# permon/permon

Measured on AMD Instinct MI355X. Metric: QPS iterations/sec + CSR SpMV GB/s (% HBM roofline), higher is better.
Workload: dtype f64; 1 GPU; configs[2]: 3-D elasticity TFETI contact, 2x2x2 subdomains of 43^3 Q1 elements (N=2044416 dof, n_lambda=102268), SMALXE+MPGP on the dual QP, F = B K^+ B' with K^+ explicit (dense local dual operators, storage class_orbit)

## Files before the change

permon_amd/csrc/ctx.hip:

```cpp
#include <sched.h>

#include <algorithm>
#include <thread>

#include "pmh_internal.h"

static thread_local char g_err[1024] = "";

int pmh_set_error(int code, const char *fmt, ...)
{
  va_list ap;
  va_start(ap, fmt);
  vsnprintf(g_err, sizeof(g_err), fmt, ap);
  va_end(ap);
  return code;
}

extern "C" const char *pmh_last_error(void) { return g_err; }

pmh_knobs_s &pmh_knobs()
{
  static pmh_knobs_s k = [] {
    pmh_knobs_s v;
    v.chain = getenv("PMH_NO_CHAIN") ? 0 : 1;
    v.chain_replay = getenv("PMH_NO_CHAIN_REPLAY") ? 0 : 1;
    v.svm_pairing = getenv("PMH_SVM_NO_PAIRING") ? 0 : 1;
    v.gt_fusion = getenv("PMH_NO_GT_FUSION") ? 0 : 1;
    v.multi_rhs = getenv("PMH_NO_MULTI_RHS") ? 0 : 1;
    v.kplus_mv = getenv("PMH_NO_KPLUS_MV") ? 0 : 1;
    v.smalxe_prefetch = getenv("PMH_SMALXE_NO_PREFETCH") ? 0 : 1;
    v.mg_d0_fusion = getenv("PMH_MG_NO_D0_FUSION") ? 0 : 1;
    v.vec_epi = getenv("PMH_NO_VEC_EPI") ? 0 : 1;
    v.mpgp_spec = getenv("PMH_MPGP_NO_SPEC") ? 0 : 1;
    v.orbit_adapted = getenv("PMH_NO_ORBIT_ADAPTED") ? 0 : 1;
    int         nt = 0;
    const char *e  = getenv("PMH_HOST_THREADS");
    if (!e) e = getenv("OMP_NUM_THREADS");
    if (e) nt = atoi(e);
    if (nt <= 0) {
      cpu_set_t set;
      CPU_ZERO(&set);
      nt = (sched_getaffinity(0, sizeof(set), &set) == 0) ? CPU_COUNT(&set) : (int)std::thread::hardware_concurrency();
      nt = std::min(16, nt);
    }
    v.host_threads = std::max(1, std::min(64, nt));
    return v;
  }();
  return k;
}
static int *knob_by_name(const char *name)
{
  if (!name) return nullptr;
  if (!strcmp(name, "chain")) return &pmh_knobs().chain;
  if (!strcmp(name, "chain_applies")) return &pmh_knobs().chain_applies;
  if (!strcmp(name, "chain_launches")) return &pmh_knobs().chain_launches;
  if (!strcmp(name, "chain_replay")) return &pmh_knobs().chain_replay;
  if (!strcmp(name, "chain_replays")) return &pmh_knobs().chain_replays;
  if (!strcmp(name, "chain_replays_redone")) return &pmh_knobs().chain_replays_redone;
  if (!strcmp(name, "host_threads")) return &pmh_knobs().host_threads;
  if (!strcmp(name, "svm_pairing")) return &pmh_knobs().svm_pairing;
  if (!strcmp(name, "gt_fusion")) return &pmh_knobs().gt_fusion;
  if (!strcmp(name, "multi_rhs")) return &pmh_knobs().multi_rhs;
  if (!strcmp(name, "kplus_mv")) return &pmh_knobs().kplus_mv;
  if (!strcmp(name, "smalxe_prefetch")) return &pmh_knobs().smalxe_prefetch;
  if (!strcmp(name, "mg_d0_fusion")) return &pmh_knobs().mg_d0_fusion;
  if (!strcmp(name, "mpgp_spec")) return &pmh_knobs().mpgp_spec;
  if (!strcmp(name, "vec_epi")) return &pmh_knobs().vec_epi;
  if (!strcmp(name, "orbit_adapted")) return &pmh_knobs().orbit_adapted;
  if (!strcmp(name, "orbit_adapted_classes")) return &pmh_knobs().orbit_adapted_classes;
  if (!strcmp(name, "orbit_adapted_fallbacks")) return &pmh_knobs().orbit_adapted_fallbacks;
  if (!strcmp(name, "orbit_adapted_spoil")) return &pmh_knobs().orbit_adapted_spoil;
  if (!strcmp(name, "orbit_narrow")) return &pmh_knobs().orbit_narrow;
  return nullptr;
}
extern "C" int pmh_set_knob(const char *name, int value)
{
  int *k = knob_by_name(name);
  if (!k) return pmh_set_error(PMH_ERR_ARG, "pmh_set_knob: unknown switch '%s'", name ? name : "(null)");
  *k = value;
  return PMH_SUCCESS;
}
extern "C" int pmh_get_knob(const char *name, int *value)
{
  int *k = knob_by_name(name);
  if (!k || !value) return pmh_set_error(PMH_ERR_ARG, "pmh_get_knob: unknown switch '%s'", name ? name : "(null)");
  *value = *k;
  return PMH_SUCCESS;
}

extern "C" int pmh_init(int device, pmh_ctx *out)
{
  PMH_ARG(out);
  int ndev = 0;
  if (hipGetDeviceCount(&ndev) != hipSuccess || ndev <= 0) return pmh_set_error(PMH_ERR_NODEVICE, "pmh_init: no HIP device visible (libpermonhip has no CPU fallback)");
  if (device < 0 || device >= ndev) return pmh_set_error(PMH_ERR_ARG, "pmh_init: device %d out of range [0,%d)", device, ndev);
  PMH_HIP(hipSetDevice(device));
  hipDeviceProp_t prop;
  PMH_HIP(hipGetDeviceProperties(&prop, device));
  if (!strstr(prop.gcnArchName, "gfx950")) return pmh_set_error(PMH_ERR_NODEVICE, "pmh_init: device %d is %s; libpermonhip is built for gfx950 (MI355X) only", device, prop.gcnArchName);
  pmh_ctx c  = new pmh_ctx_s();
  c->device  = device;
  c->num_cus = prop.multiProcessorCount;
  c->comm    = nullptr;
  c->rank    = 0;
  c->size    = 1;
  c->dist_scalars = 0;
  c->force_comm = getenv("PMH_COMM_FORCE") ? 1 : 0;
  PMH_HIP(hipStreamCreateWithFlags(&c->stream, hipStreamNonBlocking));
  PMH_HIP(hipEventCreate(&c->ev0));
  PMH_HIP(hipEventCreate(&c->ev1));
  c->partials_cap = PMH_MAX_VEC_BLOCKS;
  PMH_HIP(hipMalloc((void **)&c->d_partials, sizeof(double) * PMH_MAX_RED * c->partials_cap));
  PMH_HIP(hipMalloc((void **)&c->d_scal, sizeof(double) * PMH_NSCAL));
  PMH_HIP(hipMemset(c->d_scal, 0, sizeof(double) * PMH_NSCAL));
  PMH_HIP(hipHostMalloc((void **)&c->h_scal, sizeof(double) * PMH_NSCAL, hipHostMallocMapped));
  memset(c->h_scal, 0, sizeof(double) * PMH_NSCAL);
  PMH_HIP(hipHostMalloc((void **)&c->h_partials, sizeof(double) * PMH_MAX_RED * c->partials_cap, hipHostMallocMapped));
  memset(c->h_partials, 0, sizeof(double) * PMH_MAX_RED * c->partials_cap);
  PMH_HIP(hipMalloc((void **)&c->d_commbuf, sizeof(double) * PMH_NSCAL));
  *out = c;
  return PMH_SUCCESS;
}

extern "C" int pmh_finalize(pmh_ctx c)
{
  if (!c) return PMH_SUCCESS;
  hipSetDevice(c->device);
  hipStreamSynchronize(c->stream);
  if (c->comm) ncclCommDestroy(c->comm);
  for (int i = 0; i < c->comm_ev_cap; i++) hipEventDestroy(c->comm_ev[i]);
  delete[] c->comm_ev;
  if (c->h_stage) (void)hipHostFree(c->h_stage);
  hipFree(c->d_partials);
  hipFree(c->d_scal);
  hipFree(c->d_commbuf);
  hipHostFree(c->h_scal);
  hipHostFree(c->h_partials);
  hipEventDestroy(c->ev0);
  hipEventDestroy(c->ev1);
  hipStreamDestroy(c->stream);
  delete c;
// ... 262 lines not shown
```

permon_amd/csrc/dualchain.hip:

```cpp
#include <algorithm>
#include <cmath>
#include <type_traits>

#include "dualchain.h"
#include "emit_inline.h"
#include "box_inline.h"
#include "reduce.h"

struct pmh_dualchain_s {
  pmh_ctx  ctx;
  pmh_qppf pf;
  pmh_op   F;
  int      n, m, nwg, nseg, W;
  pmh_csr  gather = nullptr, scatter = nullptr;
  double  *mid_in = nullptr;
  const double *mid_out = nullptr;
  int     *d_seg = nullptr, *d_lrow = nullptr;
  double        *d_ev = nullptr;
  unsigned char *d_ec = nullptr;
  pmh_csr  list_for = nullptr;
  unsigned long long list_uid = 0, sc_uid = 0;
  double  *zeroed   = nullptr;
  int      nlist = 0, *d_reci = nullptr;
  double  *d_recd = nullptr;
  pmh_csr  sc_for = nullptr;
  int     *d_sc2 = nullptr;
  double  *d_sv2 = nullptr;
  unsigned char *d_scnt = nullptr;
  double  *part[3] = {nullptr, nullptr, nullptr};
  double  *c_cur   = nullptr;
  double  *w       = nullptr;
  double  *normGu    = nullptr;
  int      norm_slot = -1;
  const double *x_emitted = nullptr;
  bool     norm_done = false;
  const double *norm_ptr = nullptr;
  int      launches = 0;
  const double      *kept_x     = nullptr;
  unsigned long long kept_epoch = 0;
};


__global__ __launch_bounds__(PMH_EMIT_TILE) void k_dc_emit(int n, const double *__restrict__ x, pmh_emit_args ea)
{
  pmh_emit_regs R;
  pmh_emit_prefetch(ea, R);
  const int r = blockIdx.x * PMH_EMIT_TILE + threadIdx.x;
  pmh_emit_tail(ea, R, r < n ? x[r] : 0.0, 0.0);
}

template <int NU>
__global__ __launch_bounds__(PMH_EMIT_TILE) void k_dc_norm(pmh_emit_tab tab, const double *__restrict__ part, const double *__restrict__ Tt,
                        double *__restrict__ y2, double *__restrict__ norm_d,
                                                         double *__restrict__ norm_h)
{
  __shared__ double pt[PMH_EMIT_NW][64];
  const int         lane = threadIdx.x & 63, wave = threadIdx.x >> 6, m = tab.m;
  double            s1, s2;
  pmh_coarse_share<4, NU>(tab, part, Tt, nullptr, nullptr, s1, s2);
  pt[wave][lane] = s1;
  __syncthreads();
  if (wave == 0) {
    double y = 0.0;
#pragma unroll
    for (int w = 0; w < PMH_EMIT_NW; w++) y += pt[w][lane];
    if (lane < m) y2[lane] = y;
    const double sq = pmh_wave_all<PMH_RED_SUM>(lane < m ? y * y : 0.0);
    if (lane == 0) *norm_d = sq, *norm_h = sq;
  }
}

template <int W>
static __device__ __forceinline__ void dc_gt_load(const double *__restrict__ ev, const unsigned char *__restrict__ ec, int j, double (&v)[W],
                        unsigned char (&c)[W])
{
  typedef double dbl2 __attribute__((ext_vector_type(2)));
#pragma unroll
  for (int e = 0; e < W; e += 2) {
    const dbl2 d = *(const dbl2 *)(ev + (size_t)j * W + e);
    v[e] = d.x, v[e + 1] = d.y;
  }
#pragma unroll
  for (int h = 0; h < W / 8; h++) {
    const unsigned long long cc = *(const unsigned long long *)(ec + (size_t)j * W + 8 * h);
#pragma unroll
    for (int e = 0; e < 8; e++) c[8 * h + e] = (unsigned char)(cc >> (8 * e));
  }
}

struct dc_norm_args {
  const double *part, *Tt;
  double       *y2, *norm_d, *norm_h;
};
template <int W, int NU>
__global__ __launch_bounds__(PMH_EMIT_TILE) void k_dc_gather(int nlist, const int *__restrict__ reci, const double *__restrict__ recd,
                        const int *__restrict__ bcol, const double *__restrict__ bval,
                                                        const double *__restrict__ ev, const unsigned char *__restrict__ ec, pmh_emit_tab tab, const double *__restrict__ part,
                                                        const double *__restrict__ S, double *__restrict__ c_out, dc_norm_args na, const double *__restrict__ x, double *__restrict__ mid)
{
  typedef int    int4v __attribute__((ext_vector_type(4)));
  typedef double dbl2 __attribute__((ext_vector_type(2)));
  __shared__ double cs[64], ps[PMH_EMIT_NW][64], pt[PMH_EMIT_NW][64];
  const int         t = threadIdx.x, lane = t & 63, wave = t >> 6, i = blockIdx.x * PMH_EMIT_TILE + t, m = tab.m;
  int4v             ra = {0, -1, 0, 0}, rb = {0, 0, 0, 0};
  dbl2              da = {0.0, 0.0}, db = {0.0, 0.0};
  if (i < nlist) {
    ra = *(const int4v *)(reci + (size_t)8 * i), rb = *(const int4v *)(reci + (size_t)8 * i + 4);
    da = *(const dbl2 *)(recd + (size_t)4 * i), db = *(const dbl2 *)(recd + (size_t)4 * i + 2);
  }
  const int    r = ra.x, r2 = ra.y, k0 = ra.z, k1 = ra.w, cnt = (i < nlist) ? k1 - k0 : 0;
  const int    j[3]  = {rb.x, rb.y, rb.z};
  const double bv[3] = {da.x, da.y, db.x};
  double        xv[3], v0[W];
  unsigned char c0[W];
#pragma unroll
  for (int u = 0; u < 3; u++) xv[u] = (u < cnt) ? x[j[u]] : 0.0;
#pragma unroll
  for (int e = 0; e < W; e++) v0[e] = 0.0, c0[e] = 0;
  if (cnt > 0) dc_gt_load<W>(ev, ec, j[0], v0, c0);
  if (na.part && blockIdx.x == gridDim.x - 1) {
    double s1, s2;
    pmh_coarse_share<4, NU>(tab, na.part, na.Tt, nullptr, nullptr, s1, s2);
    pt[wave][lane] = s1;
    __syncthreads();
    if (wave == 0) {
      double y = 0.0;
#pragma unroll
      for (int w = 0; w < PMH_EMIT_NW; w++) y += pt[w][lane];
      if (lane < m) na.y2[lane] = y;
      const double sq = pmh_wave_all<PMH_RED_SUM>(lane < m ? y * y : 0.0);
      if (lane == 0) *na.norm_d = sq, *na.norm_h = sq;
    }
    return;
  }
  {
    double s1, s2;
    pmh_coarse_share<4, NU>(tab, part, S, nullptr, nullptr, s1, s2);
    ps[wave][lane] = s1;
    __syncthreads();
    if (wave == 0) {
      double cc = 0.0;
#pragma unroll
      for (int w = 0; w < PMH_EMIT_NW; w++) cc += ps[w][lane];
      cs[lane] = cc;
      if (blockIdx.x == 0 && lane < m) c_out[lane] = cc;
    }
    __syncthreads();
  }
  if (i >= nlist) return;
  double sum = 0.0;
  {
    double q = 0.0;
#pragma unroll
    for (int e = 0; e < W; e++) q += v0[e] * cs[c0[e]];
    sum += bv[0] * (-1.0 * q + xv[0]);
  }
#pragma unroll
  for (int u = 1; u < 3; u++)
    if (u < cnt) {
      double        vv[W];
      unsigned char cc[W];
      dc_gt_load<W>(ev, ec, j[u], vv, cc);
      double q = 0.0;
#pragma unroll
      for (int e = 0; e < W; e++) q += vv[e] * cs[cc[e]];
      sum += bv[u] * (-1.0 * q + xv[u]);
    }
  for (int k = k0 + 3; k < k1; k++) {
    const int     jj = bcol[k];
// ... 181 lines not shown
  DC_CHK(pmh_memcpy_h2d(ctx, dc->d_ev, ev.data(), sizeof(double) * ev.size()));
  DC_CHK(pmh_memcpy_h2d(ctx, dc->d_ec, ec.data(), ec.size()));
  for (int s = 0; s < 3; s++) {
    DC_CHK(pmh_malloc(ctx, sizeof(double) * (size_t)(nseg + 1), (void **)&dc->part[s]));
    DC_CHK(pmh_memset(ctx, dc->part[s], 0, sizeof(double) * (size_t)(nseg + 1)));
  }
  DC_CHK(pmh_malloc(ctx, sizeof(double) * 64, (void **)&dc->c_cur));
  DC_CHK(pmh_memset(ctx, dc->c_cur, 0, sizeof(double) * 64));
  DC_CHK(pmh_malloc(ctx, sizeof(double) * ((size_t)n + nseg + 1), (void **)&dc->w));
  DC_CHK(pmh_memset(ctx, dc->w, 0, sizeof(double) * ((size_t)n + nseg + 1)));
#undef DC_CHK
  *out = dc;
  return PMH_SUCCESS;
}

static int dc_prepare_stages(pmh_dualchain dc)
{
  pmh_ctx ctx = dc->ctx;
  if (!(dc->list_for == dc->gather && dc->list_uid == dc->gather->uid && dc->zeroed == dc->mid_in)) {
    const pmh_csr       Bg = dc->gather;
    std::vector<int>    rp((size_t)Bg->nrows + 1), ci((size_t)Bg->nnz);
    std::vector<double> va((size_t)Bg->nnz);
    PMH_CHK(pmh_memcpy_d2h(ctx, rp.data(), Bg->d_rowptr, sizeof(int) * rp.size()));
    PMH_CHK(pmh_memcpy_d2h(ctx, ci.data(), Bg->d_col, sizeof(int) * ci.size()));
    PMH_CHK(pmh_memcpy_d2h(ctx, va.data(), Bg->d_val, sizeof(double) * va.size()));
    auto key = [&](int r) {
      unsigned long long h = 1469598103934665603ULL;
      for (int k = rp[r]; k < rp[r + 1]; k++) {
        unsigned long long b;
        const double       a = fabs(va[k]);
        memcpy(&b, &a, 8);
        h = (h ^ (unsigned long long)(unsigned)ci[k]) * 1099511628211ULL;
        h = (h ^ b) * 1099511628211ULL;
      }
      return h;
    };
    auto opposite = [&](int r, int q) {
      if (rp[r + 1] - rp[r] != rp[q + 1] - rp[q]) return false;
      for (int k = rp[r], l = rp[q]; k < rp[r + 1]; k++, l++)
        if (ci[k] != ci[l] || va[k] != -va[l]) return false;
      return true;
    };
    std::vector<int> partner((size_t)Bg->nrows, -1);
    {
      std::vector<std::pair<unsigned long long, int>> keyed;
      for (int r = 0; r < Bg->nrows; r++)
        if (rp[r + 1] > rp[r]) keyed.push_back({key(r), r});
      std::sort(keyed.begin(), keyed.end());
      for (size_t a = 0; a < keyed.size(); a++) {
        const int r = keyed[a].second;
        if (partner[r] != -1) continue;
        for (size_t b = a + 1; b < keyed.size() && keyed[b].first == keyed[a].first; b++) {
          const int q = keyed[b].second;
          if (partner[q] == -1 && opposite(r, q)) {
            partner[r] = q, partner[q] = -2;
            break;
          }
        }
      }
    }
    std::vector<int>    reci;
    std::vector<double> recd;
    for (int r = 0; r < Bg->nrows; r++) {
      if (rp[r + 1] == rp[r] || partner[r] == -2) continue;
      const int k0 = rp[r], k1 = rp[r + 1];
      int       j[3] = {0, 0, 0};
      double    b[3] = {0.0, 0.0, 0.0};
      for (int u = 0; u < 3 && k0 + u < k1; u++) j[u] = ci[k0 + u], b[u] = va[k0 + u];
      const int ints[8] = {r, partner[r] >= 0 ? partner[r] : -1, k0, k1, j[0], j[1], j[2], 0};
      reci.insert(reci.end(), ints, ints + 8);
      recd.push_back(b[0]), recd.push_back(b[1]), recd.push_back(b[2]), recd.push_back(0.0);
    }
    if (dc->d_reci) {
      PMH_CHK(pmh_free(ctx, dc->d_reci));
      PMH_CHK(pmh_free(ctx, dc->d_recd));
    }
    dc->d_reci = nullptr, dc->d_recd = nullptr;
    PMH_CHK(pmh_malloc(ctx, sizeof(int) * (reci.size() + 8), (void **)&dc->d_reci));
    PMH_CHK(pmh_malloc(ctx, sizeof(double) * (recd.size() + 4), (void **)&dc->d_recd));
    PMH_CHK(pmh_memcpy_h2d(ctx, dc->d_reci, reci.data(), sizeof(int) * reci.size()));
    PMH_CHK(pmh_memcpy_h2d(ctx, dc->d_recd, recd.data(), sizeof(double) * recd.size()));
    PMH_CHK(pmh_memset(ctx, dc->mid_in, 0, sizeof(double) * (size_t)Bg->nrows));
    dc->nlist = (int)(reci.size() / 8), dc->list_for = Bg, dc->list_uid = Bg->uid, dc->zeroed = dc->mid_in;
  }
  if (dc->sc_for != dc->scatter || dc->sc_uid != dc->scatter->uid) {
    const pmh_csr       Bs = dc->scatter;
    const int           n  = dc->n;
    std::vector<int>    rp((size_t)n + 1), ci((size_t)Bs->nnz);
    std::vector<double> va((size_t)Bs->nnz);
    PMH_CHK(pmh_memcpy_d2h(ctx, rp.data(), Bs->d_rowptr, sizeof(int) * rp.size()));
    PMH_CHK(pmh_memcpy_d2h(ctx, ci.data(), Bs->d_col, sizeof(int) * ci.size()));
    PMH_CHK(pmh_memcpy_d2h(ctx, va.data(), Bs->d_val, sizeof(double) * va.size()));
    std::vector<int>           sc2((size_t)2 * n, 0);
    std::vector<double>        sv2((size_t)2 * n, 0.0);
    std::vector<unsigned char> cnt((size_t)n, 0);
    for (int r = 0; r < n; r++) {
      const int c = rp[r + 1] - rp[r];
      cnt[r]      = (unsigned char)std::min(c, 255);
      for (int u = 0; u < 2 && u < c; u++) sc2[(size_t)2 * r + u] = ci[rp[r] + u], sv2[(size_t)2 * r + u] = va[rp[r] + u];
    }
    if (!dc->d_sc2) {
      PMH_CHK(pmh_malloc(ctx, sizeof(int) * sc2.size(), (void **)&dc->d_sc2));
      PMH_CHK(pmh_malloc(ctx, sizeof(double) * sv2.size(), (void **)&dc->d_sv2));
      PMH_CHK(pmh_malloc(ctx, cnt.size(), (void **)&dc->d_scnt));
    }
    PMH_CHK(pmh_memcpy_h2d(ctx, dc->d_sc2, sc2.data(), sizeof(int) * sc2.size()));
    PMH_CHK(pmh_memcpy_h2d(ctx, dc->d_sv2, sv2.data(), sizeof(double) * sv2.size()));
    PMH_CHK(pmh_memcpy_h2d(ctx, dc->d_scnt, cnt.data(), cnt.size()));
    dc->sc_for = Bs, dc->sc_uid = Bs->uid;
  }
  return PMH_SUCCESS;
}

void pmh_dc_destroy(pmh_dualchain dc)
{
  if (!dc) return;
  pmh_free(dc->ctx, dc->d_seg), pmh_free(dc->ctx, dc->d_lrow), pmh_free(dc->ctx, dc->d_ev), pmh_free(dc->ctx, dc->d_ec);
  if (dc->d_reci) pmh_free(dc->ctx, dc->d_reci), pmh_free(dc->ctx, dc->d_recd);
  if (dc->d_sc2) pmh_free(dc->ctx, dc->d_sc2), pmh_free(dc->ctx, dc->d_sv2), pmh_free(dc->ctx, dc->d_scnt);
  for (int s = 0; s < 3; s++) pmh_free(dc->ctx, dc->part[s]);
  pmh_free(dc->ctx, dc->c_cur), pmh_free(dc->ctx, dc->w);
  delete dc;
}

static int dc_nu(pmh_dualchain dc) { return dc->nwg <= 128 ? 2 : 8; }

template <int V> using dc_int = std::integral_constant<int, V>;
template <typename F>
static void dc_dispatch(pmh_dualchain dc, F f)
{
  const bool w8 = dc->W == 8, nu2 = dc_nu(dc) == 2;
  if (w8 && nu2) f(dc_int<8>(), dc_int<2>());
  else if (w8) f(dc_int<8>(), dc_int<8>());
  else if (nu2) f(dc_int<16>(), dc_int<2>());
  else f(dc_int<16>(), dc_int<8>());
}

static pmh_emit_tab dc_tab(pmh_dualchain dc)
{
  pmh_emit_tab t;
  t.seg = dc->d_seg, t.gcol = dc->pf->G->d_col, t.gval = dc->pf->G->d_val, t.lrow = dc->d_lrow, t.m = dc->m, t.nwg = dc->nwg;
  return t;
}

static pmh_emit_args dc_emit_args(pmh_dualchain dc, double *part0, double *part1)
{
  pmh_emit_args ea;
  memset(&ea, 0, sizeof(ea));
  ea.tab = dc_tab(dc), ea.o[0].part = part0, ea.o[1].part = part1;
  return ea;
}

static void dc_launch_emit(pmh_dualchain dc, const double *x, double *part)
{
  hipLaunchKernelGGL(k_dc_emit, dim3((unsigned)dc->nwg), dim3(PMH_EMIT_TILE), 0, dc->ctx->stream, dc->n, x, dc_emit_args(dc, part, nullptr));
}

int pmh_dc_emit_begin(pmh_dualchain dc, const double *x, const double *p, pmh_emit_args *ea)
{
  *ea = dc_emit_args(dc, x ? dc->part[0] : nullptr, p ? dc->part[1] : nullptr);
  if ((x && x == dc->kept_x) || (p && p == dc->kept_x)) dc->kept_x = nullptr;
  if (x) dc->x_emitted = x, dc->norm_done = false, dc->norm_ptr = nullptr;
  return PMH_SUCCESS;
}

void pmh_dc_invalidate(pmh_dualchain dc, bool keep_applied)
// ... 2 lines not shown
  if (!keep_applied) dc->kept_x = nullptr;
}

int pmh_dc_set_norm_target(pmh_dualchain dc, double *Gu, int slot)
{
  PMH_ARG(dc && Gu && slot >= 0 && slot < PMH_NSCAL);
  dc->normGu = Gu, dc->norm_slot = slot, dc->norm_ptr = nullptr, dc->norm_done = false;
  return PMH_SUCCESS;
}

bool pmh_dc_norm_ready(pmh_dualchain dc, const double *u)
{
  if (!dc || !dc->normGu) return false;
  if (dc->norm_ptr == u) return true;
  if (dc->x_emitted == u && !dc->norm_done) {
    dc_dispatch(dc, [&](auto, auto NU) {
      hipLaunchKernelGGL(k_dc_norm<decltype(NU)::value>, dim3(1), dim3(PMH_EMIT_TILE), 0, dc->ctx->stream, dc_tab(dc), (const double *)dc->part[0], (const double *)dc->pf->d_Tt, dc->normGu,
                         dc->ctx->d_scal + dc->norm_slot, dc->ctx->h_scal + dc->norm_slot);
    });
    if (hipGetLastError() != hipSuccess) return false;
    dc->norm_done = true, dc->norm_ptr = u;
    return true;
  }
  return false;
}
int pmh_dc_last_launches(pmh_dualchain dc) { return dc ? dc->launches : 0; }

static int dc_last_stage(pmh_dualchain dc, const double *x, double *y, double rho, const pmh_vec_epi *epi)
{
  pmh_ctx     ctx = dc->ctx;
  hipStream_t st  = ctx->stream;
  const int   n = dc->n;
  const dim3  vgrid((unsigned)dc->nwg), eblk(PMH_EMIT_TILE);
  const int   kind = epi ? epi->kind : 0;
  pmh_emit_args ea = dc_emit_args(dc, nullptr, nullptr);
  pmh_vec_epi   e;
  memset(&e, 0, sizeof(e));
  if (epi) e = *epi;
  e.h_partials = nullptr;
  if (epi && epi->hosted) e.h_partials = ctx->h_partials, *epi->hosted = dc->nwg;
  if (kind == PMH_VEPI_GRAD_SPLIT && epi->emitted_p) {
    ea.o[1].part    = dc->part[1];
    *epi->emitted_p = 1;
  }
  dc_dispatch(dc, [&](auto W, auto NU) {
    constexpr int w = decltype(W)::value, nu = decltype(NU)::value;
    auto kern = kind == PMH_VEPI_P1 ? k_dc_final<PMH_VEPI_P1, w, nu> : kind == PMH_VEPI_GRAD_SPLIT ? k_dc_final<PMH_VEPI_GRAD_SPLIT, w, nu> : k_dc_final<0, w, nu>;
    hipLaunchKernelGGL(kern, vgrid, eblk, 0, st, n, (const double *)dc->d_ev, (const unsigned char *)dc->d_ec, ea.tab, (const double *)dc->pf->d_S, (const double *)dc->c_cur, (const double *)dc->w, rho, y,
                       e, x, ea);
  });
  dc->launches++;
  PMH_HIP(hipGetLastError());
  return PMH_SUCCESS;
}

int pmh_dc_apply(pmh_dualchain dc, const double *x, double *y, double rho, const pmh_vec_epi *epi)
{
  pmh_ctx     ctx = dc->ctx;
  hipStream_t st  = ctx->stream;
  const int   n = dc->n;
  const dim3  vgrid((unsigned)dc->nwg), eblk(PMH_EMIT_TILE);
  const int   kind = epi ? epi->kind : 0;
  dc->launches     = 0;
  dc->kept_x       = nullptr;
  const pmh_emit_tab tab = dc_tab(dc);
  int slot = (epi && epi->in_slot > 0) ? epi->in_slot - 1 : -1;
  if (slot < 0) {
    slot = (kind == PMH_VEPI_GRAD_SPLIT) ? 0 : (kind == PMH_VEPI_P1 ? 1 : 2);
    if (slot == 0) dc->x_emitted = x, dc->norm_done = false, dc->norm_ptr = nullptr;
    dc_launch_emit(dc, x, dc->part[slot]);
    dc->launches++;
  }
  PMH_CHK(dc->F->stages(&dc->gather, &dc->mid_in, &dc->scatter, &dc->mid_out));
  const pmh_csr Bg = dc->gather, Bs = dc->scatter;
  if (Bg->ncols != n || Bs->nrows != n) return pmh_set_error(PMH_ERR_STATE, "pmh_dc_apply: the operator's stages changed their dual dimension");
  PMH_CHK(dc_prepare_stages(dc));
  {
    dc_norm_args na;
    memset(&na, 0, sizeof(na));
    if (dc->normGu && dc->x_emitted && !dc->norm_done) {
      na.part = dc->part[0], na.Tt = dc->pf->d_Tt, na.y2 = dc->normGu, na.norm_d = ctx->d_scal + dc->norm_slot, na.norm_h = ctx->h_scal + dc->norm_slot;
      dc->norm_done = true, dc->norm_ptr = dc->x_emitted;
    }
    const dim3 ggrid((unsigned)(std::max(1, (dc->nlist + PMH_EMIT_TILE - 1) / PMH_EMIT_TILE) + (na.part ? 1 : 0)));
    dc_dispatch(dc, [&](auto W, auto NU) {
      hipLaunchKernelGGL(HIP_KERNEL_NAME(k_dc_gather<decltype(W)::value, decltype(NU)::value>), ggrid, eblk, 0, st, dc->nlist, (const int *)dc->d_reci, (const double *)dc->d_recd,
                         (const int *)Bg->d_col, (const double *)Bg->d_val, (const double *)dc->d_ev, (const unsigned char *)dc->d_ec, tab, (const double *)dc->part[slot],
                         (const double *)dc->pf->d_S, dc->c_cur, na, x, dc->mid_in);
    });
    dc->launches++;
  }
  PMH_HIP(hipGetLastError());
  PMH_CHK(dc->F->mid_apply());
  hipLaunchKernelGGL(k_dc_scatter, vgrid, eblk, 0, st, n, (const unsigned char *)dc->d_scnt, (const int *)dc->d_sc2, (const double *)dc->d_sv2, (const int *)Bs->d_rowptr, (const int *)Bs->d_col,
                     (const double *)Bs->d_val, dc->mid_out, dc->w, dc_emit_args(dc, dc->w + n, nullptr));
  dc->launches++;
  PMH_HIP(hipGetLastError());
  PMH_CHK(pmh_comm_allreduce_sum(ctx, dc->w, (size_t)n + (size_t)dc->nseg));
  PMH_CHK(dc_last_stage(dc, x, y, rho, epi));
  dc->kept_x = x, dc->kept_epoch = ctx->free_epoch;
  pmh_knobs().chain_applies++, pmh_knobs().chain_launches += dc->launches;
  return PMH_SUCCESS;
}

int pmh_dc_replay(pmh_dualchain dc, const double *x, double *y, double rho, const pmh_vec_epi *epi, int *replayed)
{
  const int kind = epi ? epi->kind : 0;
  if (replayed) *replayed = 0;
  bool      ok   = pmh_knobs().chain_replay && x && dc->kept_x == x && dc->kept_epoch == dc->ctx->free_epoch && (kind == 0 || kind == PMH_VEPI_GRAD_SPLIT);
  if (ok) {
    pmh_csr       g = nullptr, sc = nullptr;
    double       *mi = nullptr;
    const double *mo = nullptr;
    PMH_CHK(dc->F->stages(&g, &mi, &sc, &mo));
    ok = g && sc && g == dc->list_for && g->uid == dc->list_uid && mi == dc->zeroed && sc == dc->sc_for && sc->uid == dc->sc_uid && mo == dc->mid_out;
  }
  if (!ok) return pmh_dc_apply(dc, x, y, rho, epi);
  dc->launches = 0;
  if (kind == PMH_VEPI_GRAD_SPLIT && !(epi->in_slot > 0)) {
    dc->x_emitted = x, dc->norm_done = false, dc->norm_ptr = nullptr;
    dc_launch_emit(dc, x, dc->part[0]);
    dc->launches++;
  }
  PMH_CHK(dc_last_stage(dc, x, y, rho, epi));
  if (replayed) *replayed = 1;
  pmh_knobs().chain_applies++, pmh_knobs().chain_replays++, pmh_knobs().chain_launches += dc->launches;
  return PMH_SUCCESS;
}

int pmh_dc_test_emit(pmh_dualchain dc, const double *x)
{
  pmh_emit_args ea;
  PMH_CHK(pmh_dc_emit_begin(dc, x, nullptr, &ea));
  dc_launch_emit(dc, x, ea.o[0].part);
  PMH_HIP(hipGetLastError());
  return PMH_SUCCESS;
}
int pmh_dc_test_direction_sums(pmh_dualchain dc, int cap, double *host, int *nseg)
{
  PMH_ARG(host && nseg && cap >= dc->nseg);
  *nseg = dc->nseg;
  return pmh_memcpy_d2h(dc->ctx, host, dc->part[1], sizeof(double) * (size_t)dc->nseg);
}
int pmh_dc_test_info(pmh_dualchain dc, long long info[10])
{
  pmh_ctx ctx = dc->ctx;
  PMH_CHK(dc->F->stages(&dc->gather, &dc->mid_in, &dc->scatter, &dc->mid_out));
  PMH_CHK(dc_prepare_stages(dc));
  std::vector<int>           reci((size_t)8 * dc->nlist);
  std::vector<unsigned char> cnt((size_t)dc->n);
  PMH_CHK(pmh_memcpy_d2h(ctx, reci.data(), dc->d_reci, sizeof(int) * reci.size()));
  PMH_CHK(pmh_memcpy_d2h(ctx, cnt.data(), dc->d_scnt, cnt.size()));
  long long np = 0, n3 = 0, n2 = 0;
  for (int i = 0; i < dc->nlist; i++) np += reci[(size_t)8 * i + 1] >= 0, n3 += reci[(size_t)8 * i + 3] - reci[(size_t)8 * i + 2] > 3;
  for (int r = 0; r < dc->n; r++) n2 += cnt[r] > 2;
  const long long v[10] = {dc->n, dc->m, dc->nwg, dc->nseg, dc->W, dc_nu(dc), dc->nlist, np, n3, n2};
  for (int k = 0; k < 10; k++) info[k] = v[k];
  return PMH_SUCCESS;
}
int pmh_dc_test_read(pmh_dualchain dc, int what, int cap, double *host, int *len)
{
  PMH_ARG(host && len && what >= 0 && what <= 10);
  PMH_ARG(what < 4 || what > 6 || what == 6 || (dc->gather && dc->scatter));
  PMH_ARG((what != 7 && what != 8) || dc->normGu);
  pmh_ctx       ctx = dc->ctx;
  const int     m = dc->m;
  const double *src[11] = {dc->part[0], dc->part[1], dc->part[2], dc->c_cur, dc->mid_in, dc->mid_out, dc->w, dc->normGu, nullptr, dc->pf->d_S, dc->pf->d_Tt};
  const int     cnt[11] = {dc->nseg, dc->nseg, dc->nseg, m, dc->gather ? dc->gather->nrows : 0, dc->scatter ? dc->scatter->ncols : 0, dc->n + dc->nseg, m, 2, m * m, m * m};
  PMH_ARG(cap >= cnt[what]);
  *len = cnt[what];
  PMH_CHK(pmh_sync(ctx));
  if (what == 8) {
    host[1] = ctx->h_scal[dc->norm_slot];
    return pmh_memcpy_d2h(ctx, host, ctx->d_scal + dc->norm_slot, sizeof(double));
  }
  return pmh_memcpy_d2h(ctx, host, src[what], sizeof(double) * (size_t)cnt[what]);
}

struct StagedOp : pmh_op_s {
  pmh_csr g, mdl, sc;
  double *mi = nullptr, *mo = nullptr;
  ~StagedOp() override
  {
    pmh_free(ctx, mi);
    pmh_free(ctx, mo);
  }
  int mult(const double *x, double *y) override
  {
    PMH_CHK(pmh_csr_mult(g, x, mi));
    PMH_CHK(pmh_csr_mult(mdl, mi, mo));
    return pmh_csr_mult(sc, mo, y);
  }
  int stages(pmh_csr *gather, double **mid_in, pmh_csr *scatter, const double **mid_out) override
  {
    *gather = g, *mid_in = mi, *scatter = sc, *mid_out = mo;
    return PMH_SUCCESS;
  }
  int mid_apply() override { return pmh_csr_mult(mdl, mi, mo); }
};

extern "C" int pmh_op_test_create_staged(pmh_csr gather, pmh_csr middle, pmh_csr scatter, pmh_op *op)
{
  PMH_ARG(gather && middle && scatter && op && gather->nrows >= 1 && gather->ncols >= 1);
  PMH_ARG(middle->nrows == gather->nrows && middle->ncols == gather->nrows && scatter->nrows == gather->ncols && scatter->ncols == gather->nrows);
  StagedOp *o = new StagedOp();
  o->ctx = gather->ctx, o->n = gather->ncols, o->g = gather, o->mdl = middle, o->sc = scatter;
  const size_t bytes = sizeof(double) * (size_t)gather->nrows;
  int          rc    = pmh_malloc(o->ctx, bytes, (void **)&o->mi);
  if (!rc) rc = pmh_malloc(o->ctx, bytes, (void **)&o->mo);
  if (!rc) rc = pmh_memset(o->ctx, o->mi, 0, bytes);
  if (!rc) rc = pmh_memset(o->ctx, o->mo, 0, bytes);
  if (rc) {
    delete o;
    return rc;
  }
  *op = o;
  return PMH_SUCCESS;
}
```

permon_amd/csrc/emit_inline.h:

```cpp
#pragma once
#include <hip/hip_runtime.h>

#include "pmh_internal.h"

#define PMH_EMIT_TILE 1024
#define PMH_EMIT_NW (PMH_EMIT_TILE / 64)

template <int CTRL>
static __device__ __forceinline__ double pmh_dpp_mov(double v)
{
  int lo = __double2loint(v), hi = __double2hiint(v);
  lo     = __builtin_amdgcn_update_dpp(0, lo, CTRL, 0xf, 0xf, false);
  hi     = __builtin_amdgcn_update_dpp(0, hi, CTRL, 0xf, 0xf, false);
  return __hiloint2double(hi, lo);
}

template <int OP = PMH_RED_SUM>
static __device__ __forceinline__ double pmh_wave_all(double v)
{
#define PMH_COMB(a, b) ((OP == PMH_RED_SUM) ? ((a) + (b)) : fmin((a), (b)))
  v = PMH_COMB(v, pmh_dpp_mov<0xB1>(v));
  v = PMH_COMB(v, pmh_dpp_mov<0x4E>(v));
  v = PMH_COMB(v, pmh_dpp_mov<0x141>(v));
  v = PMH_COMB(v, pmh_dpp_mov<0x140>(v));
// ... 12 lines not shown
{
  __shared__ double bp[K][PMH_EMIT_NW];
  const int         lane = threadIdx.x & 63, wave = threadIdx.x >> 6, nw = blockDim.x >> 6;
#pragma unroll
  for (int k = 0; k < K; k++) {
    const double s = (op[k] == PMH_RED_SUM) ? pmh_wave_all<PMH_RED_SUM>(v[k]) : pmh_wave_all<PMH_RED_MIN>(v[k]);
    if (lane == 0) bp[k][wave] = s;
  }
  __syncthreads();
  if (threadIdx.x < K) {
    const int k = threadIdx.x;
    double    r = bp[k][0];
    for (int w = 1; w < nw; w++) r = (op[k] == PMH_RED_SUM) ? (r + bp[k][w]) : fmin(r, bp[k][w]);
    partials[(size_t)k * ld + blockIdx.x] = r;
    if (h_partials) h_partials[(size_t)k * ld + blockIdx.x] = r;
  }
}

static __device__ __forceinline__ double pmh_sum_block_partials(const double *__restrict__ row, int nblocks)
{
  const int lane = threadIdx.x & 63;
  double    p[8];
#pragma unroll
  for (int u = 0; u < 8; u++) p[u] = (lane + 64 * u < nblocks) ? row[lane + 64 * u] : 0.0;
  double acc = 0.0;
#pragma unroll
  for (int u = 0; u < 8; u++) acc += p[u];
  return pmh_wave_all<PMH_RED_SUM>(acc);
}

struct pmh_emit_regs {
  int    k0[4], k1[4], pp[4], gc[4][4];
  double gv[4][4];
};
static __device__ __forceinline__ void pmh_emit_prefetch(const pmh_emit_args &ea, pmh_emit_regs &R)
{
  if (ea.o[0].part == nullptr && ea.o[1].part == nullptr) return;
  const int lane = threadIdx.x & 63, wave = __builtin_amdgcn_readfirstlane(threadIdx.x >> 6), base = (int)blockIdx.x * PMH_EMIT_TILE;
#pragma unroll
  for (int q = 0; q < 4; q++) {
    const int s = (int)blockIdx.x * 64 + wave + q * PMH_EMIT_NW;
    R.k0[q] = ea.tab.seg[3 * s], R.k1[q] = ea.tab.seg[3 * s + 1], R.pp[q] = ea.tab.seg[3 * s + 2];
  }
#pragma unroll
  for (int q = 0; q < 4; q++)
#pragma unroll
    for (int u = 0; u < 4; u++) {
      const int k = R.k0[q] + lane + 64 * u;
      R.gv[q][u]  = (k < R.k1[q]) ? ea.tab.gval[k] : 0.0;
      R.gc[q][u]  = (k < R.k1[q]) ? ea.tab.gcol[k] - base : 0;
    }
}
static __device__ __forceinline__ void pmh_emit_tail(const pmh_emit_args &ea, const pmh_emit_regs &R, double v0, double v1)
{
  __shared__ double xs[2][PMH_EMIT_TILE];
  const int         t = threadIdx.x, lane = t & 63, base = (int)blockIdx.x * PMH_EMIT_TILE;
  const bool        e0 = ea.o[0].part != nullptr, e1 = ea.o[1].part != nullptr;
  if (!e0 && !e1) return;
  xs[0][t] = v0, xs[1][t] = v1;
  __syncthreads();
#pragma unroll
  for (int q = 0; q < 4; q++) {
    if (R.k1[q] <= R.k0[q]) continue;
    double a0 = 0.0, a1 = 0.0;
#pragma unroll
    for (int u = 0; u < 4; u++)
      if (R.k0[q] + lane + 64 * u < R.k1[q]) a0 += R.gv[q][u] * xs[0][R.gc[q][u]], a1 += R.gv[q][u] * xs[1][R.gc[q][u]];
    for (int k = R.k0[q] + lane + 256; k < R.k1[q]; k += 64) {
      const double v = ea.tab.gval[k];
      const int    c = ea.tab.gcol[k] - base;
      a0 += v * xs[0][c], a1 += v * xs[1][c];
    }
    if (e0) {
      a0 = pmh_wave_all<PMH_RED_SUM>(a0);
      if (lane == 0) ea.o[0].part[R.pp[q]] = a0;
    }
    if (e1) {
      a1 = pmh_wave_all<PMH_RED_SUM>(a1);
      if (lane == 0) ea.o[1].part[R.pp[q]] = a1;
    }
  }
}

template <int RPW, int NU = 8>
static __device__ __forceinline__ void pmh_coarse_share(const pmh_emit_tab &tab, const double *__restrict__ part, const double *__restrict__ M1,
                        const double *__restrict__ M2, double *a_out,
                                                       double &s1, double &s2)
{
  const int lane = threadIdx.x & 63, wave = threadIdx.x >> 6, nw = blockDim.x >> 6, m = tab.m;
  s1 = 0.0, s2 = 0.0;
#pragma unroll 1
  for (int qb = 0; qb < RPW; qb += 4) {
    if (wave + nw * qb >= m) break;
    double pv[4][NU], m1[4], m2[4];
#pragma unroll
    for (int q = 0; q < 4; q++) {
      const int  r  = wave + nw * (qb + q);
      const bool in = r < m;
      const int  c0 = in ? tab.lrow[r] : 0, c1 = in ? tab.lrow[r + 1] : 0;
#pragma unroll
      for (int u = 0; u < NU; u++) {
        const int c = c0 + lane + 64 * u;
        pv[q][u]    = (c < c1) ? part[c] : 0.0;
      }
      m1[q] = (in && M1 && lane < m) ? M1[(size_t)r * m + lane] : 0.0;
      m2[q] = (in && M2 && lane < m) ? M2[(size_t)r * m + lane] : 0.0;
    }
#pragma unroll
    for (int q = 0; q < 4; q++) {
      const int r = wave + nw * (qb + q);
      if (r >= m) break;
      double acc = 0.0;
#pragma unroll
      for (int u = 0; u < NU; u++) acc += pv[q][u];
      acc = pmh_wave_all<PMH_RED_SUM>(acc);
      if (a_out && lane == 0) a_out[r] = acc;
      s1 += m1[q] * acc, s2 += m2[q] * acc;
    }
  }
}
```

permon_amd/csrc/feti.hip:

```cpp
#include <algorithm>
#include <cmath>

#include "pmh_internal.h"
#include "feti_internal.h"
#include "mv_internal.h"
#include "diag_inv.h"
#include "reduce.h"


extern "C" int pmh_gluing_create(pmh_ctx ctx, int n_x, int n_lambda, int n_leaves, const int *leaves_row, const int *leaves_root, const double *leaves_sign, pmh_gluing *out)
{
  PMH_ARG(ctx && out && n_x >= 0 && n_lambda >= 0 && n_leaves >= 0);
  PMH_ARG(n_leaves == 0 || (leaves_row && leaves_root && leaves_sign));
  for (int i = 0; i < n_leaves; i++) {
    if (leaves_row[i] < 0 || leaves_row[i] >= n_x) return pmh_set_error(PMH_ERR_ARG, "pmh_gluing_create: leaf %d row %d out of [0,%d)", i, leaves_row[i], n_x);
    if (leaves_root[i] < 0 || leaves_root[i] >= n_lambda) return pmh_set_error(PMH_ERR_ARG, "pmh_gluing_create: leaf %d root %d out of [0,%d)", i, leaves_root[i], n_lambda);
  }
  auto build = [&](int nrows, int ncols, const int *rows, const int *cols, pmh_csr *M) -> int {
    std::vector<int>    rp((size_t)nrows + 1, 0), ci((size_t)n_leaves);
    std::vector<double> va((size_t)n_leaves);
    for (int i = 0; i < n_leaves; i++) rp[rows[i] + 1]++;
    for (int r = 0; r < nrows; r++) rp[r + 1] += rp[r];
    std::vector<int> pos(rp.begin(), rp.end() - 1);
    for (int i = 0; i < n_leaves; i++) {
// ... 727 lines not shown
  return pmh_csr_timing_enable(M->K->K, max_launches);
}

extern "C" int pmh_matinv_timing_get(pmh_matinv M, int *launches, double *total_ms, double *bytes_per_launch)
{
  PMH_ARG(M && launches && total_ms);
  if (M->mvc_state == 1) return pmh_matinv_mv_timing(M->mvc, 0, launches, total_ms, bytes_per_launch);
  if (M->Kb) {
    if (bytes_per_launch) *bytes_per_launch = pmh_bsr3_bytes(M->Kb);
    return pmh_bsr3_timing_get(M->Kb, launches, total_ms);
  }
  if (bytes_per_launch) PMH_CHK(pmh_csr_algorithmic_bytes(M->K->K, bytes_per_launch));
  return pmh_csr_timing_get(M->K->K, PMH_EPI_NONE, launches, total_ms);
}

extern "C" int pmh_matinv_multi_rhs_active(pmh_matinv M, int *active)
{
  PMH_ARG(M && active);
  PMH_CHK(matinv_mvc_init(M));
  *active = M->mvc_state == 1;
  return PMH_SUCCESS;
}

int pmh_matinv_test_pick(int entries, const double *hs, const int *hi, int cap, double *scal, int *ints)
{
  for (int e = 0; e < entries && e < cap; e++) {
    const int q = hi[(1 * entries + e) * 2 + 1] > hi[(0 * entries + e) * 2 + 1] ? 1 : 0;
    for (int k = 0; k < 2; k++) {
      if (scal) scal[2 * e + k] = hs[(q * entries + e) * 2 + k];
      if (ints) ints[2 * e + k] = hi[(q * entries + e) * 2 + k];
    }
  }
  return PMH_SUCCESS;
}
extern "C" int pmh_matinv_test_info(pmh_matinv M, long long info[8], int cap, double *scal, int *ints)
{
  PMH_ARG(M && info && cap >= 0);
  if (M->mvc_state == 1) return pmh_matinv_mv_test_state(M->mvc, info, cap, scal, ints);
  const int           nb = M->nblocks;
  std::vector<double> hs(4 * (size_t)nb);
  std::vector<int>    hi(4 * (size_t)nb);
  int                 na = 0, dn = 0;
  PMH_CHK(pmh_sync(M->ctx));
  PMH_CHK(pmh_memcpy_d2h(M->ctx, hs.data(), M->d_bs, sizeof(double) * hs.size()));
  PMH_CHK(pmh_memcpy_d2h(M->ctx, hi.data(), M->d_bi, sizeof(int) * hi.size()));
  PMH_CHK(pmh_memcpy_d2h(M->ctx, &na, M->d_nactive, sizeof(int)));
  PMH_CHK(pmh_memcpy_d2h(M->ctx, &dn, M->d_done, sizeof(int)));
  info[0] = M->wgs, info[1] = M->Kb ? 1 : 0, info[2] = 1, info[3] = na, info[4] = dn, info[5] = nb, info[6] = M->last_max_its, info[7] = M->total_spmv;
  return pmh_matinv_test_pick(nb, hs.data(), hi.data(), cap, scal, ints);
}

extern "C" int pmh_matinv_last_iterations(pmh_matinv M, int *max_block_its, long long *total_spmv)
{
  PMH_ARG(M);
  if (max_block_its) *max_block_its = M->last_max_its;
  if (total_spmv) *total_spmv = M->total_spmv;
  return PMH_SUCCESS;
}

struct FetiDualOp : pmh_op_s {
  pmh_gluing B;
  pmh_matinv Kplus;
  double    *t1, *t2;
  long long  applies = 0;
  ~FetiDualOp() override
  {
    pmh_free(ctx, t1);
    pmh_free(ctx, t2);
  }
  int mult(const double *x, double *y) override
  {
    applies++;
    if (Kplus->E && pmh_fexplicit_matches(Kplus->E, B)) return pmh_fexplicit_apply(Kplus->E, x, y);
    PMH_CHK(pmh_gluing_mult(B, x, t1));
    PMH_CHK(pmh_matinv_mult(Kplus, t1, t2));
    return pmh_gluing_mult_transpose(B, t2, y);
  }
  int mult_transpose(const double *x, double *y) override { return mult(x, y); }
  int stages(pmh_csr *gather, double **mid_in, pmh_csr *scatter, const double **mid_out) override
  {
    if (Kplus->E && pmh_fexplicit_matches(Kplus->E, B)) return pmh_fexplicit_stages(Kplus->E, gather, mid_in, scatter, mid_out);
    *gather = B->Bt, *mid_in = t1, *scatter = B->B, *mid_out = t2;
    return PMH_SUCCESS;
  }
  int mid_apply() override
  {
    applies++;
    if (Kplus->E && pmh_fexplicit_matches(Kplus->E, B)) return pmh_fexplicit_mid(Kplus->E);
    return pmh_matinv_mult(Kplus, t1, t2);
  }
};

extern "C" int pmh_feti_dual_applies(pmh_op F, long long *n)
{
  const FetiDualOp *o = dynamic_cast<const FetiDualOp *>(F);
  PMH_ARG(o && n);
  *n = o->applies;
  return PMH_SUCCESS;
}

extern "C" int pmh_op_create_feti_dual(pmh_gluing B, pmh_matinv Kplus, pmh_op *F)
{
  PMH_ARG(B && Kplus && F);
  PMH_ARG(B->n_x == Kplus->n);
  FetiDualOp *o = new FetiDualOp();
  o->ctx        = B->ctx;
  o->n          = B->n_lambda;
  o->B          = B;
  o->Kplus      = Kplus;
  PMH_CHK(pmh_malloc(o->ctx, sizeof(double) * (size_t)(B->n_x ? B->n_x : 1), (void **)&o->t1));
  PMH_CHK(pmh_malloc(o->ctx, sizeof(double) * (size_t)(B->n_x ? B->n_x : 1), (void **)&o->t2));
  *F = o;
  return PMH_SUCCESS;
}

extern "C" int pmh_pc_dual_lumped_apply(pmh_gluing B, pmh_blockdiag K, const double *x, double *y)
{
  PMH_ARG(B && K && B->n_x == K->n);
  pmh_ctx ctx = B->ctx;
  double *xw, *yw;
  PMH_CHK(pmh_malloc(ctx, sizeof(double) * (size_t)(K->n ? K->n : 1), (void **)&xw));
  PMH_CHK(pmh_malloc(ctx, sizeof(double) * (size_t)(K->n ? K->n : 1), (void **)&yw));
  int rc = pmh_gluing_mult(B, x, xw);
  if (!rc) rc = pmh_blockdiag_mult(K, xw, yw);
  if (!rc) rc = pmh_gluing_mult_transpose(B, yw, y);
  pmh_free(ctx, xw);
  pmh_free(ctx, yw);
  return rc;
}

struct pmh_feti_chain_s {
  pmh_ctx    ctx;
  pmh_gluing B;
  pmh_matinv Kplus;
  pmh_qppf   pf;
  int        n_x, n_lambda, has_box;
  pmh_op     F, A;
  double    *f, *d, *b_bar, *b, *lb_new, *lam_tilde, *t_x, *t_l;
};

extern "C" int pmh_qpt_feti_chain_create(pmh_gluing B, pmh_matinv Kplus, const double *f, const double *c, pmh_qppf pf, const double *e, const double *lb, pmh_feti_chain *out)
{
  PMH_ARG(B && Kplus && f && c && out && (!pf || e));
  PMH_ARG(B->n_x == Kplus->n && (!pf || pf->n == B->n_lambda));
  pmh_ctx          ctx = B->ctx;
  const int        nl = B->n_lambda, nx = B->n_x;
  pmh_feti_chain   ch = new pmh_feti_chain_s();
  memset(ch, 0, sizeof(*ch));
  ch->ctx = ctx, ch->B = B, ch->Kplus = Kplus, ch->pf = pf, ch->n_x = nx, ch->n_lambda = nl, ch->has_box = lb ? 1 : 0;
  const size_t bl = sizeof(double) * (size_t)(nl ? nl : 1), bx = sizeof(double) * (size_t)(nx ? nx : 1);
  PMH_CHK(pmh_malloc(ctx, bx, (void **)&ch->f));
  PMH_CHK(pmh_malloc(ctx, bx, (void **)&ch->t_x));
  PMH_CHK(pmh_malloc(ctx, bl, (void **)&ch->d));
  PMH_CHK(pmh_malloc(ctx, bl, (void **)&ch->t_l));
  PMH_CHK(pmh_malloc(ctx, bl, (void **)&ch->lam_tilde));
  PMH_CHK(pmh_memcpy_d2d(ctx, ch->f, f, bx));
  PMH_CHK(pmh_op_create_feti_dual(B, Kplus, &ch->F));
  PMH_CHK(pmh_matinv_mult(Kplus, ch->f, ch->t_x));
  PMH_CHK(pmh_gluing_mult_transpose(B, ch->t_x, ch->d));
  PMH_CHK(pmh_vec_axpy(ctx, nl, ch->d, -1.0, c));
  if (lb) {
    PMH_CHK(pmh_malloc(ctx, bl, (void **)&ch->lb_new));
    PMH_CHK(pmh_memcpy_d2d(ctx, ch->lb_new, lb, bl));
  }
  if (!pf) {
    PMH_CHK(pmh_memset(ctx, ch->lam_tilde, 0, bl));
// ... 121 lines not shown
```

permon_amd/csrc/feti_internal.h:

```cpp
#pragma once
#include <algorithm>
#include <vector>

#include "pmh_internal.h"

struct pmh_fexplicit_s;

struct pmh_gluing_s {
  pmh_ctx ctx;
  int     n_x, n_lambda, n_leaves;
  pmh_csr B, Bt;
  double *d_tmp;
  std::vector<int>    h_row, h_root;
  std::vector<double> h_sign;
};

struct pmh_blockdiag_s {
  pmh_ctx          ctx;
  int              nblocks, n;
  std::vector<int> rowstart;
  int             *d_rowstart;
  pmh_csr          K;
  pmh_bsr3         Kb = nullptr;
};

struct pmh_matinv_s {
  pmh_blockdiag K;
  pmh_ctx       ctx;
  int           n, nblocks, wgs;
  double        rtol, atol;
  int           max_it, jacobi;
  double       *dinv, *r, *z, *p, *Ap;
  double       *d_part, *d_partB;
  double       *d_bs;
  int          *d_bi;
  int          *d_nactive, *d_done, *h_nactive;
  int           last_max_its;
  long long     total_spmv;
  int     kdim;
  double *d_R, *d_coef, *d_fproj, *d_kpart;
  double *d_fnorm2 = nullptr;
  double  kernel_tol = 64.0;
  int  left = 0, nfix = 0;
  int *d_fix = nullptr;
  pmh_mg  mg;
  pmh_bsr3 Kb;
  pmh_fexplicit_s *E;
  struct pmh_matinv_mv_s *mvc = nullptr;
  int                     mvc_state = 0;
};

bool pmh_fexplicit_matches(pmh_fexplicit_s *E, pmh_gluing B);
int  pmh_fexplicit_apply(pmh_fexplicit_s *E, const double *lambda, double *y);
int  pmh_fexplicit_stages(pmh_fexplicit_s *E, pmh_csr *gather, double **mid_in, pmh_csr *scatter, const double **mid_out);
int  pmh_fexplicit_mid(pmh_fexplicit_s *E);
int  pmh_fexplicit_store_symmetrized(pmh_fexplicit_s *E, int b, const double *S, int lds);
int  pmh_fexplicit_mark_assembled(pmh_fexplicit_s *E, long long n_solves, double seconds);
struct fx_batch_window {
  int       begin = 0, end = 1 << 30;
  int       nbatch = 0;
  long long nsolves = 0;
  double    loop_seconds = 0.0;
  bool      complete = false;
};
int  pmh_fexplicit_set_window(pmh_fexplicit_s *E, fx_batch_window *w);

#include "mv_internal.h"
struct pmh_asm_solver {
  pmh_matinv    M = nullptr;
  pmh_matinv_mv V = nullptr;
  double       *umv = nullptr;
  int open(pmh_matinv solver, int nslots)
  {
    M = solver;
    if (nslots == solver->nblocks) return PMH_SUCCESS;
    if (nslots != solver->nblocks * PMH_MV_R) return pmh_set_error(PMH_ERR_ARG, "pmh_fexplicit_assemble: %d slots for a solver of %d blocks (one per block, or %d per block)", nslots, solver->nblocks, PMH_MV_R);
    int rc = pmh_matinv_mv_create(solver, &V);
    if (rc == PMH_EPI_UNSUPPORTED)
      return pmh_set_error(PMH_ERR_SUP, "pmh_fexplicit_assemble: the multi-right-hand-side K^+ does not apply to this solver: %s", pmh_mv_why());
    if (rc) return rc;
    return pmh_malloc(M->ctx, sizeof(double) * len(), (void **)&umv);
  }
  void close()
  {
    if (V) pmh_matinv_mv_destroy(V), V = nullptr;
    if (umv && M) pmh_free(M->ctx, umv), umv = nullptr;
  }
  int    R() const { return V ? PMH_MV_R : 1; }
  size_t len() const { return (size_t)std::max(1, M->n) * R(); }
  int    rows(int s) const { return M->K->rowstart[s / R() + 1] - M->K->rowstart[s / R()]; }
  int    rhs_index(int s, int rel) const { return V ? (M->K->rowstart[s / PMH_MV_R] + rel) * PMH_MV_R + s % PMH_MV_R : M->K->rowstart[s] + rel; }
  const double *sol_of(const double *sol, int s) const { return V ? sol + (size_t)(s % PMH_MV_R) * M->n + M->K->rowstart[s / PMH_MV_R] : sol + M->K->rowstart[s]; }
  int solve(const double *rhs, double *sol)
  {
    if (!V) return pmh_matinv_mult(M, rhs, sol);
    PMH_CHK(pmh_matinv_mv_mult(V, rhs, umv));
    return pmh_matinv_mv_to_columns(V, umv, sol);
  }
  bool hit_the_limit() const { return (V ? pmh_matinv_mv_last_iterations(V) : M->last_max_its) >= M->max_it; }
};
```

permon_amd/csrc/fexplicit.hip:

```cpp
#include <algorithm>
#include <thread>
#include <chrono>
#include <cmath>
#include <map>

#include "feti_internal.h"
#include "fshared.h"
#include "fx_assemble.h"
#include "pmh_internal.h"
#include "reduce.h"

typedef double dbl2 __attribute__((ext_vector_type(2)));

struct pmh_fexplicit_s {
  pmh_ctx       ctx;
  pmh_gluing    B;
  pmh_blockdiag K;
  pmh_gluing    Bhat;
  int           nb, ntot;
  std::vector<int> gstart;
  std::vector<int> ngam;
  std::vector<int> gamma;
  std::vector<size_t> goff;
  std::vector<int> ld;
// ... 958 lines not shown

int pmh_fexplicit_store_symmetrized(pmh_fexplicit_s *E, int b, const double *S, int lds)
{
  PMH_ARG(E && b >= 0 && b < E->nb && S && lds >= E->ngam[b]);
  if (E->sh || (E->storage != PMH_FX_FULL && E->storage != PMH_FX_SYM)) return pmh_set_error(PMH_ERR_SUP, "pmh_fexplicit_store_symmetrized: FULL / SYM storage only");
  if (E->stripe_size > 1) return pmh_set_error(PMH_ERR_SUP, "pmh_fexplicit_store_symmetrized: not on a striped operator");
  const int n = E->ngam[b];
  if (!n) return PMH_SUCCESS;
  const long long tot = (long long)n * n;
  const dim3      grid((unsigned)std::max(1LL, std::min(2048LL, (tot + PMH_BLOCK - 1) / PMH_BLOCK)));
  hipLaunchKernelGGL(k_fx_store_sym, grid, dim3(PMH_BLOCK), 0, E->ctx->stream, n, lds, E->ld[b], E->storage == PMH_FX_SYM ? 1 : 0, S, E->W[b]);
  PMH_HIP(hipGetLastError());
  return PMH_SUCCESS;
}

int pmh_fexplicit_mark_assembled(pmh_fexplicit_s *E, long long n_solves, double seconds)
{
  PMH_ARG(E);
  E->assembled = 1, E->n_solves += n_solves, E->assemble_seconds += seconds;
  return PMH_SUCCESS;
}


static int fx_gemv(pmh_fexplicit E)
{
  if (!E->nwg) return PMH_SUCCESS;
  if (E->storage == PMH_FX_SYM) {
    hipStream_t st    = E->ctx->stream;
    bool        timed = false;
    if (E->ev_on && (E->ev_seen++ % E->ev_stride) == 0 && (size_t)(2 * E->ev_used + 2) <= E->ev.size() && (size_t)E->ev_used < E->ev_mid.size()) {
      timed = true;
      PMH_HIP(hipEventRecord(E->ev[2 * E->ev_used], st));
    }
#define SYMV_LAUNCH(V) hipLaunchKernelGGL(k_fx_symv<V>, dim3(E->nsw), dim3(PMH_BLOCK), 0, st, (const int *)E->d_sw_block, (const int *)E->d_sw_band, (const int *)E->d_sw_seg, (const int *)E->d_gstart, (const int *)E->d_ld, (const long long *)E->d_woff, (const long long *)E->d_poff, (const long long *)E->d_doff, (const double *)E->Wbase, (const double *)E->xh, E->ydir, E->partial, E->seg)
    SYMV_LAUNCH(0);
#undef SYMV_LAUNCH
    if (timed) PMH_HIP(hipEventRecord(E->ev_mid[E->ev_used], st));
    if (E->nfw)
      hipLaunchKernelGGL(k_fx_symv_fin, dim3(E->nfw), dim3(PMH_BLOCK), 0, st, (const int *)E->d_fw_block, (const int *)E->d_fw_col0, (const int *)E->d_gstart, (const int *)E->d_ld, (const long long *)E->d_poff,
                         (const long long *)E->d_doff, (const int *)E->d_own_ptr, (const int *)E->d_own_list, (const double *)E->ydir, (const double *)E->partial, E->yh, E->seg);
    if (timed) {
      PMH_HIP(hipEventRecord(E->ev[2 * E->ev_used + 1], st));
      E->ev_used++;
    }
    PMH_HIP(hipGetLastError());
    return PMH_SUCCESS;
  }
  hipStream_t st    = E->ctx->stream;
  bool        timed = false;
  if (E->ev_on && (E->ev_seen++ % E->ev_stride) == 0 && (size_t)(2 * E->ev_used + 2) <= E->ev.size()) {
    timed = true;
    PMH_HIP(hipEventRecord(E->ev[2 * E->ev_used], st));
  }
#define FX_LAUNCH(RW) hipLaunchKernelGGL(k_fx_gemv<RW>, dim3(E->nwg), dim3(PMH_BLOCK), 0, st, (const int *)E->d_wg_block, (const int *)E->d_wg_row0, (const int *)E->d_gstart, (const int *)E->d_ngam, (const int *)E->d_ld, (const long long *)E->d_woff, (const double *)E->Wbase, (const double *)E->xh, E->yh)
  if (E->rw == 8) FX_LAUNCH(8);
  else if (E->rw == 2) FX_LAUNCH(2);
  else FX_LAUNCH(4);
#undef FX_LAUNCH
  if (timed) {
    PMH_HIP(hipEventRecord(E->ev[2 * E->ev_used + 1], st));
    E->ev_used++;
  }
  PMH_HIP(hipGetLastError());
  return PMH_SUCCESS;
}

bool pmh_fexplicit_matches(pmh_fexplicit_s *E, pmh_gluing B) { return E && E->assembled && (E->B == B || (E->stripe_size >= 1 && E->B->n_lambda == B->n_lambda)); }

int pmh_fexplicit_apply(pmh_fexplicit_s *E, const double *lambda, double *y)
{
  if (E->sh) return fxs_apply(E->sh, lambda, y);
  PMH_CHK(pmh_gluing_mult(E->Bhat, lambda, E->xh));
  PMH_CHK(fx_gemv(E));
  return pmh_gluing_mult_transpose(E->Bhat, E->yh, y);
}

int pmh_fexplicit_stages(pmh_fexplicit_s *E, pmh_csr *gather, double **mid_in, pmh_csr *scatter, const double **mid_out)
{
  if (E->sh) return fxs_stages(E->sh, gather, mid_in, scatter, mid_out);
  *gather = E->Bhat->Bt, *mid_in = E->xh, *scatter = E->Bhat->B, *mid_out = E->yh;
  return PMH_SUCCESS;
}
int pmh_fexplicit_mid(pmh_fexplicit_s *E) { return E->sh ? fxs_mid(E->sh) : fx_gemv(E); }

extern "C" int pmh_fexplicit_mult(pmh_fexplicit E, const double *lambda, double *y)
{
  PMH_ARG(E && lambda && y);
  if (!E->assembled) return pmh_set_error(PMH_ERR_STATE, "pmh_fexplicit_mult: the explicit blocks are not assembled yet");
  return pmh_fexplicit_apply(E, lambda, y);
}

extern "C" int pmh_fexplicit_dense_mult(pmh_fexplicit E, const double *xh, double *yh)
{
  PMH_ARG(E && xh && yh);
  if (E->sh) {
    const size_t nbytes = sizeof(double) * (size_t)fxs_multivector_length(E->sh);
    PMH_CHK(pmh_memcpy_d2d(E->ctx, fxs_X(E->sh), xh, nbytes));
    PMH_CHK(fxs_dense(E->sh));
    return pmh_memcpy_d2d(E->ctx, yh, fxs_Y(E->sh), nbytes);
  }
  PMH_CHK(pmh_memcpy_d2d(E->ctx, E->xh, xh, sizeof(double) * (size_t)E->ntot));
  PMH_CHK(fx_gemv(E));
  return pmh_memcpy_d2d(E->ctx, yh, E->yh, sizeof(double) * (size_t)E->ntot);
}

extern "C" int pmh_fexplicit_compressed_size(pmh_fexplicit E, int *ntot, int *gstart )
{
  PMH_ARG(E);
  if (E->sh) {
    if (ntot) *ntot = (int)fxs_multivector_length(E->sh);
    if (gstart)
      for (int b = 0; b <= E->nb; b++) gstart[b] = -1;
    return PMH_SUCCESS;
  }
  if (ntot) *ntot = E->ntot;
  if (gstart)
    for (int b = 0; b <= E->nb; b++) gstart[b] = E->gstart[b];
  return PMH_SUCCESS;
}

extern "C" int pmh_matinv_attach_explicit(pmh_matinv Kplus, pmh_fexplicit E)
{
  PMH_ARG(Kplus);
  if (E && !E->assembled) return pmh_set_error(PMH_ERR_STATE, "pmh_matinv_attach_explicit: assemble the explicit blocks first");
  if (E && E->stripe_size < 1 && E->K->n != Kplus->n) return pmh_set_error(PMH_ERR_ARG, "pmh_matinv_attach_explicit: size mismatch (%d vs %d)", E->K->n, Kplus->n);
  Kplus->E = E;
  return PMH_SUCCESS;
}

extern "C" int pmh_fexplicit_timing_enable(pmh_fexplicit E, int max_launches, int stride)
{
  PMH_ARG(E && max_launches >= 0);
  if (E->sh) return fxs_timing_enable(E->sh, max_launches);
  while ((int)E->ev.size() < 2 * max_launches) {
    hipEvent_t e;
    PMH_HIP(hipEventCreate(&e));
    E->ev.push_back(e);
  }
  while ((int)E->ev_mid.size() < max_launches) {
    hipEvent_t e;
    PMH_HIP(hipEventCreate(&e));
    E->ev_mid.push_back(e);
  }
  E->ev_on = max_launches > 0, E->ev_used = 0, E->ev_seen = 0, E->ev_stride = std::max(1, stride);
  return PMH_SUCCESS;
}

extern "C" int pmh_fexplicit_timing_get(pmh_fexplicit E, int *launches, double *total_ms, double *first_kernel_ms)
{
  PMH_ARG(E && launches && total_ms);
  if (E->sh) {
    return fxs_timing_get(E->sh, launches, total_ms, first_kernel_ms);
  }
  PMH_CHK(pmh_sync(E->ctx));
  double tot = 0.0, first = 0.0;
  for (int i = 0; i < E->ev_used; i++) {
    float ms = 0.f;
    PMH_HIP(hipEventElapsedTime(&ms, E->ev[2 * i], E->ev[2 * i + 1]));
    tot += ms;
    if (E->storage == PMH_FX_SYM) {
      PMH_HIP(hipEventElapsedTime(&ms, E->ev[2 * i], E->ev_mid[i]));
      first += ms;
    }
  }
  *launches = E->ev_used, *total_ms = tot;
  if (first_kernel_ms) *first_kernel_ms = (E->storage == PMH_FX_SYM) ? first : tot;
// ... 3 lines not shown
```

permon_amd/csrc/fshared.h:

```cpp
#pragma once
#include "feti_internal.h"

struct fx_shared;
int       fxs_create(pmh_gluing B, pmh_blockdiag K, const int *block_class, int sym, fx_shared **out, const int *extra_ptr = nullptr, const int *extra_rel = nullptr);
void      fxs_destroy(fx_shared *S);
int       fxs_set_stripe(fx_shared *S, int rank, int size);
int       fxs_class_union(fx_shared *S, int c, int *n_c, int *urel_out);
int       fxs_set_symmetry(fx_shared *S, int c, int nsym, const int *posmap, const signed char *sign);
int       fxs_set_symmetry_ops(fx_shared *S, int c, int nsym, const int *ops);
int       fxs_orbit_adapted(fx_shared *S, int c);
long long fxs_dense_bytes(fx_shared *S);
double    fxs_apply_bytes(fx_shared *S);
double    fxs_apply_flops(fx_shared *S);
void      fxs_apply_flops_detail(fx_shared *S, double *issued, double *dense);
int       fxs_assemble(fx_shared *S, pmh_matinv solver, int nslots, const int *slot_class, double rtol, int max_it, long long *n_solves, fx_batch_window *w = nullptr);
int       fxs_apply(fx_shared *S, const double *lambda, double *y);
int       fxs_dense(fx_shared *S);
int       fxs_stages(fx_shared *S, pmh_csr *gather, double **mid_in, pmh_csr *scatter, const double **mid_out);
int       fxs_mid(fx_shared *S);
long long fxs_multivector_length(fx_shared *S);
double   *fxs_X(fx_shared *S);
double   *fxs_Y(fx_shared *S);
int       fxs_fill_pattern(fx_shared *S, int byte);
int       fxs_get_block(fx_shared *S, int b, int n, const int *gamma, double *out_host);
int       fxs_test_load_class(fx_shared *S, int c, const double *W_host, int *all_loaded);
int       fxs_orbit_plan_info(fx_shared *S, int c, long long info[24]);
int       fxs_orbit_adapted_info(fx_shared *S, int c, long long info[200]);
int       fxs_orbit_adapted_transform(fx_shared *S, int c, int inverse, const double *in, double *out);
int       fxs_timing_enable(fx_shared *S, int max_launches);
int       fxs_timing_get(fx_shared *S, int *launches, double *total_ms, double *first_kernel_ms);
```

permon_amd/csrc/fshared.hip:

```cpp
#include "fshared_adapted.h"
#include "fx_assemble.h"
#include "orbitbasis.h"

extern char **environ;

static int fxs_build_launch(fx_shared *S)
{
  if (S->sym) {
    struct band { int c, g, m, nj; };
    std::vector<band> bands;
    long long         steps = 0;
    for (int c = 0; c < S->ncls; c++) {
      fxs_class &C = S->C[c];
      for (int m = C.nmb - 1; m >= 0; m--) {
        if (!C.own[FXM_MB * m]) continue;
        for (int g = 0; g < C.ngroups; g++) {
          const int nj = std::min(C.nsb, FXM_MB * (m + 1)) * FXM_RT;
          bands.push_back({c, g, m, nj});
          steps += (nj + 1) / 2;
        }
      }
    }
    int nwg = (int)std::max(1LL, std::min((long long)S->ctx->num_cus, steps));
    if (const char *e = getenv("PMH_FXM_NWG")) nwg = std::max(1, atoi(e));
// ... 161 lines not shown
    } else if (sym) {
      C.nsb = C.ld / FXM_RS, C.nmb = (C.nsb + FXM_MB - 1) / FXM_MB;
      C.own.assign((size_t)std::max(1, C.nsb), 1);
      C.ptm.assign((size_t)C.nmb + 1, 0);
      for (int m = 0; m < C.nmb; m++) C.ptm[m + 1] = C.ptm[m] + (long long)std::min(C.nsb, FXM_MB * (m + 1)) * FXM_RS * FXS_S;
      C.ptoff = pttot, C.ptsize = C.ptm[C.nmb];
      pttot += C.ngroups * C.ptsize;
      wtot += (long long)FXM_RS * FXM_RS * ((long long)C.nsb * (C.nsb + 1) / 2);
    } else
      wtot += (long long)C.ld * C.ld;
    xtot += (long long)C.ngroups * C.ld * C.S;
    PMH_CHK(pmh_malloc(ctx, sizeof(int) * (size_t)std::max(1, C.nc), (void **)&C.d_urel));
    if (C.nc) PMH_CHK(pmh_memcpy_h2d(ctx, C.d_urel, C.urel.data(), sizeof(int) * (size_t)C.nc));
  }
  if (xtot >= (1LL << 31)) return pmh_set_error(PMH_ERR_SUP, "pmh_fexplicit_create_shared: the multivector numbering exceeds 32-bit indices");
  S->nX = xtot, S->wtot = wtot;
  std::vector<int> rows((size_t)std::max(1, B->n_leaves));
  for (int i = 0; i < B->n_leaves; i++) {
    const int        b = lb[i];
    const fxs_class &C = S->C[S->cls[b]];
    rows[i]            = (int)(C.xoff + (long long)group[b] * C.ld * C.S + (long long)C.pos[B->h_row[i] - K->rowstart[b]] * C.S + slot[b]);
  }
  if (sym == 2) {
    for (auto &C : S->C) C.tmask.assign((size_t)std::max(1, C.ngroups) * std::max(1, C.nc) * FXS_S, 0);
    for (int i = 0; i < B->n_leaves; i++) {
      const int  b = lb[i];
      fxs_class &C = S->C[S->cls[b]];
      C.tmask[((size_t)group[b] * C.nc + C.pos[B->h_row[i] - K->rowstart[b]]) * FXS_S + slot[b]] = 1;
    }
    for (auto &C : S->C) {
      PMH_CHK(pmh_malloc(ctx, C.tmask.size(), (void **)&C.d_tmask));
      PMH_CHK(pmh_memcpy_h2d(ctx, C.d_tmask, C.tmask.data(), C.tmask.size()));
    }
  }
  PMH_CHK(pmh_gluing_create(ctx, (int)std::max(1LL, xtot), B->n_lambda, B->n_leaves, rows.data(), B->h_root.data(), B->h_sign.data(), &S->Bc));
  if (sym == 2) {
    if (2 * xtot >= (1LL << 31)) return pmh_set_error(PMH_ERR_SUP, "pmh_fexplicit_create_shared_orbit: the signed multivector numbering exceeds 32-bit indices");
    std::vector<int>    rows2((size_t)std::max(1, 2 * B->n_leaves)), root2((size_t)std::max(1, 2 * B->n_leaves));
    std::vector<double> sign2((size_t)std::max(1, 2 * B->n_leaves));
    for (int i = 0; i < B->n_leaves; i++) {
      const int slot_i = slot[lb[i]], base = rows[i] - slot_i, Sc = S->C[S->cls[lb[i]]].S;
      rows2[2 * i] = 2 * base + slot_i, rows2[2 * i + 1] = 2 * base + Sc + slot_i;
      root2[2 * i] = root2[2 * i + 1] = B->h_root[i];
      sign2[2 * i] = B->h_sign[i], sign2[2 * i + 1] = -B->h_sign[i];
    }
    PMH_CHK(pmh_gluing_create(ctx, (int)std::max(1LL, 2 * xtot), B->n_lambda, 2 * B->n_leaves, rows2.data(), root2.data(), sign2.data(), &S->Bc2));
    PMH_CHK(pmh_malloc(ctx, sizeof(double) * (size_t)std::max(32LL, 2 * xtot), (void **)&S->X2));
    PMH_CHK(pmh_memset(ctx, S->X2, 0, sizeof(double) * (size_t)std::max(32LL, 2 * xtot)));
  }
  {
    const size_t bytes = sizeof(double) * (size_t)std::max(32LL, wtot);
    hipError_t   e     = hipMalloc((void **)&S->Wbase, bytes);
    if (e != hipSuccess) return pmh_set_error(PMH_ERR_HIP, "pmh_fexplicit_create_shared: %.2f GB for the shared explicit operators: %s", bytes / 1e9, hipGetErrorString(e));
    PMH_HIP(hipMemsetAsync(S->Wbase, 0, bytes, ctx->stream));
  }
  if (sym == 1) {
    S->pt_tot = pttot;
    PMH_CHK(pmh_malloc(ctx, sizeof(double) * (size_t)std::max(16LL, pttot), (void **)&S->pt));
  }
  PMH_CHK(pmh_malloc(ctx, sizeof(double) * (size_t)std::max(16LL, xtot), (void **)&S->X));
  PMH_CHK(pmh_malloc(ctx, sizeof(double) * (size_t)std::max(16LL, xtot), (void **)&S->Y));
  PMH_CHK(pmh_memset(ctx, S->X, 0, sizeof(double) * (size_t)std::max(16LL, xtot)));
  PMH_CHK(pmh_memset(ctx, S->Y, 0, sizeof(double) * (size_t)std::max(16LL, xtot)));
  std::vector<int>       ldv(S->ncls);
  std::vector<long long> wo(S->ncls), xo(S->ncls);
  for (int c = 0; c < S->ncls; c++) ldv[c] = S->C[c].ld, wo[c] = S->C[c].woff, xo[c] = S->C[c].xoff;
  PMH_CHK(pmh_malloc(ctx, sizeof(int) * S->ncls, (void **)&S->d_ld));
  PMH_CHK(pmh_malloc(ctx, sizeof(long long) * S->ncls, (void **)&S->d_woff));
  PMH_CHK(pmh_malloc(ctx, sizeof(long long) * S->ncls, (void **)&S->d_xoff));
  PMH_CHK(pmh_memcpy_h2d(ctx, S->d_ld, ldv.data(), sizeof(int) * S->ncls));
  PMH_CHK(pmh_memcpy_h2d(ctx, S->d_woff, wo.data(), sizeof(long long) * S->ncls));
  PMH_CHK(pmh_memcpy_h2d(ctx, S->d_xoff, xo.data(), sizeof(long long) * S->ncls));
  if (sym != 2) PMH_CHK(fxs_build_launch(S));
  *out = S;
  return PMH_SUCCESS;
}

static void fxa_free(pmh_ctx ctx, fxs_class &C)
{
  fxa_class *a = C.oa;
  if (!a) return;
  if (a->Wh) (void)hipFree(a->Wh);
  for (void *q : {(void *)a->d_ir, (void *)a->d_tab, (void *)a->Xh, (void *)a->Yh, (void *)a->d_toff, (void *)a->d_osize, (void *)a->d_tbase, (void *)a->d_opos, (void *)a->d_rowinfo, (void *)a->d_items,
                  (void *)a->d_tmask, (void *)a->d_tabN, (void *)a->d_tabNT, (void *)a->d_nfx, (void *)a->d_nyd, (void *)a->d_nxh, (void *)a->d_nyh})
    if (q) pmh_free(ctx, q);
  delete a;
  C.oa = nullptr;
}

void fxs_destroy(fx_shared *S)
{
  if (!S) return;
  pmh_ctx ctx = S->ctx;
  for (auto &C : S->C) {
    if (C.d_urel) pmh_free(ctx, C.d_urel);
    if (C.d_tmask) pmh_free(ctx, C.d_tmask);
    if (C.d_nseg) pmh_free(ctx, C.d_nseg);
    if (C.d_ptoff) pmh_free(ctx, C.d_ptoff);
    if (C.d_ownfirst) pmh_free(ctx, C.d_ownfirst);
    if (C.d_posmap) pmh_free(ctx, C.d_posmap), pmh_free(ctx, C.d_sign);
    if (C.d_gidx) pmh_free(ctx, C.d_gidx), pmh_free(ctx, C.d_reppos), pmh_free(ctx, C.d_use);
    if (C.d_coltab) pmh_free(ctx, C.d_coltab), pmh_free(ctx, C.d_fintab), pmh_free(ctx, C.d_finbase);
    if (C.d_kinv) pmh_free(ctx, C.d_kinv), pmh_free(ctx, C.d_unittab), pmh_free(ctx, C.d_lut);
    fxa_free(ctx, C);
  }
  if (S->pt) pmh_free(ctx, S->pt);
  if (S->d_wgl) pmh_free(ctx, S->d_wgl);
  if (S->d_items) pmh_free(ctx, S->d_items);
  if (S->d_wgfirst) pmh_free(ctx, S->d_wgfirst);
  if (S->d_wgfirst_all) pmh_free(ctx, S->d_wgfirst_all);
  if (S->d_fin_args) pmh_free(ctx, S->d_fin_args);
  if (S->d_zrow_of) pmh_free(ctx, S->d_zrow_of), pmh_free(ctx, (void *)S->d_coltab_of), pmh_free(ctx, (void *)S->d_gidx_of);
  pmh_gluing_destroy(S->Bc);
  for (auto e : S->ev_mid) (void)hipEventDestroy(e);
  pmh_gluing_destroy(S->Bc2);
  pmh_free(ctx, S->X2);
  if (S->Wbase) (void)hipFree(S->Wbase);
  if (S->Afund) (void)hipFree(S->Afund);
  if (S->cpart) pmh_free(ctx, S->cpart);
  if (S->part) pmh_free(ctx, S->part);
  pmh_free(ctx, S->X), pmh_free(ctx, S->Y), pmh_free(ctx, S->d_wg), pmh_free(ctx, S->d_ld), pmh_free(ctx, S->d_woff), pmh_free(ctx, S->d_xoff);
  for (hipEvent_t e : S->ev) (void)hipEventDestroy(e);
  delete S;
}


static inline int fxm_owner(int m, int nmb, int size)
{
  const int i = nmb - 1 - m, round = i / size, k = i % size;
  return (round & 1) ? size - 1 - k : k;
}

extern "C" int pmh_fexplicit_class_sym_plan(int n_c, int size, int *owner_out, double *bytes_per_rank)
{
  PMH_ARG(n_c >= 1 && size >= 1);
  const int nsb = (n_c + FXM_RS - 1) / FXM_RS, nmb = (nsb + FXM_MB - 1) / FXM_MB;
  if (bytes_per_rank)
    for (int r = 0; r < size; r++) bytes_per_rank[r] = 0.0;
  for (int m = 0; m < nmb; m++) {
    const int o = fxm_owner(m, nmb, size);
    if (owner_out) owner_out[m] = o;
    if (bytes_per_rank)
      for (int sb = FXM_MB * m; sb < std::min(nsb, FXM_MB * (m + 1)); sb++) bytes_per_rank[o] += (double)(sb + 1) * FXM_RT * FXM_RT * 2048.0;
  }
  return PMH_SUCCESS;
}

int fxs_set_stripe(fx_shared *S, int rank, int size)
{
  if (S->sym == 2) {
    S->stripe_rank = rank, S->stripe_size = size, S->fxo_ready = 0;
    return PMH_SUCCESS;
  }
  if (S->sym) {
    for (auto &C : S->C) {
      for (int m = 0; m < C.nmb; m++)
        for (int sb = FXM_MB * m; sb < std::min(C.nsb, FXM_MB * (m + 1)); sb++) C.own[sb] = fxm_owner(m, C.nmb, size) == rank;
    }
    return fxs_build_launch(S);
  }
  for (auto &C : S->C) {
    const int nrg = C.ld / 32;
    C.r0 = (int)((long long)nrg * rank / size) * 32;
    C.r1 = (int)((long long)nrg * (rank + 1) / size) * 32;
  }
  return fxs_build_launch(S);
}

long long fxs_dense_bytes(fx_shared *S) { return S->sym ? (long long)S->owned_bytes : (long long)sizeof(double) * S->wtot; }
static bool fxa_active(fx_shared *S)
{
  if (S->sym != 2 || !pmh_knobs().orbit_adapted) return false;
  bool any = false;
  for (const fxs_class &C : S->C) {
    if (!C.nc) continue;
    if (!C.oa) return false;
    any = true;
  }
  return any;
}
int fxs_orbit_adapted(fx_shared *S, int c) { return c >= 0 && c < S->ncls && S->C[c].oa && fxa_active(S); }
double fxs_apply_flops(fx_shared *S)
{
  if (!fxa_active(S)) return S->sym == 2 ? S->flops : 0.0;
  double f = 0.0;
  for (const fxs_class &C : S->C)
    if (C.oa) f += C.oa->flops;
  return f;
}
void fxs_apply_flops_detail(fx_shared *S, double *issued, double *dense)
{
  *issued = S->sym == 2 ? S->flops_issued : 0.0, *dense = S->sym == 2 ? S->flops_dense : 0.0;
  if (!fxa_active(S)) return;
  *issued = 0.0;
  for (const fxs_class &C : S->C)
    if (C.oa) *issued += C.oa->flops_issued;
}
double fxs_apply_bytes(fx_shared *S)
{
  if (!fxa_active(S)) return S->bytes;
  double b = 0.0;
  for (const fxs_class &C : S->C)
    if (C.oa) b += C.oa->bytes;
  return b;
}

int fxs_class_union(fx_shared *S, int c, int *n_c, int *urel_out)
{
  PMH_ARG(S && c >= 0 && c < S->ncls);
  if (n_c) *n_c = S->C[c].nc;
  if (urel_out && S->C[c].nc) memcpy(urel_out, S->C[c].urel.data(), sizeof(int) * (size_t)S->C[c].nc);
  return PMH_SUCCESS;
}

int fxs_set_symmetry(fx_shared *S, int c, int nsym, const int *posmap, const signed char *sign)
{
  PMH_ARG(S && c >= 0 && c < S->ncls && nsym >= 1 && posmap && sign);
  if (!S->sym) return pmh_set_error(PMH_ERR_SUP, "pmh_fexplicit_set_class_symmetry: needs the PMH_FX_CLASS_SYM or PMH_FX_CLASS_ORBIT storage");
  S->fxo_ready = 0;
  fxs_class &C  = S->C[c];
  const int  nc = C.nc;
  std::vector<char> seen((size_t)std::max(1, nc));
  for (int g = 0; g < nsym; g++) {
    std::fill(seen.begin(), seen.end(), 0);
    for (int i = 0; i < nc; i++) {
      const int t = posmap[(size_t)g * nc + i];
      if (t < 0 || t >= nc || seen[t] || (sign[(size_t)g * nc + i] != 1 && sign[(size_t)g * nc + i] != -1))
        return pmh_set_error(PMH_ERR_ARG, "pmh_fexplicit_set_class_symmetry: operation %d is not a signed permutation of the %d touched dofs", g, nc);
      if (g == 0 && (t != i || sign[i] != 1)) return pmh_set_error(PMH_ERR_ARG, "pmh_fexplicit_set_class_symmetry: operation 0 must be the identity");
      seen[t] = 1;
    }
  }
  C.nsym = nsym;
  C.h_ops.clear();
  fxa_free(S->ctx, C);
  C.h_posmap.assign(posmap, posmap + (size_t)nsym * nc);
  C.h_sign.assign(sign, sign + (size_t)nsym * nc);
  if (C.d_posmap) pmh_free(S->ctx, C.d_posmap), pmh_free(S->ctx, C.d_sign);
  PMH_CHK(pmh_malloc(S->ctx, sizeof(int) * (size_t)std::max(1, nsym * nc), (void **)&C.d_posmap));
  PMH_CHK(pmh_malloc(S->ctx, (size_t)std::max(1, nsym * nc), (void **)&C.d_sign));
  if (nc) {
    PMH_CHK(pmh_memcpy_h2d(S->ctx, C.d_posmap, C.h_posmap.data(), sizeof(int) * (size_t)nsym * nc));
    PMH_CHK(pmh_memcpy_h2d(S->ctx, C.d_sign, C.h_sign.data(), (size_t)nsym * nc));
  }
  return PMH_SUCCESS;
}


int fxs_set_symmetry_ops(fx_shared *S, int c, int nsym, const int *ops)
{
  PMH_ARG(S && c >= 0 && c < S->ncls && ops && nsym == S->C[c].nsym);
  S->C[c].h_ops.assign(ops, ops + 6 * (size_t)nsym);
  return PMH_SUCCESS;
}

static int fxo_instance(int tm, int tn, int tnw, bool tables)
{
  if (tnw == 48) return tables && tn == 64 && (tm == 192 || tm == 128 || tm == 64) ? tm + 2 : 0;
  if (tm != 144 && tm != 128 && tm != 112 && tm != 96 && tm != 80) return 0;
  if (!tables) return tn == 128 ? 1000 + tm : 0;
  return tn == 64 ? tm + 1 : (tn == 128 ? tm : 0);
}
static int fxo_launch_kind(const fx_shared *S, const fxs_class &C) { return S->merged_tm > 0 && S->nwg_all > 0 ? 2 : (C.S != FXS_S ? 1 : 0); }

static int fxo_gemm(fx_shared *S)
{
  hipStream_t st = S->ctx->stream;
  const bool  merged = S->merged_tm > 0 && S->nwg_all > 0;
  if (merged) {
#define FXO_LAUNCH_ALL(NI, NWM, TNW)                                                                                                                                                                      \
  hipLaunchKernelGGL(HIP_KERNEL_NAME(k_fxo_gemm16<NI, NWM, true, TNW>), dim3(S->nwg_all), dim3(256), 0, st, (const int *)S->d_items, (const long long *)S->d_wgl, (const int *)S->d_wg,                 \
                     (const int *)(S->d_wg + S->ncls), (const int *)nullptr, 0, (const double *)S->Afund, (const int *)nullptr, (const double *)S->X2, S->cpart, (const int *)S->d_wgfirst_all, \
                     (const int *const *)S->d_coltab_of, (const int *)S->d_zrow_of, (const int *const *)S->d_gidx_of, (const int *)(S->d_zrow_of + S->ncls))
    switch (fxo_instance(S->merged_tm, S->merged_tn, S->merged_tnw, true)) {
    case 194: FXO_LAUNCH_ALL(3, 4, 48); break;
    case 130: FXO_LAUNCH_ALL(2, 4, 48); break;
    case 66: FXO_LAUNCH_ALL(1, 4, 48); break;
    case 144: FXO_LAUNCH_ALL(9, 1, 128); break;
    case 145: FXO_LAUNCH_ALL(9, 1, 64); break;
    case 128: FXO_LAUNCH_ALL(4, 2, 128); break;
    case 129: FXO_LAUNCH_ALL(4, 2, 64); break;
    case 112: FXO_LAUNCH_ALL(7, 1, 128); break;
    case 113: FXO_LAUNCH_ALL(7, 1, 64); break;
    case 96: FXO_LAUNCH_ALL(3, 2, 128); break;
    case 97: FXO_LAUNCH_ALL(3, 2, 64); break;
    case 80: FXO_LAUNCH_ALL(5, 1, 128); break;
// ... 37 lines not shown
      case 112: FXO_LAUNCH_T(7, 1, 128); break;
      case 113: FXO_LAUNCH_T(7, 1, 64); break;
      case 96: FXO_LAUNCH_T(3, 2, 128); break;
      case 97: FXO_LAUNCH_T(3, 2, 64); break;
      case 80: FXO_LAUNCH_T(5, 1, 128); break;
      case 81: FXO_LAUNCH_T(5, 1, 64); break;
      default: return pmh_set_error(PMH_ERR_STATE, "PMH_FX_CLASS_ORBIT: row tile %d has no 16x16x4 kernel", C.tm);
      }
#undef FXO_LAUNCH_T
    } else {
      switch (fxo_instance(C.tm, C.tn, C.tnw, false)) {
      case 1144: FXO_LAUNCH((k_fxo_gemm16<9, 1>)); break;
      case 1128: FXO_LAUNCH((k_fxo_gemm16<4, 2>)); break;
      case 1112: FXO_LAUNCH((k_fxo_gemm16<7, 1>)); break;
      case 1096: FXO_LAUNCH((k_fxo_gemm16<3, 2>)); break;
      case 1080: FXO_LAUNCH((k_fxo_gemm16<5, 1>)); break;
      default: return pmh_set_error(PMH_ERR_STATE, "PMH_FX_CLASS_ORBIT: row tile %d has no 16x16x4 kernel", C.tm);
      }
    }
#undef FXO_LAUNCH
    if (!merged && S->ev_mid_pending >= 0 && c == S->ncls - 1) PMH_HIP(hipEventRecord(S->ev_mid[S->ev_mid_pending], st));
#ifdef FXO_TRACE
    if (++traced == 300) {
      std::vector<unsigned long long> h(8 * 64 * 8);
      PMH_HIP(hipStreamSynchronize(st));
      PMH_HIP(hipMemcpy(h.data(), d_trace, sizeof(unsigned long long) * h.size(), hipMemcpyDeviceToHost));
      for (int w = 0; w < 8; w++) {
        fprintf(stderr, "FXO_TRACE workgroup %d (cycles of the shader clock; per chunk: loads issued | products | wait vmcnt | LDS store | barrier | total)\n", w * 37);
        for (int ch = 0; ch < 63; ch++) {
          const unsigned long long *q = &h[((size_t)w * 64 + ch) * 8];
          if (!q[5]) break;
#ifdef FXO_TRACE_FULL
          fprintf(stderr, "  chunk %2d: %6llu | %6llu | %6llu | %6llu | %6llu | %6llu\n", ch, q[1] - q[0], q[2] - q[1], q[3] - q[2], q[4] - q[3], q[5] - q[4], q[5] - q[0]);
#else
          fprintf(stderr, "  chunk %2d: %6llu | %6llu | %6llu | %6llu | %6llu | %6llu\n", ch, 0ULL, q[2] - q[0], 0ULL, 0ULL, q[5] - q[2], q[5] - q[0]);
#endif
        }
      }
    }
#endif
    if (C.fin_elems > 0 && !S->d_fin_args)
      hipLaunchKernelGGL(k_fxo_fin, dim3((unsigned)((C.fin_elems + PMH_BLOCK - 1) / PMH_BLOCK), C.ngroups), dim3(PMH_BLOCK), 0, st, C.Mp / C.tm, C.tm, C.nsymp, C.nc, (const int *)C.d_fintab,
                         (const int *)C.d_unittab, (const long long *)C.d_finbase, (const int *)C.d_lut, (const int *)C.d_coltab, (const double *)S->cpart, (const signed char *)C.d_use, (const int *)C.d_reppos, (const int *)C.d_posmap, C.xoff, C.ld,
                         S->Y, C.S, (const char *)C.d_tmask);
  }
  if (S->d_fin_args && S->fin_nbx > 0)
    hipLaunchKernelGGL(k_fxo_fin_all, dim3((unsigned)S->fin_nbx, (unsigned)S->fin_ngroups, (unsigned)S->ncls), dim3(PMH_BLOCK), 0, st, (const fxo_fin_args *)S->d_fin_args, (const double *)S->cpart, S->Y);
  PMH_HIP(hipGetLastError());
  return PMH_SUCCESS;
}

__global__ __launch_bounds__(PMH_BLOCK) void k_fxo_signed_copy(long long n, int nslot, const double *__restrict__ X, double *__restrict__ X2)
{
  for (long long i = (long long)blockIdx.x * PMH_BLOCK + threadIdx.x; i < n; i += (long long)gridDim.x * PMH_BLOCK) {
    const long long p = i / nslot, sl = i % nslot;
    const double    v = X[i];
    X2[2 * p * nslot + sl] = v, X2[(2 * p + 1) * nslot + sl] = -v;
  }
}

static void fxa_launch_transform(fx_shared *S, const fxs_class &C, bool inv)
{
  const fxa_class *a  = C.oa;
  hipStream_t      st = S->ctx->stream;
  if (a->narrow) {
    const dim3 grid(a->norb, C.ngroups), block(FXN_T);
    if (inv)
      hipLaunchKernelGGL(k_fxa_narrow<true>, grid, block, 0, st, (const double *)a->d_tabNT, (const int *)a->d_osize, (const int *)a->d_nyd, (const long long *)a->d_nyh, a->norb, (long long)C.ld * FXS_S,
                         (const double *)a->Yh, S->Y + C.xoff);
    else
      hipLaunchKernelGGL(k_fxa_narrow<false>, grid, block, 0, st, (const double *)a->d_tabN, (const int *)a->d_osize, (const int *)a->d_nfx, (const long long *)a->d_nxh, a->norb, 2LL * C.ld * FXS_S,
                         (const double *)(S->X2 + 2 * C.xoff), a->Xh);
    return;
  }
  const dim3 grid(a->norb, (a->NC + FXA_CB - 1) / FXA_CB);
  if (inv)
    hipLaunchKernelGGL(k_fxa_transform<true>, grid, dim3(PMH_BLOCK), 0, st, (const fxa_irrep *)a->d_ir, (const double *)a->d_tab, (const long long *)a->d_toff, (const int *)a->d_osize, (const int *)a->d_tbase,
                       (const int *)a->d_opos, (const int *)a->d_rowinfo, a->NC, C.nc, C.ld, C.xoff, (const double *)S->X2, a->Xh, (const double *)a->Yh, S->Y, (const char *)a->d_tmask);
  else
    hipLaunchKernelGGL(k_fxa_transform<false>, grid, dim3(PMH_BLOCK), 0, st, (const fxa_irrep *)a->d_ir, (const double *)a->d_tab, (const long long *)a->d_toff, (const int *)a->d_osize, (const int *)a->d_tbase,
                       (const int *)a->d_opos, (const int *)a->d_rowinfo, a->NC, C.nc, C.ld, C.xoff, (const double *)S->X2, a->Xh, (const double *)a->Yh, S->Y, (const char *)a->d_tmask);
}

static int fxa_launch(fx_shared *S)
{
  hipStream_t st = S->ctx->stream;
  for (fxs_class &C : S->C)
    if (C.oa) fxa_launch_transform(S, C, false);
  for (fxs_class &C : S->C)
    if (fxa_class *a = C.oa)
      if (a->nitems) hipLaunchKernelGGL(k_fxa_prod, dim3(a->nitems), dim3(64 * FXA_WAVES), 0, st, (const int *)a->d_items, (const fxa_irrep *)a->d_ir, (const double *)a->Wh, (const double *)a->Xh, a->Yh);
  if (S->ev_mid_pending >= 0) PMH_HIP(hipEventRecord(S->ev_mid[S->ev_mid_pending], st));
  for (fxs_class &C : S->C)
    if (C.oa) fxa_launch_transform(S, C, true);
  PMH_HIP(hipGetLastError());
  return PMH_SUCCESS;
}

template <class T> static int fxa_upload(pmh_ctx ctx, const std::vector<T> &h, T **d)
{
  PMH_CHK(pmh_malloc(ctx, sizeof(T) * std::max<size_t>(1, h.size()), (void **)d));
  if (!h.empty()) PMH_CHK(pmh_memcpy_h2d(ctx, *d, h.data(), sizeof(T) * h.size()));
  return PMH_SUCCESS;
}

static int fxa_build_class(fx_shared *S, fxs_class &C, bool spoil)
{
  pmh_ctx     ctx = S->ctx;
  oab_basis   B;
  std::string why;
  if (!oab_build(C.nsym, C.nc, C.h_posmap.data(), C.h_sign.data(), C.h_ops.data(), B, why)) {
    if (getenv("PMH_ORBIT_ADAPTED_VERBOSE")) fprintf(stderr, "orbit_adapted: no basis (%s): the class keeps the GEMM\n", why.c_str());
    return PMH_SUCCESS;
  }
  if (B.norb != C.M_all) return PMH_SUCCESS;
  for (int o = 0; o < B.norb; o++)
    if (B.opos[B.tbase[o]] != C.reps[o]) return PMH_SUCCESS;
  fxa_class *a = new fxa_class();
  C.oa = a;
  a->norb = B.norb, a->NC = C.ngroups * FXS_S, a->nc = C.nc;
  const int M = C.M_all;
  long long wtot = 0, htot = 0, ytot = 0;
  a->narrow = pmh_knobs().orbit_narrow && a->NC <= FXN_NC && C.nc < (1 << 23);
  double    tfl = 0.0, tfl_issued = 0.0, tab_read = 0.0;
  for (int o = 0; o < B.norb; o++) {
    const double no = B.osize[o], no4 = (B.osize[o] + 3) & ~3;
    tfl += 2.0 * 2.0 * no * no * a->NC;
    tfl_issued += 2.0 * 2.0 * no * (a->narrow ? no4 : no) * a->NC;
    tab_read += a->narrow ? no * no4 * C.ngroups : 48.0 * 48.0;
  }
  a->flops = tfl, a->flops_issued = tfl_issued;
  for (int i = 0; i < OAB_NIRREP; i++) {
    fxa_irrep &I = a->ir[i];
    I.d = B.d[i], I.m = B.m[i];
    I.nks = ((I.m + 7) / 8 + FXA_KU - 1) / FXA_KU * FXA_KU, I.nob = (I.m + 15) / 16, I.nbt = (I.d * a->NC + 15) / 16, I.ldy = 16 * I.nbt;
    I.woff = wtot, I.hoff = htot, I.yoff = ytot;
    wtot += (long long)I.nob * I.nks * 128, htot += (long long)I.nbt * I.nks * 128, ytot += (long long)I.nob * 16 * I.ldy;
    a->flops += 2.0 * (double)I.m * I.m * I.d * a->NC;
    a->flops_issued += 2.0 * (16.0 * I.nob) * (8.0 * I.nks) * (16.0 * I.nbt);
  }
  a->bytes = 8.0 * ((double)wtot + 2.0 * htot + 2.0 * ytot + 2.0 * tab_read + 2.0 * (double)C.nc * a->NC) + (a->narrow ? 2.0 * 12.0 * C.nc * C.ngroups : 0.0);
  {
    const size_t bytes = sizeof(double) * (size_t)std::max(128LL, wtot);
    hipError_t   e     = hipMalloc((void **)&a->Wh, bytes);
    if (e != hipSuccess) return pmh_set_error(PMH_ERR_HIP, "PMH_FX_CLASS_ORBIT: %.2f GB for the blocks of the symmetry-adapted form: %s", bytes / 1e9, hipGetErrorString(e));
    PMH_HIP(hipMemsetAsync(a->Wh, 0, bytes, ctx->stream));
  }
  PMH_CHK(pmh_malloc(ctx, sizeof(double) * (size_t)std::max(128LL, htot), (void **)&a->Xh));
  PMH_CHK(pmh_malloc(ctx, sizeof(double) * (size_t)std::max(128LL, ytot), (void **)&a->Yh));
  PMH_CHK(pmh_memset(ctx, a->Xh, 0, sizeof(double) * (size_t)std::max(128LL, htot)));
  PMH_CHK(pmh_memset(ctx, a->Yh, 0, sizeof(double) * (size_t)std::max(128LL, ytot)));
  std::vector<int> rowinfo((size_t)C.nc), orb_of((size_t)C.nc), items;
  for (int o = 0; o < B.norb; o++)
    for (int t = 0; t < B.osize[o]; t++) orb_of[B.tbase[o] + t] = o;
  for (int r = 0; r < C.nc; r++) rowinfo[r] = B.row_irrep[r] | (B.row_partner[r] << 4) | (B.row_index[r] << 8);
  {
    int order[OAB_NIRREP];
    for (int i = 0; i < OAB_NIRREP; i++) order[i] = i;
    std::stable_sort(order, order + OAB_NIRREP, [&](int x, int y) { return a->ir[x].m > a->ir[y].m; });
    for (int i : order) {
      const fxa_irrep &I = a->ir[i];
      for (int nb0 = 0; nb0 < I.nbt; nb0 += 4)
        for (int ob = 0; ob < I.nob; ob++) {
          const int nbw = std::min(4, I.nbt - nb0);
          items.insert(items.end(), {i, ob, nb0, nbw});
          a->items_of_width[i][nbw - 1]++;
        }
    }
    a->nitems = (int)(items.size() / 4);
  }
  std::vector<fxa_irrep> irv(a->ir, a->ir + OAB_NIRREP);
// ... 31 lines not shown
          nxh[f] = fxa_xh_off(I, B.row_index[r], n), nyh[f] = I.yoff + (long long)B.row_index[r] * I.ldy + n, nyd[f] = pos << 8 | bits;
        }
      }
    PMH_CHK(fxa_upload(ctx, nfx, &a->d_nfx));
    PMH_CHK(fxa_upload(ctx, nyd, &a->d_nyd));
    PMH_CHK(fxa_upload(ctx, nxh, &a->d_nxh));
    PMH_CHK(fxa_upload(ctx, nyh, &a->d_nyh));
  }
  double *Abuf = nullptr;
  int    *d_reprow = nullptr;
  PMH_CHK(pmh_malloc(ctx, sizeof(double) * (size_t)C.nc * M, (void **)&Abuf));
  PMH_CHK(fxa_upload(ctx, C.reprow, &d_reprow));
  {
    std::vector<int> hops;
    int             *d_hops = nullptr;
    double          *tmp = nullptr;
    PMH_CHK(pmh_malloc(ctx, sizeof(int) * OAB_NOP, (void **)&d_hops));
    PMH_CHK(pmh_malloc(ctx, sizeof(double) * (size_t)C.nc, (void **)&tmp));
    const int nbx = std::max(1, std::min(64, (C.nc + PMH_BLOCK - 1) / PMH_BLOCK));
    for (int o = 0; o < B.norb; o++) {
      if (B.osize[o] == OAB_NOP) continue;
      const int p = C.reps[o];
      hops.clear();
      for (int g = 0; g < OAB_NOP; g++)
        if (C.h_posmap[(size_t)g * C.nc + p] == p) hops.push_back(g);
      PMH_CHK(pmh_memcpy_h2d(ctx, d_hops, hops.data(), sizeof(int) * hops.size()));
      hipLaunchKernelGGL(k_fxa_stab_avg, dim3(nbx), dim3(PMH_BLOCK), 0, ctx->stream, (int)hops.size(), (const int *)d_hops, p, C.reprow[o], C.tm, C.nc, C.nkc, (const int *)C.d_posmap, (const signed char *)C.d_sign,
                         (const int *)C.d_kinv, (const double *)(S->Afund + C.aoff), tmp);
      hipLaunchKernelGGL(k_fxa_stab_store, dim3(nbx), dim3(PMH_BLOCK), 0, ctx->stream, C.reprow[o], C.tm, C.nc, C.nkc, (const int *)C.d_kinv, (const double *)tmp, S->Afund + C.aoff);
      PMH_CHK(pmh_sync(ctx));
    }
    pmh_free(ctx, d_hops), pmh_free(ctx, tmp);
  }
  hipLaunchKernelGGL(k_fxa_rows, dim3(B.norb, (M + 63) / 64), dim3(64), 0, ctx->stream, M, C.tm, C.nkc, (const double *)a->d_tab, (const long long *)a->d_toff, (const int *)a->d_osize, (const int *)a->d_tbase,
                     (const int *)a->d_opos, (const int *)C.d_kinv, (const int *)d_reprow, (const double *)(S->Afund + C.aoff), Abuf);
  int rc = PMH_SUCCESS;
  for (int i = 0; i < OAB_NIRREP && !rc; i++) {
    const fxa_irrep &I = a->ir[i];
    if (!I.m) continue;
    std::vector<int>    fn0((size_t)I.m), orb((size_t)I.m);
    std::vector<double> vs(3 * (size_t)I.m);
    for (int r = 0; r < C.nc; r++)
      if (B.row_irrep[r] == i && B.row_partner[r] == 0) {
        const int k = B.row_index[r], o = orb_of[r];
        fn0[k] = r, orb[k] = o;
        for (int b = 0; b < 3; b++) vs[3 * (size_t)k + b] = B.row_vs[3 * (size_t)r + b];
      }
    int    *d_fn0 = nullptr, *d_orb = nullptr;
    double *d_vs = nullptr;
    if ((rc = fxa_upload(ctx, fn0, &d_fn0)) || (rc = fxa_upload(ctx, orb, &d_orb)) || (rc = fxa_upload(ctx, vs, &d_vs))) break;
    hipLaunchKernelGGL(k_fxa_combine, dim3((unsigned)(((long long)I.m * I.m + PMH_BLOCK - 1) / PMH_BLOCK)), dim3(PMH_BLOCK), 0, ctx->stream, I, M, (const int *)d_fn0, (const int *)d_orb, (const double *)d_vs,
                       (const double *)Abuf, a->Wh);
    rc = pmh_sync(ctx);
    pmh_free(ctx, d_fn0), pmh_free(ctx, d_orb), pmh_free(ctx, d_vs);
  }
  if (!rc) rc = pmh_sync(ctx);
  pmh_free(ctx, Abuf), pmh_free(ctx, d_reprow);
  if (!rc && hipGetLastError() != hipSuccess) rc = pmh_set_error(PMH_ERR_HIP, "PMH_FX_CLASS_ORBIT: a set-up launch of the symmetry-adapted form failed");
  if (!rc && spoil) {
    std::vector<double> bad = tabp;
    for (int o = 0; o < B.norb; o++)
      for (int j = 0; j < B.osize[o]; j++) bad[(size_t)toffp[o] + j] = -bad[(size_t)toffp[o] + j];
    rc = pmh_memcpy_h2d(ctx, a->d_tab, bad.data(), sizeof(double) * bad.size());
    tabp.swap(bad);
  }
  if (!rc && a->narrow) {
    std::vector<double> tabN(tabp.size()), tabNT(tabp.size());
    for (int o = 0; o < B.norb; o++)
      for (int t = 0; t < 48; t++)
        for (int j = 0; j < 48; j++) {
          const double v = tabp[(size_t)toffp[o] + t * 48 + j];
          tabN[(size_t)toffp[o] + fxn_tab_off(t, j)] = v, tabNT[(size_t)toffp[o] + fxn_tab_off(j, t)] = v;
        }
    rc = fxa_upload(ctx, tabN, &a->d_tabN);
    if (!rc) rc = fxa_upload(ctx, tabNT, &a->d_tabNT);
  }
  return rc;
}

static int fxa_setup(fx_shared *S)
{
  pmh_ctx ctx = S->ctx;
  for (fxs_class &C : S->C) fxa_free(ctx, C);
  if (!pmh_knobs().orbit_adapted || S->stripe_size > 1 || ctx->size > 1) return PMH_SUCCESS;
  for (char **e = environ; e && *e; e++)
    if (!strncmp(*e, "PMH_FXO_", 8)) return PMH_SUCCESS;
  const bool spoil = pmh_knobs().orbit_adapted_spoil != 0;
  pmh_knobs().orbit_adapted_spoil = 0;
  bool any = false;
  for (fxs_class &C : S->C) {
    if (!C.nc) continue;
    if (C.S != FXS_S || C.nsym != OAB_NOP || C.h_ops.size() != 6 * (size_t)OAB_NOP || C.m0 != 0 || C.m1 != C.M_all || C.tmask.empty()) {
      if (getenv("PMH_ORBIT_ADAPTED_VERBOSE")) fprintf(stderr, "orbit_adapted: not eligible (slots %d, operations %d, box operations known %d): the class keeps the GEMM\n", C.S, C.nsym, (int)(C.h_ops.size() / 6));
      continue;
    }
    const int rc = fxa_build_class(S, C, spoil);
    if (rc) {
      fxa_free(ctx, C);
      return rc;
    }
    any = any || C.oa;
  }
  if (!any) return PMH_SUCCESS;
  std::vector<double> x((size_t)S->nX, 0.0), y0((size_t)S->nX), y1((size_t)S->nX);
  unsigned long long  seed = 0x9E3779B97F4A7C15ULL;
  for (fxs_class &C : S->C) {
    if (!C.oa) continue;
    for (int g = 0; g < C.ngroups; g++)
      for (int p = 0; p < C.nc; p++)
        for (int sl = 0; sl < FXS_S; sl++)
          if (C.tmask[((size_t)g * C.nc + p) * FXS_S + sl]) {
            seed = seed * 6364136223846793005ULL + 1442695040888963407ULL;
            x[(size_t)(C.xoff + (long long)g * C.ld * FXS_S + (long long)p * FXS_S + sl)] = (double)(seed >> 11) / 4503599627370496.0 - 1.0;
          }
  }
  PMH_CHK(pmh_memcpy_h2d(ctx, S->X, x.data(), sizeof(double) * x.size()));
  for (const fxs_class &C : S->C) {
    const long long n = (long long)C.ngroups * C.ld * C.S;
    if (!n) continue;
    hipLaunchKernelGGL(k_fxo_signed_copy, dim3((unsigned)std::min<long long>(4096, (n + PMH_BLOCK - 1) / PMH_BLOCK)), dim3(PMH_BLOCK), 0, ctx->stream, n, C.S, (const double *)(S->X + C.xoff), S->X2 + 2 * C.xoff);
  }
  PMH_CHK(fxo_gemm(S));
  PMH_CHK(pmh_memcpy_d2h(ctx, y0.data(), S->Y, sizeof(double) * y0.size()));
  PMH_CHK(pmh_memset(ctx, S->Y, 0, sizeof(double) * (size_t)S->nX));
  PMH_CHK(fxa_launch(S));
  PMH_CHK(pmh_memcpy_d2h(ctx, y1.data(), S->Y, sizeof(double) * y1.size()));
  for (fxs_class &C : S->C) {
    if (!C.oa) continue;
    double dd = 0.0, nn = 0.0;
    for (int g = 0; g < C.ngroups; g++)
      for (long long k = 0; k < (long long)C.nc * FXS_S; k++)
        if (C.tmask[(size_t)g * C.nc * FXS_S + (size_t)k]) {
          const size_t i = (size_t)(C.xoff + (long long)g * C.ld * FXS_S + k);
          dd += (y1[i] - y0[i]) * (y1[i] - y0[i]), nn += y0[i] * y0[i];
        }
    if (getenv("PMH_ORBIT_ADAPTED_VERBOSE")) fprintf(stderr, "orbit_adapted: self-check against the GEMM: normwise relative difference %.3e (n_c = %d, %d groups)\n", std::sqrt(dd / nn), C.nc, C.ngroups);
    if (!(dd <= 1e-20 * nn)) fxa_free(ctx, C), pmh_knobs().orbit_adapted_fallbacks++;
    else pmh_knobs().orbit_adapted_classes++;
  }
  PMH_CHK(pmh_memset(ctx, S->X, 0, sizeof(double) * (size_t)S->nX));
  PMH_CHK(pmh_memset(ctx, S->X2, 0, sizeof(double) * 2 * (size_t)S->nX));
  PMH_CHK(pmh_memset(ctx, S->Y, 0, sizeof(double) * (size_t)S->nX));
  return pmh_sync(ctx);
}

static inline int     fxs_row_grid(int n) { return std::max(1, std::min(64, (n + PMH_BLOCK - 1) / PMH_BLOCK)); }
static inline double *fxs_super_band(fx_shared *S, const fxs_class &C, int row)
{
  const long long sb = row / FXM_RS;
  return S->Wbase + C.woff + (long long)FXM_RS * FXM_RS * (sb * (sb + 1) / 2);
}
static void fxo_store_row(fx_shared *S, const fxs_class &C, int row, const int *d_rel, const double *u)
{
  hipLaunchKernelGGL(k_fxo_store_row, dim3(fxs_row_grid(C.nc)), dim3(PMH_BLOCK), 0, S->ctx->stream, row, C.tm, C.nc, C.nkc, d_rel, (const int *)C.d_kinv, u, S->Afund + C.aoff);
}

static void fxs_plan_full(fx_shared *S, fx_asm_plan &P)
{
  for (int c = 0; c < S->ncls; c++) {
    const fxs_class &C = S->C[c];
    for (int p = C.r0; p < std::min(C.r1, C.nc); p++) P.todo[c].push_back({C.urel[p], p});
  }
  P.write = [S](int c, int p, const double *u) {
    const fxs_class &C = S->C[c];
    fx_extract_row(S->ctx, C.nc, C.d_urel, u, S->Wbase + C.woff + (long long)p * C.ld);
  };
}

static void fxs_plan_tiles(fx_shared *S, fx_asm_plan &P)
{
  std::vector<std::map<int, std::vector<std::pair<int, int>>>> members(S->ncls);
  for (int c = 0; c < S->ncls; c++) {
    const fxs_class &C = S->C[c];
    if (C.nsym <= 1) {
      for (int p = 0; p < C.nc; p++)
        if (C.own[p / FXM_RS]) P.todo[c].push_back({C.urel[p], p});
      continue;
    }
    std::vector<int> rep_of((size_t)C.nc, -1), op_of((size_t)C.nc, 0);
    for (int p = 0; p < C.nc; p++) {
      if (rep_of[p] >= 0) continue;
      for (int g = 0; g < C.nsym; g++) {
        const int r = C.h_posmap[(size_t)g * C.nc + p];
        if (rep_of[r] < 0) rep_of[r] = p, op_of[r] = g;
      }
    }
    for (int r = 0; r < C.nc; r++)
      if (C.own[r / FXM_RS]) {
        members[c][rep_of[r]].push_back({r, op_of[r]});
        if (op_of[r] != 0) P.check[c].push_back({C.urel[r], r});
      }
    for (const auto &m : members[c]) P.todo[c].push_back({C.urel[m.first], m.first});
  }
  P.write = [S, members = std::move(members)](int c, int p, const double *u) {
    const fxs_class &C = S->C[c];
    if (members[c].empty()) {
      hipLaunchKernelGGL(k_fxs_extract_sym, dim3(fxs_row_grid(p + 1)), dim3(PMH_BLOCK), 0, S->ctx->stream, p, (const int *)C.d_urel, u, fxs_super_band(S, C, p));
      return;
    }
    for (const auto &rg : members[c].at(p)) {
      const int r = rg.first, g = rg.second;
      hipLaunchKernelGGL(k_fxs_extract_symg, dim3(fxs_row_grid(C.nc)), dim3(PMH_BLOCK), 0, S->ctx->stream, r, C.nc, (double)C.h_sign[(size_t)g * C.nc + p], (const int *)C.d_urel, u,
                         (const int *)(C.d_posmap + (size_t)g * C.nc), (const signed char *)(C.d_sign + (size_t)g * C.nc), fxs_super_band(S, C, r));
    }
  };
  P.check_row = [S](int c, int r, const double *u, double *d_out) {
    const fxs_class &C = S->C[c];
    hipLaunchKernelGGL(k_fxs_check_row, dim3(fxs_row_grid(r + 1)), dim3(PMH_BLOCK), 0, S->ctx->stream, r, (const int *)C.d_urel, u, (const double *)fxs_super_band(S, C, r), d_out);
    return fxs_row_grid(r + 1);
  };
}

static void fxs_plan_orbit(fx_shared *S, fx_asm_plan &P)
{
  for (int c = 0; c < S->ncls; c++) {
    const fxs_class &C = S->C[c];
    if (!C.nc) continue;
    for (int pl = 0; pl < C.m1 - C.m0; pl++) P.todo[c].push_back({C.urel[C.reps[C.m0 + pl]], pl});
    for (int r = 0; r < C.nc; r++)
      if (C.op_of[r] != 0) {
        const int k = (int)(std::lower_bound(C.reps.begin(), C.reps.end(), C.rep_of[r]) - C.reps.begin());
        if (k >= C.m0 && k < C.m1) P.check[c].push_back({C.urel[r], r});
      }
  }
  P.write     = [S](int c, int pl, const double *u) { fxo_store_row(S, S->C[c], S->C[c].reprow[pl], S->C[c].d_urel, u); };
  P.check_row = [S](int c, int r, const double *u, double *d_out) {
    const fxs_class &C = S->C[c];
    const int        g = C.op_of[r], p = C.rep_of[r], pl = (int)(std::lower_bound(C.reps.begin(), C.reps.end(), p) - C.reps.begin()) - C.m0;
    hipLaunchKernelGGL(k_fxo_check_row, dim3(fxs_row_grid(C.nc)), dim3(PMH_BLOCK), 0, S->ctx->stream, C.reprow[pl], C.tm, C.nc, C.nkc, (double)C.h_sign[(size_t)g * C.nc + p], (const int *)C.d_urel,
                       (const int *)C.d_kinv, u, (const int *)(C.d_posmap + (size_t)g * C.nc), (const signed char *)(C.d_sign + (size_t)g * C.nc), (const double *)(S->Afund + C.aoff), d_out);
    return fxs_row_grid(C.nc);
  };
}

int fxs_assemble(fx_shared *S, pmh_matinv solver, int nslots, const int *slot_class, double rtol, int max_it, long long *n_solves, fx_batch_window *w)
{
  PMH_ARG(S && solver && nslots >= 1 && (solver->nblocks == nslots || solver->nblocks * PMH_MV_R == nslots) && slot_class);
  if (S->sym == 2) PMH_CHK(fxo_prepare(S));
  fx_asm_plan P(S->ncls);
  for (int c = 0; c < S->ncls; c++)
    if (S->C[c].nc) P.nloc[c] = S->C[c].nloc;
  if (S->sym == 2) fxs_plan_orbit(S, P);
  else if (S->sym) fxs_plan_tiles(S, P);
  else fxs_plan_full(S, P);
  PMH_CHK(fx_assemble_run(S->ctx, P, solver, nslots, slot_class, rtol, max_it, n_solves, w));
  if (S->sym == 2 && (!w || w->complete)) return fxa_setup(S);
  return PMH_SUCCESS;
}

static int fxs_gemm(fx_shared *S)
{
  if (S->sym == 2 && !S->fxo_ready) return pmh_set_error(PMH_ERR_STATE, "PMH_FX_CLASS_ORBIT: apply before the assembly");
  if (!S->nwg) return PMH_SUCCESS;
  hipStream_t st    = S->ctx->stream;
  const bool  timed = S->ev_on && (size_t)(2 * S->ev_used + 2) <= S->ev.size();
  if (timed) PMH_HIP(hipEventRecord(S->ev[2 * S->ev_used], st));
  const long long stride = std::max(16LL, S->nX);
  if (S->sym == 2) {
    S->ev_mid_pending = timed ? S->ev_used : -1;
    if (fxa_active(S)) PMH_CHK(fxa_launch(S));
    else PMH_CHK(fxo_gemm(S));
    S->ev_mid_pending = -1;
  } else if (S->sym) {
    hipLaunchKernelGGL(k_fxs_symm8, dim3(S->nwg), dim3(FXM_THREADS), 0, st, (const int *)S->d_wg, (const int *)S->d_items, (const long long *)S->d_wgl, (const int *)S->d_ld, (const long long *)S->d_xoff,
                       (const double *)S->Wbase, (const double *)S->X, S->part, stride, S->pt);
    for (auto &C : S->C)
      hipLaunchKernelGGL(k_fxs_symfin, dim3((unsigned)(((long long)C.ld * FXS_S / 2 * 8 + PMH_BLOCK - 1) / PMH_BLOCK), C.ngroups), dim3(PMH_BLOCK), 0, st, C.ld, C.nmb, C.nown, (const int *)C.d_nseg, (const int *)C.d_ownfirst,
                         (const long long *)C.d_ptoff, C.xoff, stride, (const double *)S->part, (const double *)S->pt, S->Y);
  } else {
  hipLaunchKernelGGL(k_fxs_gemm8, dim3(S->nwg), dim3(PMH_BLOCK), 0, st, (const int *)S->d_wg, (const int *)S->d_ld, (const long long *)S->d_woff, (const long long *)S->d_xoff, (const double *)S->Wbase,
                     (const double *)S->X, S->part, stride);
  hipLaunchKernelGGL(k_fxs_fin, dim3((unsigned)((S->nX / 2 + PMH_BLOCK - 1) / PMH_BLOCK)), dim3(PMH_BLOCK), 0, st, S->nX, S->nseg, stride, (const double *)S->part, S->Y);
  }
  if (timed) {
    PMH_HIP(hipEventRecord(S->ev[2 * S->ev_used + 1], st));
    S->ev_used++;
  }
  PMH_HIP(hipGetLastError());
  return PMH_SUCCESS;
}

int fxs_apply(fx_shared *S, const double *lambda, double *y)
{
  if (S->sym == 2) PMH_CHK(pmh_gluing_mult(S->Bc2, lambda, S->X2));
  else PMH_CHK(pmh_gluing_mult(S->Bc, lambda, S->X));
  PMH_CHK(fxs_gemm(S));
  return pmh_gluing_mult_transpose(S->Bc, S->Y, y);
}

int fxs_stages(fx_shared *S, pmh_csr *gather, double **mid_in, pmh_csr *scatter, const double **mid_out)
{
  if (S->sym == 2) *gather = S->Bc2->Bt, *mid_in = S->X2;
  else *gather = S->Bc->Bt, *mid_in = S->X;
  *scatter = S->Bc->B, *mid_out = S->Y;
  return PMH_SUCCESS;
}
int fxs_mid(fx_shared *S) { return fxs_gemm(S); }

int fxs_dense(fx_shared *S)
{
  if (S->sym == 2 && S->nX > 0) {
    for (const fxs_class &C : S->C) {
      const long long n = (long long)C.ngroups * C.ld * C.S;
      if (!n) continue;
      hipLaunchKernelGGL(k_fxo_signed_copy, dim3((unsigned)std::min<long long>(4096, (n + PMH_BLOCK - 1) / PMH_BLOCK)), dim3(PMH_BLOCK), 0, S->ctx->stream, n, C.S, (const double *)(S->X + C.xoff), S->X2 + 2 * C.xoff);
    }
    PMH_HIP(hipGetLastError());
  }
  return fxs_gemm(S);
}
long long fxs_multivector_length(fx_shared *S) { return S->nX; }
double   *fxs_X(fx_shared *S) { return S->X; }
double   *fxs_Y(fx_shared *S) { return S->Y; }

int fxs_fill_pattern(fx_shared *S, int byte)
{
  if (S->sym == 2) {
    PMH_CHK(fxo_prepare(S));
    PMH_HIP(hipMemsetAsync(S->Afund, byte, sizeof(double) * (size_t)S->afund_tot, S->ctx->stream));
    return pmh_sync(S->ctx);
  }
  PMH_HIP(hipMemsetAsync(S->Wbase, byte, sizeof(double) * (size_t)S->wtot, S->ctx->stream));
  return pmh_sync(S->ctx);
}

int fxs_get_block(fx_shared *S, int b, int n, const int *gamma, double *out_host)
{
  const fxs_class    &C = S->C[S->cls[b]];
  if (S->sym == 2) {
    if (!S->fxo_ready || C.m0 != 0 || C.m1 != C.M_all) return pmh_set_error(PMH_ERR_STATE, "pmh_fexplicit_get_block: the orbit storage holds only this rank's representatives");
    std::vector<double> T((size_t)C.Mp * C.ldk), row((size_t)C.nc);
    PMH_HIP(hipMemcpy(T.data(), S->Afund + C.aoff, sizeof(double) * T.size(), hipMemcpyDeviceToHost));
    for (int i = 0; i < n; i++) {
      const int r = C.pos[gamma[i] - S->K->rowstart[b]], p = C.rep_of[r], g = C.op_of[r], pl = (int)(std::lower_bound(C.reps.begin(), C.reps.end(), p) - C.reps.begin());
      const double  sp = (double)C.h_sign[(size_t)g * C.nc + p];
      const int     pr = C.reprow[pl];
      const double *ab = T.data() + (size_t)(pr / C.tm) * C.nkc * (FXO_TK * C.tm) + pr % C.tm;
      for (int cc = 0; cc < C.nc; cc++) {
        const int k = C.kinv[cc];
        row[C.h_posmap[(size_t)g * C.nc + cc]] = sp * (double)C.h_sign[(size_t)g * C.nc + cc] * ab[(size_t)(k / FXO_TK) * (FXO_TK * C.tm) + (k % FXO_TK) * C.tm];
      }
      for (int k = 0; k < n; k++) out_host[(size_t)i * n + k] = row[C.pos[gamma[k] - S->K->rowstart[b]]];
    }
    return PMH_SUCCESS;
  }
  if (S->sym) {
    const long long     len = (long long)FXM_RS * FXM_RS * ((long long)C.nsb * (C.nsb + 1) / 2);
    std::vector<double> T((size_t)len);
    PMH_HIP(hipMemcpy(T.data(), S->Wbase + C.woff, sizeof(double) * (size_t)len, hipMemcpyDeviceToHost));
    auto at = [&](int p, int c) {
      const int hi = std::max(p, c), lo = std::min(p, c), sb = hi / FXM_RS, Il = (hi % FXM_RS) / 16, r = hi & 15, q = r >> 2, l = 16 * (r & 3) + (lo & 15);
      const double v = T[(size_t)((long long)FXM_RS * FXM_RS * ((long long)sb * (sb + 1) / 2) + ((long long)(lo >> 4) * FXM_RT + Il) * 256 + (q >> 1) * 128 + 2 * l + (q & 1))];
      return hi == lo ? 2.0 * v : v;
    };
    for (int i = 0; i < n; i++)
      for (int k = 0; k < n; k++) out_host[(size_t)i * n + k] = at(C.pos[gamma[i] - S->K->rowstart[b]], C.pos[gamma[k] - S->K->rowstart[b]]);
    return PMH_SUCCESS;
  }
  std::vector<double> row((size_t)std::max(1, C.ld));
  for (int i = 0; i < n; i++) {
    const int p = C.pos[gamma[i] - S->K->rowstart[b]];
    PMH_HIP(hipMemcpy(row.data(), S->Wbase + C.woff + (long long)p * C.ld, sizeof(double) * (size_t)C.ld, hipMemcpyDeviceToHost));
    for (int k = 0; k < n; k++) out_host[(size_t)i * n + k] = row[C.pos[gamma[k] - S->K->rowstart[b]]];
  }
  return PMH_SUCCESS;
}

int fxs_test_load_class(fx_shared *S, int c, const double *W, int *all_loaded)
{
  PMH_ARG(S && W && all_loaded && c >= 0 && c < S->ncls);
  if (S->sym != 2) return pmh_set_error(PMH_ERR_ARG, "pmh_fexplicit_test_load_class: needs the PMH_FX_CLASS_ORBIT storage");
  pmh_ctx    ctx = S->ctx;
  if (!S->fxo_ready)
    for (fxs_class &D : S->C) D.test_loaded = 0;
  PMH_CHK(fxo_prepare(S));
  fxs_class &C = S->C[c];
  const int  M = C.m1 - C.m0;
  if (C.nc) {
    std::vector<double> rows((size_t)M * C.nc);
    std::vector<int>    ident((size_t)C.nc);
    for (int pl = 0; pl < M; pl++) memcpy(&rows[(size_t)pl * C.nc], W + (size_t)C.reps[C.m0 + pl] * C.nc, sizeof(double) * (size_t)C.nc);
    for (int i = 0; i < C.nc; i++) ident[i] = i;
    double *d_rows = nullptr;
    int    *d_ident = nullptr;
    PMH_CHK(pmh_malloc(ctx, sizeof(double) * rows.size(), (void **)&d_rows));
    int rc = pmh_malloc(ctx, sizeof(int) * ident.size(), (void **)&d_ident);
    if (!rc) rc = pmh_memcpy_h2d(ctx, d_rows, rows.data(), sizeof(double) * rows.size());
    if (!rc) rc = pmh_memcpy_h2d(ctx, d_ident, ident.data(), sizeof(int) * ident.size());
    for (int pl = 0; pl < M && !rc; pl++)
      fxo_store_row(S, C, C.reprow[pl], d_ident, d_rows + (size_t)pl * C.nc);
    if (!rc && hipGetLastError() != hipSuccess) rc = pmh_set_error(PMH_ERR_HIP, "pmh_fexplicit_test_load_class: launch failed");
// ... 105 lines not shown
```

permon_amd/csrc/fshared_adapted.h:

```cpp
#pragma once
#include "fshared_kernels.h"

#define FXA_CB 64
#define FXA_LDT 49

__host__ __device__ __forceinline__ long long fxa_xh_off(const fxa_irrep &I, int r, int n) { return I.hoff + ((((long long)(n >> 4) * I.nks + (r >> 3)) * 64 + (r & 3) * 16 + (n & 15)) << 1) + ((r >> 2) & 1); }
__device__ __forceinline__ long long fxa_wh_off(const fxa_irrep &I, int r, int c) { return I.woff + ((((long long)(r >> 4) * I.nks + (c >> 3)) * 64 + (c & 3) * 16 + (r & 15)) << 1) + ((c >> 2) & 1); }

template <bool INV>
__global__ __launch_bounds__(PMH_BLOCK) void k_fxa_transform(const fxa_irrep *__restrict__ ir, const double *__restrict__ tab, const long long *__restrict__ toff, const int *__restrict__ osize,
                                                             const int *__restrict__ tbase, const int *__restrict__ opos, const int *__restrict__ rowinfo, int NC, int nc, int ld, long long xbase0,
                                                             const double *__restrict__ X2, double *__restrict__ Xh, const double *__restrict__ Yh, double *__restrict__ Y,
                                                             const char *__restrict__ tmask)
{
  __shared__ double Ts[48 * FXA_LDT];
  __shared__ double vs[48 * FXA_CB];
  const int o = blockIdx.x, no = osize[o], tb = tbase[o], c0 = blockIdx.y * FXA_CB, ncb = min(FXA_CB, NC - c0);
  const double *__restrict__ T = tab + toff[o];
  for (int e = threadIdx.x; e < 48 * 48; e += PMH_BLOCK) {
    const int t = e / 48, j = e % 48;
    Ts[INV ? j * FXA_LDT + t : t * FXA_LDT + j] = T[e];
  }
  for (int e = threadIdx.x; e < ((no + 3) & ~3) * ncb; e += PMH_BLOCK) {
    const int b = e / ncb, cl = e % ncb, col = c0 + cl;
    if (b >= no) vs[b * FXA_CB + cl] = 0.0;
    else if (INV) {
      const int       ri = rowinfo[tb + b];
      const fxa_irrep I  = ir[ri & 15];
      vs[b * FXA_CB + cl] = Yh[I.yoff + (long long)(ri >> 8) * I.ldy + ((ri >> 4) & 3) * NC + col];
    } else
      vs[b * FXA_CB + cl] = X2[2 * (xbase0 + (long long)(col >> 3) * ld * FXS_S + (long long)opos[tb + b] * FXS_S) + (col & 7)];
  }
  __syncthreads();
  for (int e = threadIdx.x; e < no * ncb; e += PMH_BLOCK) {
    const int a = e / ncb, cl = e % ncb, col = c0 + cl;
    double s0 = 0.0, s1 = 0.0, s2 = 0.0, s3 = 0.0;
    for (int b = 0; b < no; b += 4) {
      s0 = FXS_MAD(Ts[a * FXA_LDT + b], vs[b * FXA_CB + cl], s0), s1 = FXS_MAD(Ts[a * FXA_LDT + b + 1], vs[(b + 1) * FXA_CB + cl], s1);
      s2 = FXS_MAD(Ts[a * FXA_LDT + b + 2], vs[(b + 2) * FXA_CB + cl], s2), s3 = FXS_MAD(Ts[a * FXA_LDT + b + 3], vs[(b + 3) * FXA_CB + cl], s3);
    }
    const double s = (s0 + s1) + (s2 + s3);
    if (INV) {
      const int pos = opos[tb + a], g = col >> 3, sl = col & 7;
      if (tmask[((long long)g * nc + pos) * FXS_S + sl]) Y[xbase0 + (long long)g * ld * FXS_S + (long long)pos * FXS_S + sl] = s;
    } else {
      const int       ri = rowinfo[tb + a];
      const fxa_irrep I  = ir[ri & 15];
      Xh[fxa_xh_off(I, ri >> 8, ((ri >> 4) & 3) * NC + col)] = s;
    }
  }
}

#define FXN_NC 16
#define FXN_T (48 * FXS_S / 2)
__host__ __device__ __forceinline__ int fxn_tab_off(int a, int j) { return ((((a >> 4) * 24 + (j >> 1)) * 16 + (a & 15)) << 1) + (j & 1); }

template <bool INV>
__global__ __launch_bounds__(FXN_T) void k_fxa_narrow(const double *__restrict__ tab, const int *__restrict__ osize, const int *__restrict__ rec, const long long *__restrict__ recl, int norb,
                                                      long long gstride, const double *__restrict__ src, double *__restrict__ dst)
{
  __shared__ dbl2 vs[FXN_T];
  const int  o = blockIdx.x, g = blockIdx.y, a = threadIdx.x >> 2, sl = 2 * (threadIdx.x & 3), no = osize[o];
  const bool live = a < no;
  int        r  = 0;
  long long  rl = 0;
  dbl2       v  = dbl2{0.0, 0.0}, t[24];
#pragma unroll
  for (int k = 0; k < 24; k++) t[k] = dbl2{0.0, 0.0};
  if (live) {
    const long long f = ((long long)g * norb + o) * 48 + a;
    r = rec[INV ? f : o * 48 + a], rl = recl[f];
    const dbl2 *__restrict__ row = (const dbl2 *)(tab + (long long)o * 48 * 48 + fxn_tab_off(a, 0));
#pragma unroll
    for (int k = 0; k < 24; k++)
      if (2 * k < no) t[k] = row[16 * k];
    v = *(const dbl2 *)(INV ? src + rl + sl : src + (long long)g * gstride + r + sl);
  }
  vs[threadIdx.x] = v;
  __syncthreads();
  if (!live) return;
  dbl2 s0 = dbl2{0.0, 0.0}, s1 = s0, s2 = s0, s3 = s0;
#pragma unroll
  for (int k = 0; k < 12; k++)
    if (4 * k < no) {
      const dbl2 *x = vs + 4 * k * (FXS_S / 2) + (threadIdx.x & 3);
      const dbl2  x0 = x[0], x1 = x[FXS_S / 2], x2 = x[2 * (FXS_S / 2)], x3 = x[3 * (FXS_S / 2)];
      s0.x = FXS_MAD(t[2 * k].x, x0.x, s0.x), s1.x = FXS_MAD(t[2 * k].y, x1.x, s1.x), s2.x = FXS_MAD(t[2 * k + 1].x, x2.x, s2.x), s3.x = FXS_MAD(t[2 * k + 1].y, x3.x, s3.x);
      s0.y = FXS_MAD(t[2 * k].x, x0.y, s0.y), s1.y = FXS_MAD(t[2 * k].y, x1.y, s1.y), s2.y = FXS_MAD(t[2 * k + 1].x, x2.y, s2.y), s3.y = FXS_MAD(t[2 * k + 1].y, x3.y, s3.y);
    }
  const double sx = (s0.x + s1.x) + (s2.x + s3.x), sy = (s0.y + s1.y) + (s2.y + s3.y);
  if (INV) {
    double *__restrict__ y = dst + (long long)g * gstride + (long long)(r >> 8) * FXS_S + sl;
    if ((r >> sl) & 1) y[0] = sx;
    if ((r >> sl) & 2) y[1] = sy;
  } else
    dst[rl + 2 * sl] = sx, dst[rl + 2 * sl + 2] = sy;
}

template <bool TOYH>
__global__ __launch_bounds__(PMH_BLOCK) void k_fxa_logical(const fxa_irrep *__restrict__ ir, const int *__restrict__ rowinfo, int nc, int NC, const double *__restrict__ in, double *__restrict__ out)
{
  const long long e = (long long)blockIdx.x * PMH_BLOCK + threadIdx.x;
  if (e >= (long long)nc * NC) return;
  const int       ri = rowinfo[e / NC], col = (int)(e % NC), n = ((ri >> 4) & 3) * NC + col;
  const fxa_irrep I  = ir[ri & 15];
  if (TOYH) out[I.yoff + (long long)(ri >> 8) * I.ldy + n] = in[e];
  else out[e] = in[fxa_xh_off(I, ri >> 8, n)];
}

template <int NBW, int U>
__device__ __forceinline__ void fxa_prod_rows(const fxa_irrep &I, int ob, int nb0, const double *__restrict__ Wh, const double *__restrict__ Xh, double *__restrict__ Yh, int lane, int wave,
                                              double (*red)[16 * 64])
{
  const dbl2 *__restrict__ w = (const dbl2 *)(Wh + I.woff + (long long)ob * I.nks * 128) + lane;
  const dbl2 *__restrict__ x = (const dbl2 *)(Xh + I.hoff + (long long)nb0 * I.nks * 128) + lane;
  dbl4 acc[NBW];
#pragma unroll
  for (int j = 0; j < NBW; j++) acc[j] = dbl4{0.0, 0.0, 0.0, 0.0};
  const int ks1 = fxa_wave_k0(I.nks, U, wave + 1);
  for (int ks = fxa_wave_k0(I.nks, U, wave); ks < ks1; ks += U) {
    dbl2 a[U], b[U][NBW];
#pragma unroll
    for (int u = 0; u < U; u++) a[u] = w[(long long)(ks + u) * 64];
#pragma unroll
    for (int u = 0; u < U; u++)
#pragma unroll
      for (int j = 0; j < NBW; j++) b[u][j] = x[((long long)j * I.nks + ks + u) * 64];
#pragma unroll
    for (int u = 0; u < U; u++) {
#pragma unroll
      for (int j = 0; j < NBW; j++) acc[j] = __builtin_amdgcn_mfma_f64_16x16x4f64(a[u].x, b[u][j].x, acc[j], 0, 0, 0);
#pragma unroll
      for (int j = 0; j < NBW; j++) acc[j] = __builtin_amdgcn_mfma_f64_16x16x4f64(a[u].y, b[u][j].y, acc[j], 0, 0, 0);
    }
  }
  if (wave > 0) {
#pragma unroll
    for (int j = 0; j < NBW; j++)
#pragma unroll
      for (int r = 0; r < 4; r++) red[wave - 1][(4 * j + r) * 64 + lane] = acc[j][r];
  }
  __syncthreads();
  if (wave > 0) return;
#pragma unroll
  for (int v = 0; v < FXA_WAVES - 1; v++)
#pragma unroll
    for (int j = 0; j < NBW; j++)
#pragma unroll
      for (int r = 0; r < 4; r++) acc[j][r] += red[v][(4 * j + r) * 64 + lane];
  double *__restrict__ y = Yh + I.yoff + (long long)(ob * 16 + (lane >> 4)) * I.ldy + nb0 * 16 + (lane & 15);
#pragma unroll
  for (int j = 0; j < NBW; j++)
#pragma unroll
    for (int r = 0; r < 4; r++) y[(long long)(4 * r) * I.ldy + j * 16] = acc[j][r];
}

__global__ __launch_bounds__(64 * FXA_WAVES) void k_fxa_prod(const int *__restrict__ items, const fxa_irrep *__restrict__ ir, const double *__restrict__ Wh, const double *__restrict__ Xh,
                                                              double *__restrict__ Yh)
{
  __shared__ double red[FXA_WAVES - 1][16 * 64];
  const int *it = items + 4 * blockIdx.x;
  const int  lane = threadIdx.x & 63, wave = __builtin_amdgcn_readfirstlane(threadIdx.x >> 6);
  const fxa_irrep I = ir[__builtin_amdgcn_readfirstlane(it[0])];
  const int  ob = __builtin_amdgcn_readfirstlane(it[1]), nb0 = __builtin_amdgcn_readfirstlane(it[2]), nbw = __builtin_amdgcn_readfirstlane(it[3]);
  switch (nbw) {
  case 1: fxa_prod_rows<1, fxa_trip_steps(1)>(I, ob, nb0, Wh, Xh, Yh, lane, wave, red); break;
  case 2: fxa_prod_rows<2, fxa_trip_steps(2)>(I, ob, nb0, Wh, Xh, Yh, lane, wave, red); break;
  case 3: fxa_prod_rows<3, fxa_trip_steps(3)>(I, ob, nb0, Wh, Xh, Yh, lane, wave, red); break;
  default: fxa_prod_rows<4, fxa_trip_steps(4)>(I, ob, nb0, Wh, Xh, Yh, lane, wave, red); break;
  }
}

__global__ __launch_bounds__(PMH_BLOCK) void k_fxa_stab_avg(int nh, const int *__restrict__ hops, int p, int pr, int tm, int nc, int nkc, const int *__restrict__ posmap, const signed char *__restrict__ sign,
                                                             const int *__restrict__ kinv, const double *__restrict__ A, double *__restrict__ tmp)
{
  const double *__restrict__ arow = A + (long long)(pr / tm) * nkc * (FXO_TK * tm) + pr % tm;
  for (int c = blockIdx.x * PMH_BLOCK + threadIdx.x; c < nc; c += gridDim.x * PMH_BLOCK) {
    double s = 0.0;
    for (int h = 0; h < nh; h++) {
// ... 46 lines not shown
```

permon_amd/csrc/fshared_types.h:

```cpp
#pragma once
#include <algorithm>
#include <chrono>
#include <map>
#include <cmath>

#include "feti_internal.h"
#include "fshared.h"
#include "pmh_internal.h"
#include "reduce.h"

typedef double dbl2 __attribute__((ext_vector_type(2)));

#define FXS_S 8
#define FXS_PAD 128

struct fxa_irrep {
  int       d, m, nks, nob, nbt, ldy;
  long long woff, hoff, yoff;
};
#define FXA_WAVES 4
#define FXA_KU 8
__host__ __device__ constexpr int fxa_trip_steps(int nbw) { return nbw <= 2 ? FXA_KU : FXA_KU / 2; }
__host__ __device__ inline int fxa_wave_k0(int nks, int U, int wave) { return U * ((nks / U) * wave / FXA_WAVES); }

struct fxa_class {
  int        norb = 0, NC = 0, nitems = 0, nc = 0;
  fxa_irrep  ir[10];
  fxa_irrep *d_ir = nullptr;
  double    *d_tab = nullptr, *Wh = nullptr, *Xh = nullptr, *Yh = nullptr;
  long long *d_toff = nullptr;
  int       *d_osize = nullptr, *d_tbase = nullptr, *d_opos = nullptr, *d_rowinfo = nullptr, *d_items = nullptr;
  char      *d_tmask = nullptr;
  int        narrow = 0;
  double    *d_tabN = nullptr, *d_tabNT = nullptr;
  int       *d_nfx = nullptr, *d_nyd = nullptr;
  long long *d_nxh = nullptr, *d_nyh = nullptr;
  double     flops = 0.0, flops_issued = 0.0, bytes = 0.0;
  int        items_of_width[10][4] = {};
};

struct fxs_class {
  std::vector<int> h_ops;
  fxa_class       *oa = nullptr;
  std::vector<int> blocks;
  std::vector<int> urel;
  std::vector<int> pos;
  int              nloc = 0, nc = 0, ld = 0, ngroups = 0, r0 = 0, r1 = 0;
  long long        woff = 0, xoff = 0;
  int             *d_urel = nullptr;
  int              nsb = 0, nmb = 0;
  std::vector<char> own;
  long long        ptoff = 0, ptsize = 0;
  std::vector<long long> ptm;
  int             *d_nseg = nullptr;
  long long       *d_ptoff = nullptr;
  int             *d_ownfirst = nullptr, nown = 0;
  int                      nsym = 0;
  std::vector<int>         h_posmap;
  std::vector<signed char> h_sign;
  int                     *d_posmap = nullptr;
  signed char             *d_sign = nullptr;
  std::vector<int> reps, rep_of, op_of;
  int              M_all = 0, m0 = 0, m1 = 0, Mp = 0, ldk = 0, nkc = 0, nsymp = 0, tm = 128, tnw = 0;
  long long        aoff = 0, coff = 0;
  int             *d_gidx = nullptr, *d_reppos = nullptr;
  std::vector<char> tmask;
  char             *d_tmask = nullptr;
  std::vector<int>  reprow;
  int              *d_coltab = nullptr, *d_fintab = nullptr;
  long long        *d_finbase = nullptr;
  int               item_first = 0, item_count = 0, fin_elems = 0, wgf_first = 0, wg_count = 0;
  int               tn = 128;
  int               S = 8;
  signed char     *d_use = nullptr;
  std::vector<int> kinv;
  int             *d_kinv = nullptr, *d_unittab = nullptr, *d_lut = nullptr;
  int              nseg = 1;
  int              plan_units = 0, plan_units_work = 0, plan_smax = 0, plan_wg2 = 0, test_loaded = 0;
};

struct fx_shared {
  pmh_ctx                ctx;
  pmh_gluing             B;
  pmh_blockdiag          K;
  int                    nb, ncls;
  std::vector<int>       cls;
  std::vector<fxs_class> C;
  pmh_gluing             Bc = nullptr;
  pmh_gluing             Bc2 = nullptr;
  double                *X2  = nullptr;
  double                *Wbase = nullptr, *X = nullptr, *Y = nullptr;
  long long              nX = 0, wtot = 0;
  int                   *d_wg = nullptr;
  int                    nwg = 0, nseg = 0;
  double                *part = nullptr;
  long long              part_cap = 0;
  int                   *d_ld = nullptr;
  long long             *d_woff = nullptr, *d_xoff = nullptr;
  double                 bytes = 0.0;
  std::vector<hipEvent_t> ev;
  int                    ev_used = 0, ev_on = 0;
  std::vector<hipEvent_t> ev_mid;
  int                    ev_mid_pending = -1;
  int                    sym = 0, segj = 0;
  long long             *d_wgl = nullptr;
  int                   *d_items = nullptr, *d_wgfirst = nullptr;
  int                   *d_wgfirst_all = nullptr, *d_zrow_of = nullptr, nwg_all = 0, merged_tm = 0, merged_tn = 128, merged_tnw = 0;
  const int            **d_coltab_of = nullptr, **d_gidx_of = nullptr;
  void                  *d_fin_args = nullptr;
  int                    fin_nbx = 0, fin_ngroups = 0;
  double                *pt = nullptr;
  long long              pt_tot = 0;
  double                 owned_bytes = 0.0;
  double                *Afund = nullptr, *cpart = nullptr;
  long long              afund_tot = 0, cpart_cap = 0;
  int                    fxo_ready = 0, fxo_S = 1, stripe_rank = 0, stripe_size = 0;
  double                 flops = 0.0, flops_issued = 0.0, flops_dense = 0.0;
};

#define FXO_TM 128
#define FXO_TN 128
#define FXO_TK 16

struct fxo_fin_args {
  int              ntile, tm, nsymp, nc, ld, nslot, nbx, ngroups;
  const int       *fintab, *unittab, *lut, *coltab, *reppos, *posmap;
  const long long *unitbase;
  const signed char *use;
  const char      *tmask;
  long long        xbase0;
};

int  fxo_row_tile(int M);
int  fxo_prepare(fx_shared *S);
```

permon_amd/csrc/pmh_internal.h:

```cpp
#pragma once
#include <hip/hip_runtime.h>
#include <rccl/rccl.h>

#include <cstdarg>
#include <cstdio>
#include <cstdlib>
#include <cstring>
#include <vector>

#include "permon_hip.h"

#define PMH_BLOCK 256
#define PMH_MAX_VEC_BLOCKS 2048
#define PMH_MAX_RED 8
#define PMH_NSCAL 64

int pmh_set_error(int code, const char *fmt, ...);

struct pmh_knobs_s {
  int chain;
  int chain_applies = 0, chain_launches = 0;
  int chain_replay = 1, chain_replays = 0, chain_replays_redone = 0;
  int gt_fusion = 1;
  int smalxe_prefetch = 1;
  int vec_epi = 1;
  int orbit_adapted = 1, orbit_adapted_classes = 0, orbit_adapted_fallbacks = 0, orbit_adapted_spoil = 0;
  int orbit_narrow = 1;
  int mpgp_spec = 1;
  int mg_d0_fusion = 1;
  int kplus_mv = 1;
  int multi_rhs = 1;
  int svm_pairing = 1;
  int host_threads = 1;
};
pmh_knobs_s &pmh_knobs();
inline int   pmh_host_threads() { return pmh_knobs().host_threads > 1 ? pmh_knobs().host_threads : 1; }

#define PMH_HIP(call) \
  do { \
    hipError_t e_ = (call); \
    if (e_ != hipSuccess) return pmh_set_error(PMH_ERR_HIP, "%s:%d %s -> %s", __FILE__, __LINE__, #call, hipGetErrorString(e_)); \
  } while (0)
#define PMH_CHK(call) \
  do { \
    int rc_ = (call); \
    if (rc_) return rc_; \
  } while (0)
#define PMH_NCCL(call) \
  do { \
    ncclResult_t r_ = (call); \
    if (r_ != ncclSuccess) return pmh_set_error(PMH_ERR_COMM, "%s:%d %s -> %s", __FILE__, __LINE__, #call, ncclGetErrorString(r_)); \
  } while (0)
#define PMH_ARG(cond) \
  do { \
    if (!(cond)) return pmh_set_error(PMH_ERR_ARG, "%s:%d argument check failed: %s", __FILE__, __LINE__, #cond); \
  } while (0)

struct pmh_ctx_s {
  int         device;
  int         num_cus;
  hipStream_t stream;
  hipEvent_t  ev0, ev1;
  double     *d_partials;
  int         partials_cap;
  double     *d_scal;
  double     *h_scal;
  double     *h_partials;
  ncclComm_t comm;
  int        rank, size, force_comm;
  double    *d_commbuf;
  int        dist_scalars;
  unsigned long long free_epoch = 0;
  pmh_comm_host_fn hook      = nullptr;
  void            *hook_user = nullptr;
  double          *h_stage   = nullptr;
  size_t           stage_cap = 0;
  hipEvent_t *comm_ev      = nullptr;
  int         comm_ev_cap = 0, comm_ev_used = 0;
  double      comm_ev_bytes = 0.0;
};
static inline bool pmh_comm_on(pmh_ctx c) { return (c->comm || c->hook) && (c->size > 1 || c->force_comm); }
int pmh_comm_allreduce_scalars(pmh_ctx c, double *dscal, int K, const int *ops );
int pmh_comm_sum_host(pmh_ctx c, double *h, int k);

enum { PMH_SPMV_ELL = 0, PMH_SPMV_STREAM = 1, PMH_SPMV_MEDIUM = 2, PMH_SPMV_VECTOR = 3, PMH_SPMV_LONG = 4 };
struct pmh_csr_s {
  pmh_ctx   ctx;
  int       nrows, ncols;
  long long nnz;
  int      *d_rowptr, *d_col;
  double   *d_val;
  int       plan;
  int       width;
  int      *d_rowblocks;
  unsigned short *d_col16;
  int      *d_cbase;
  double         *d_ell_val;
  unsigned short *d_ell_c16;
  int            *d_ell_col;
  int            *d_ell_cbase;
  int             ell_nrb;
  int       n_rowblocks;
  double   *d_blockpart;
  int       n_launch_blocks;
  pmh_csr   transpose;
  const int    *h_rowptr, *h_col;
  const double *h_val;
  unsigned long long uid = 0;
  int           congruent_nrep = 0;
  int      *d_lchunks, *d_lrow;
  double   *d_lpart;
  double   *d_lpart2;
  int       l_nchunks;
  std::vector<hipEvent_t> *ev;
  std::vector<int>        *ev_kind;
  int                      ev_used, ev_pending;
};
int pmh_csr_row_lanes(pmh_csr A);

enum { PMH_EPI_NONE = 0, PMH_EPI_ADD = 1, PMH_EPI_SUB = 2, PMH_EPI_MPGP = 3 };
struct pmh_spmv_epi {
  int           kind;
  const double *y1;
  const double *g, *xx, *lb, *ub;
  int           scal_base;
  const int    *halt;
};
int pmh_csr_spmv_launch(pmh_csr A, const double *x, double *y, const pmh_spmv_epi &epi);
int pmh_csr_adopt_transpose(pmh_csr A, pmh_csr At);
inline void pmh_csr_set_host_hint(pmh_csr A, const int *rowptr, const int *col, const double *val) { A->h_rowptr = rowptr, A->h_col = col, A->h_val = val; }
int pmh_csr_mult_partials(pmh_csr A, const double *x, const int **lrow, const double **part);
int pmh_csr_mult_partials2(pmh_csr A, const double *x, const double *x2, const int **lrow, const double **part, const double **part2);
int pmh_csr_mult_then_dense(pmh_csr A, const double *x, const double *Mt, double *tmp, double *y, int norm_slot = -1);

#define PMH_EPI_UNSUPPORTED (-77)
enum { PMH_VEPI_P1 = 1, PMH_VEPI_GRAD_SPLIT = 2 };
struct pmh_vec_epi {
  int           kind;
  const double *g, *xx, *lb, *ub, *b;
  double        astol;
  double       *gf, *p;
  double       *partials;
  int           ld, prow;
  int           p_fresh, x_from_spec;
  double        spec_alpha;
  double       *x_out;
  int           in_slot, same_input;
  double       *h_partials;
  int          *hosted, *emitted_p, *replayed;
};
struct pmh_emit_tab {
  const int    *seg;
  const int    *gcol;
  const double *gval;
  const int    *lrow;
  int           m, nwg;
};
struct pmh_emit_out {
  double *part;
};
struct pmh_emit_args {
  pmh_emit_tab tab;
  pmh_emit_out o[2];
};

struct pmh_op_s {
  pmh_ctx ctx;
  int     n;
  virtual ~pmh_op_s() {}
  virtual int     mult(const double *x, double *y) = 0;
  virtual int     mult_epi(const double *, double *, const pmh_vec_epi &) { return PMH_EPI_UNSUPPORTED; }
  virtual int     mult_same_input(const double *x, double *y, int *  = nullptr) { return mult(x, y); }
  virtual int     emit_begin(const double * , const double * , pmh_emit_args *) { return PMH_EPI_UNSUPPORTED; }
  virtual void    emit_invalidate(bool  = false) {}
  virtual int     spec_expansion_ready() { return 0; }
  virtual int     mult_transpose(const double *, double *) { return pmh_set_error(PMH_ERR_SUP, "this operator has no MatMultTranspose slot"); }
  virtual pmh_csr as_csr() { return nullptr; }
  virtual int     maxeig_start(double * ) { return PMH_EPI_UNSUPPORTED; }
  virtual int     stages(pmh_csr * , double ** , pmh_csr * , const double ** ) { return PMH_EPI_UNSUPPORTED; }
  virtual int     mid_apply() { return pmh_set_error(PMH_ERR_SUP, "this operator has no middle stage"); }
};

struct pmh_qppf_s {
  pmh_ctx ctx;
  pmh_csr G;
  int     m, n;
  int     orthonormal;
  double *d_inv;
  int     implicit_orth;
  double *d_Tt, *d_S, *tmp_m;
  std::vector<double> h_T;
  double *G_left, *Gt_right;
  double  ggt_mfma_ms, host_inverse_ms;
  int           onerow = 0;
  const double *row = nullptr;
  double        row_aat = 0.0;
  double       *or_part = nullptr, *or_s = nullptr;
};

int pmh_onerow_dot(pmh_qppf pf, const double *v, double coef, double *out);
int pmh_onerow_scaled_row(pmh_qppf pf, const double *s, double coef, const double *v , double *y);

enum { PMH_RED_SUM = 0, PMH_RED_MIN = 1 };
int pmh_finalize_partials(pmh_ctx ctx, const double *partials, int ld, int nblocks, int K, const int *ops, int scal_base, const int *halt = nullptr, int *post_inc = nullptr);
int pmh_finalize_partials_slots(pmh_ctx ctx, const double *partials, int ld, int nblocks, int K, const int *ops, const int *slots);
int pmh_vec_grid(int n);

int pmh_qpc_box_project_flag(pmh_ctx ctx, int n, const double *x, const double *lb, const double *ub, double *Px, int slot);
int pmh_k_dot_partials(pmh_ctx ctx, int n, const double *x, const double *y, int slot);
int pmh_qppf_apply_G_norm2(pmh_qppf pf, const double *v, double *Gv, int slot);
int pmh_mpgp_set_pre_test_hook(pmh_mpgp s, int (*f)(void *), void *user);
int pmh_mpgp_set_convergence_margin(pmh_mpgp s, double margin);
int pmh_mpgp_set_gradient_valid(pmh_mpgp s, int valid, double **g);
int pmh_mpgp_x_applied(pmh_mpgp s);
int pmh_mpgp_set_first_operand_applied(pmh_mpgp s, int on);
int pmh_mpgp_set_pre_p1_hook(pmh_mpgp s, int (*f)(void *), void *user);
int pmh_op_penalized_arm_aux_normG(pmh_op op, const double *u, double *Gu, int slot);
enum { PMH_PEN_FOLD = 0, PMH_PEN_CHAIN = 1, PMH_PEN_ONE_LAUNCH = 2, PMH_PEN_TEN_LAUNCH = 3, PMH_PEN_DENSE_INVERSE = 4, PMH_PEN_PLAIN = 5 };
int pmh_op_penalized_take_aux_done(pmh_op op);
int pmh_op_penalized_set_normG_target(pmh_op op, double *Gu, int slot);
int pmh_op_penalized_normG_ready(pmh_op op, const double *u);
int pmh_op_penalized_chain_launches(pmh_op op);
#define PMH_SLOT_NORMBU2 48
#define PMH_SLOT_PROJ_CHANGED 52
#define PMH_SLOT_TEST_SPMV 56
int pmh_host_scalar(pmh_ctx ctx, int slot, double *v);

struct pmh_bsr3_s {
  pmh_ctx   ctx;
  int       n, nbr, ntiles, storage, tb;
  int       nrep, rep_rows;
  long long nblocks, npad;
  double    scale;
  int      *d_tile_br, *d_browptr, *d_bcol;
  long long *d_tile_off;
  void     *d_val;
  std::vector<hipEvent_t> ev;
  std::vector<double>     ev_extra;
  int                     ev_used, ev_on, ev_seen, ev_stride;
};
typedef pmh_bsr3_s *pmh_bsr3;
enum { PMH_BSR_F64 = 0, PMH_BSR_F32 = 1, PMH_BSR_F16 = 2 };
enum { PMH_BSR_EPI_PRE = 10, PMH_BSR_EPI_POST1 = 11, PMH_BSR_EPI_POST2 = 12 };
template <typename T> struct pmh_bsr3_epi {
  const T *y1;
  const T *dinv;
  T       *r, *d;
  double  *z64;
  T        c0, c1, c2;
};
int    pmh_bsr3_from_csr(pmh_csr A, int storage, pmh_bsr3 *out, int tile = 0, int nrep_hint = 1);
int    pmh_bsr3_destroy(pmh_bsr3 B);
double pmh_bsr3_bytes(pmh_bsr3 B);
double pmh_bsr3_bytes_blockdiag(pmh_bsr3 B);
int    pmh_bsr3_replicas(pmh_bsr3 B);
int    pmh_bsr3_spmv_f64(pmh_bsr3 B, const double *x, double *y, int epi, const double *y1, const int *halt);
int    pmh_bsr3_spmv_f32(pmh_bsr3 B, const float *x, float *y, int epi, const float *y1, const int *halt);
int    pmh_bsr3_spmv_epi_f64(pmh_bsr3 B, const double *x, double *y, int epi, const pmh_bsr3_epi<double> &e, const int *halt);
int    pmh_bsr3_spmv_epi_f32(pmh_bsr3 B, const float *x, float *y, int epi, const pmh_bsr3_epi<float> &e, const int *halt);
int    pmh_bsr3_timing_enable(pmh_bsr3 B, int max_launches);
int    pmh_bsr3_timing_get(pmh_bsr3 B, int *launches, double *total_ms, double *epilogue_bytes = nullptr);
int    pmh_csr_ensure_transpose(pmh_csr A);

// ... 3 lines not shown
```

Measured before the change: 4848 QPS iterations/s.

## Fuse dual-chain gather into the orbit-adapted forward transform kernel

```diff
diff --git a/permon_amd/csrc/ctx.hip b/permon_amd/csrc/ctx.hip
--- a/permon_amd/csrc/ctx.hip
+++ b/permon_amd/csrc/ctx.hip
@@ -57,6 +57,8 @@
   if (!strcmp(name, "chain_replay")) return &pmh_knobs().chain_replay;
   if (!strcmp(name, "chain_replays")) return &pmh_knobs().chain_replays;
   if (!strcmp(name, "chain_replays_redone")) return &pmh_knobs().chain_replays_redone;
+  if (!strcmp(name, "chain_gather_fused")) return &pmh_knobs().chain_gather_fused;
+  if (!strcmp(name, "chain_gather_fused_last")) return &pmh_knobs().chain_gather_fused_last;
   if (!strcmp(name, "host_threads")) return &pmh_knobs().host_threads;
   if (!strcmp(name, "svm_pairing")) return &pmh_knobs().svm_pairing;
   if (!strcmp(name, "gt_fusion")) return &pmh_knobs().gt_fusion;
diff --git a/permon_amd/csrc/dualchain.hip b/permon_amd/csrc/dualchain.hip
--- a/permon_amd/csrc/dualchain.hip
+++ b/permon_amd/csrc/dualchain.hip
@@ -23,6 +23,9 @@
   double  *zeroed   = nullptr;
   int      nlist = 0, *d_reci = nullptr;
   double  *d_recd = nullptr;
+  std::vector<int>    h_reci;
+  std::vector<double> h_recd;
+  bool     mid_in_written = true;
   pmh_csr  sc_for = nullptr;
   int     *d_sc2 = nullptr;
   double  *d_sv2 = nullptr;
@@ -67,24 +70,6 @@
     if (lane < m) y2[lane] = y;
     const double sq = pmh_wave_all<PMH_RED_SUM>(lane < m ? y * y : 0.0);
     if (lane == 0) *norm_d = sq, *norm_h = sq;
-  }
-}
-
-template <int W>
-static __device__ __forceinline__ void dc_gt_load(const double *__restrict__ ev, const unsigned char *__restrict__ ec, int j, double (&v)[W],
-                        unsigned char (&c)[W])
-{
-  typedef double dbl2 __attribute__((ext_vector_type(2)));
-#pragma unroll
-  for (int e = 0; e < W; e += 2) {
-    const dbl2 d = *(const dbl2 *)(ev + (size_t)j * W + e);
-    v[e] = d.x, v[e + 1] = d.y;
-  }
-#pragma unroll
-  for (int h = 0; h < W / 8; h++) {
-    const unsigned long long cc = *(const unsigned long long *)(ec + (size_t)j * W + 8 * h);
-#pragma unroll
-    for (int e = 0; e < 8; e++) c[8 * h + e] = (unsigned char)(cc >> (8 * e));
   }
 }
 
@@ -432,6 +417,7 @@
     PMH_CHK(pmh_memcpy_h2d(ctx, dc->d_recd, recd.data(), sizeof(double) * recd.size()));
     PMH_CHK(pmh_memset(ctx, dc->mid_in, 0, sizeof(double) * (size_t)Bg->nrows));
     dc->nlist = (int)(reci.size() / 8), dc->list_for = Bg, dc->list_uid = Bg->uid, dc->zeroed = dc->mid_in;
+    dc->h_reci.swap(reci), dc->h_recd.swap(recd);
   }
   if (dc->sc_for != dc->scatter || dc->sc_uid != dc->scatter->uid) {
     const pmh_csr       Bs = dc->scatter;
@@ -600,15 +586,28 @@
       na.part = dc->part[0], na.Tt = dc->pf->d_Tt, na.y2 = dc->normGu, na.norm_d = ctx->d_scal + dc->norm_slot, na.norm_h = ctx->h_scal + dc->norm_slot;
       dc->norm_done = true, dc->norm_ptr = dc->x_emitted;
     }
-    const dim3 ggrid((unsigned)(std::max(1, (dc->nlist + PMH_EMIT_TILE - 1) / PMH_EMIT_TILE) + (na.part ? 1 : 0)));
-    dc_dispatch(dc, [&](auto W, auto NU) {
-      hipLaunchKernelGGL(HIP_KERNEL_NAME(k_dc_gather<decltype(W)::value, decltype(NU)::value>), ggrid, eblk, 0, st, dc->nlist, (const int *)dc->d_reci, (const double *)dc->d_recd,
-                         (const int *)Bg->d_col, (const double *)Bg->d_val, (const double *)dc->d_ev, (const unsigned char *)dc->d_ec, tab, (const double *)dc->part[slot],
-                         (const double *)dc->pf->d_S, dc->c_cur, na, x, dc->mid_in);
-    });
+    bool fused = false;
+    if (pmh_knobs().chain_gather_fused) {
+      pmh_gather_fused_args ga;
+      ga.x = x, ga.part = dc->part[slot], ga.tab = tab, ga.nseg = dc->nseg, ga.W = dc->W, ga.NU = dc_nu(dc), ga.S = dc->pf->d_S, ga.ev = dc->d_ev, ga.ec = dc->d_ec, ga.c_out = dc->c_cur;
+      ga.norm_part = na.part, ga.Tt = na.Tt, ga.y2 = na.y2, ga.norm_d = na.norm_d, ga.norm_h = na.norm_h;
+      ga.gather = Bg, ga.gather_uid = Bg->uid, ga.nlist = dc->nlist, ga.h_reci = dc->h_reci.data(), ga.h_recd = dc->h_recd.data();
+      const int rc = dc->F->gather_fused(ga);
+      if (rc != PMH_SUCCESS && rc != PMH_EPI_UNSUPPORTED) return rc;
+      fused = rc == PMH_SUCCESS;
+    }
+    if (!fused) {
+      const dim3 ggrid((unsigned)(std::max(1, (dc->nlist + PMH_EMIT_TILE - 1) / PMH_EMIT_TILE) + (na.part ? 1 : 0)));
+      dc_dispatch(dc, [&](auto W, auto NU) {
+        hipLaunchKernelGGL(HIP_KERNEL_NAME(k_dc_gather<decltype(W)::value, decltype(NU)::value>), ggrid, eblk, 0, st, dc->nlist, (const int *)dc->d_reci, (const double *)dc->d_recd,
+                           (const int *)Bg->d_col, (const double *)Bg->d_val, (const double *)dc->d_ev, (const unsigned char *)dc->d_ec, tab, (const double *)dc->part[slot],
+                           (const double *)dc->pf->d_S, dc->c_cur, na, x, dc->mid_in);
+      });
+      PMH_HIP(hipGetLastError());
+    }
     dc->launches++;
-  }
-  PMH_HIP(hipGetLastError());
+    dc->mid_in_written = !fused, pmh_knobs().chain_gather_fused_last = fused;
+  }
   PMH_CHK(dc->F->mid_apply());
   hipLaunchKernelGGL(k_dc_scatter, vgrid, eblk, 0, st, n, (const unsigned char *)dc->d_scnt, (const int *)dc->d_sc2, (const double *)dc->d_sv2, (const int *)Bs->d_rowptr, (const int *)Bs->d_col,
                      (const double *)Bs->d_val, dc->mid_out, dc->w, dc_emit_args(dc, dc->w + n, nullptr));
@@ -681,6 +680,7 @@
   PMH_ARG(host && len && what >= 0 && what <= 10);
   PMH_ARG(what < 4 || what > 6 || what == 6 || (dc->gather && dc->scatter));
   PMH_ARG((what != 7 && what != 8) || dc->normGu);
+  if (what == 4 && !dc->mid_in_written) return pmh_set_error(PMH_ERR_SUP, "pmh_dc_test_read: the last application's gather ran inside the operator's forward transform: mid_in was not written");
   pmh_ctx       ctx = dc->ctx;
   const int     m = dc->m;
   const double *src[11] = {dc->part[0], dc->part[1], dc->part[2], dc->c_cur, dc->mid_in, dc->mid_out, dc->w, dc->normGu, nullptr, dc->pf->d_S, dc->pf->d_Tt};
diff --git a/permon_amd/csrc/emit_inline.h b/permon_amd/csrc/emit_inline.h
--- a/permon_amd/csrc/emit_inline.h
+++ b/permon_amd/csrc/emit_inline.h
@@ -118,6 +118,24 @@
   }
 }
 
+template <int W>
+static __device__ __forceinline__ void dc_gt_load(const double *__restrict__ ev, const unsigned char *__restrict__ ec, int j, double (&v)[W],
+                        unsigned char (&c)[W])
+{
+  typedef double dbl2 __attribute__((ext_vector_type(2)));
+#pragma unroll
+  for (int e = 0; e < W; e += 2) {
+    const dbl2 d = *(const dbl2 *)(ev + (size_t)j * W + e);
+    v[e] = d.x, v[e + 1] = d.y;
+  }
+#pragma unroll
+  for (int h = 0; h < W / 8; h++) {
+    const unsigned long long cc = *(const unsigned long long *)(ec + (size_t)j * W + 8 * h);
+#pragma unroll
+    for (int e = 0; e < 8; e++) c[8 * h + e] = (unsigned char)(cc >> (8 * e));
+  }
+}
+
 template <int RPW, int NU = 8>
 static __device__ __forceinline__ void pmh_coarse_share(const pmh_emit_tab &tab, const double *__restrict__ part, const double *__restrict__ M1,
                         const double *__restrict__ M2, double *a_out,
diff --git a/permon_amd/csrc/feti.hip b/permon_amd/csrc/feti.hip
--- a/permon_amd/csrc/feti.hip
+++ b/permon_amd/csrc/feti.hip
@@ -833,6 +833,10 @@
     if (Kplus->E && pmh_fexplicit_matches(Kplus->E, B)) return pmh_fexplicit_stages(Kplus->E, gather, mid_in, scatter, mid_out);
     *gather = B->Bt, *mid_in = t1, *scatter = B->B, *mid_out = t2;
     return PMH_SUCCESS;
+  }
+  int gather_fused(const pmh_gather_fused_args &g) override
+  {
+    return (Kplus->E && pmh_fexplicit_matches(Kplus->E, B)) ? pmh_fexplicit_gather_fused(Kplus->E, g) : PMH_EPI_UNSUPPORTED;
   }
   int mid_apply() override
   {
diff --git a/permon_amd/csrc/feti_internal.h b/permon_amd/csrc/feti_internal.h
--- a/permon_amd/csrc/feti_internal.h
+++ b/permon_amd/csrc/feti_internal.h
@@ -53,6 +53,7 @@
 bool pmh_fexplicit_matches(pmh_fexplicit_s *E, pmh_gluing B);
 int  pmh_fexplicit_apply(pmh_fexplicit_s *E, const double *lambda, double *y);
 int  pmh_fexplicit_stages(pmh_fexplicit_s *E, pmh_csr *gather, double **mid_in, pmh_csr *scatter, const double **mid_out);
+int  pmh_fexplicit_gather_fused(pmh_fexplicit_s *E, const pmh_gather_fused_args &g);
 int  pmh_fexplicit_mid(pmh_fexplicit_s *E);
 int  pmh_fexplicit_store_symmetrized(pmh_fexplicit_s *E, int b, const double *S, int lds);
 int  pmh_fexplicit_mark_assembled(pmh_fexplicit_s *E, long long n_solves, double seconds);
diff --git a/permon_amd/csrc/fexplicit.hip b/permon_amd/csrc/fexplicit.hip
--- a/permon_amd/csrc/fexplicit.hip
+++ b/permon_amd/csrc/fexplicit.hip
@@ -1064,6 +1064,7 @@
   return PMH_SUCCESS;
 }
 int pmh_fexplicit_mid(pmh_fexplicit_s *E) { return E->sh ? fxs_mid(E->sh) : fx_gemv(E); }
+int pmh_fexplicit_gather_fused(pmh_fexplicit_s *E, const pmh_gather_fused_args &g) { return E->sh ? fxs_gather_fused(E->sh, g) : PMH_EPI_UNSUPPORTED; }
 
 extern "C" int pmh_fexplicit_mult(pmh_fexplicit E, const double *lambda, double *y)
 {
diff --git a/permon_amd/csrc/fshared.h b/permon_amd/csrc/fshared.h
--- a/permon_amd/csrc/fshared.h
+++ b/permon_amd/csrc/fshared.h
@@ -18,6 +18,7 @@
 int       fxs_dense(fx_shared *S);
 int       fxs_stages(fx_shared *S, pmh_csr *gather, double **mid_in, pmh_csr *scatter, const double **mid_out);
 int       fxs_mid(fx_shared *S);
+int       fxs_gather_fused(fx_shared *S, const pmh_gather_fused_args &g);
 long long fxs_multivector_length(fx_shared *S);
 double   *fxs_X(fx_shared *S);
 double   *fxs_Y(fx_shared *S);
diff --git a/permon_amd/csrc/fshared.hip b/permon_amd/csrc/fshared.hip
--- a/permon_amd/csrc/fshared.hip
+++ b/permon_amd/csrc/fshared.hip
@@ -267,7 +267,7 @@
   if (!a) return;
   if (a->Wh) (void)hipFree(a->Wh);
   for (void *q : {(void *)a->d_ir, (void *)a->d_tab, (void *)a->Xh, (void *)a->Yh, (void *)a->d_toff, (void *)a->d_osize, (void *)a->d_tbase, (void *)a->d_opos, (void *)a->d_rowinfo, (void *)a->d_items,
-                  (void *)a->d_tmask, (void *)a->d_tabN, (void *)a->d_tabNT, (void *)a->d_nfx, (void *)a->d_nyd, (void *)a->d_nxh, (void *)a->d_nyh})
+                  (void *)a->d_tmask, (void *)a->d_tabN, (void *)a->d_tabNT, (void *)a->d_nfx, (void *)a->d_nyd, (void *)a->d_nxh, (void *)a->d_nyh, (void *)a->d_gri, (void *)a->d_grd})
     if (q) pmh_free(ctx, q);
   delete a;
   C.oa = nullptr;
@@ -379,14 +379,14 @@
   if (!fxa_active(S)) return;
   *issued = 0.0;
   for (const fxs_class &C : S->C)
-    if (C.oa) *issued += C.oa->flops_issued;
+    if (C.oa) *issued += C.oa->flops_issued + (S->last_fused ? C.oa->fused_flops : 0.0);
 }
 double fxs_apply_bytes(fx_shared *S)
 {
   if (!fxa_active(S)) return S->bytes;
   double b = 0.0;
   for (const fxs_class &C : S->C)
-    if (C.oa) b += C.oa->bytes;
+    if (C.oa) b += C.oa->bytes + (S->last_fused ? C.oa->fused_bytes : 0.0);
   return b;
 }
 
@@ -590,11 +590,11 @@
                        (const int *)a->d_opos, (const int *)a->d_rowinfo, a->NC, C.nc, C.ld, C.xoff, (const double *)S->X2, a->Xh, (const double *)a->Yh, S->Y, (const char *)a->d_tmask);
 }
 
-static int fxa_launch(fx_shared *S)
+static int fxa_launch(fx_shared *S, bool skip_forward = false)
 {
   hipStream_t st = S->ctx->stream;
   for (fxs_class &C : S->C)
-    if (C.oa) fxa_launch_transform(S, C, false);
+    if (C.oa && !skip_forward) fxa_launch_transform(S, C, false);
   for (fxs_class &C : S->C)
     if (fxa_class *a = C.oa)
       if (a->nitems) hipLaunchKernelGGL(k_fxa_prod, dim3(a->nitems), dim3(64 * FXA_WAVES), 0, st, (const int *)a->d_items, (const fxa_irrep *)a->d_ir, (const double *)a->Wh, (const double *)a->Xh, a->Yh);
@@ -792,6 +792,7 @@
 {
   pmh_ctx ctx = S->ctx;
   for (fxs_class &C : S->C) fxa_free(ctx, C);
+  S->grec_for = nullptr, S->grec_ok = 0, S->fwd_fused = 0;
   if (!pmh_knobs().orbit_adapted || S->stripe_size > 1 || ctx->size > 1) return PMH_SUCCESS;
   for (char **e = environ; e && *e; e++)
     if (!strncmp(*e, "PMH_FXO_", 8)) return PMH_SUCCESS;
@@ -958,17 +959,20 @@
   return PMH_SUCCESS;
 }
 
-static int fxs_gemm(fx_shared *S)
-{
+static int fxs_gemm(fx_shared *S, bool fwd_done = false)
+{
+  S->fwd_fused = 0;
   if (S->sym == 2 && !S->fxo_ready) return pmh_set_error(PMH_ERR_STATE, "PMH_FX_CLASS_ORBIT: apply before the assembly");
   if (!S->nwg) return PMH_SUCCESS;
   hipStream_t st    = S->ctx->stream;
-  const bool  timed = S->ev_on && (size_t)(2 * S->ev_used + 2) <= S->ev.size();
-  if (timed) PMH_HIP(hipEventRecord(S->ev[2 * S->ev_used], st));
+  const bool  timed = fwd_done ? S->fwd_timed != 0 : S->ev_on && (size_t)(2 * S->ev_used + 2) <= S->ev.size();
+  if (timed && !fwd_done) PMH_HIP(hipEventRecord(S->ev[2 * S->ev_used], st));
+  S->last_fused = fwd_done;
   const long long stride = std::max(16LL, S->nX);
   if (S->sym == 2) {
     S->ev_mid_pending = timed ? S->ev_used : -1;
-    if (fxa_active(S)) PMH_CHK(fxa_launch(S));
+    if (fxa_active(S)) PMH_CHK(fxa_launch(S, fwd_done));
+    else if (fwd_done) return pmh_set_error(PMH_ERR_STATE, "PMH_FX_CLASS_ORBIT: the fused gather ran for a class that is not in the symmetry-adapted form");
     else PMH_CHK(fxo_gemm(S));
     S->ev_mid_pending = -1;
   } else if (S->sym) {
@@ -992,6 +996,7 @@
 
 int fxs_apply(fx_shared *S, const double *lambda, double *y)
 {
+  S->fwd_fused = 0;
   if (S->sym == 2) PMH_CHK(pmh_gluing_mult(S->Bc2, lambda, S->X2));
   else PMH_CHK(pmh_gluing_mult(S->Bc, lambda, S->X));
   PMH_CHK(fxs_gemm(S));
@@ -1000,12 +1005,114 @@
 
 int fxs_stages(fx_shared *S, pmh_csr *gather, double **mid_in, pmh_csr *scatter, const double **mid_out)
 {
+  S->fwd_fused = 0;
   if (S->sym == 2) *gather = S->Bc2->Bt, *mid_in = S->X2;
   else *gather = S->Bc->Bt, *mid_in = S->X;
   *scatter = S->Bc->B, *mid_out = S->Y;
   return PMH_SUCCESS;
 }
-int fxs_mid(fx_shared *S) { return fxs_gemm(S); }
+int fxs_mid(fx_shared *S)
+{
+  const bool fwd_done = S->fwd_fused != 0;
+  S->fwd_fused        = 0;
+  return fxs_gemm(S, fwd_done);
+}
+
+static int fxs_gather_records(fx_shared *S, const pmh_gather_fused_args &g)
+{
+  pmh_ctx ctx = S->ctx;
+  S->grec_for = g.gather, S->grec_uid = g.gather_uid, S->grec_ok = 0;
+  for (fxs_class &C : S->C)
+    if (fxa_class *a = C.oa) {
+      if (a->d_gri) PMH_CHK(pmh_free(ctx, a->d_gri));
+      if (a->d_grd) PMH_CHK(pmh_free(ctx, a->d_grd));
+      a->d_gri = nullptr, a->d_grd = nullptr;
+    }
+  const long long  nrows = 2 * S->nX;
+  if (g.gather->nrows < nrows || g.tab.m > 64) return PMH_SUCCESS;
+  std::vector<int> where((size_t)std::max(1LL, nrows), -1);
+  long long        nplus = 0, found = 0;
+  for (int i = 0; i < g.nlist; i++) {
+    const int r = g.h_reci[(size_t)8 * i], r2 = g.h_reci[(size_t)8 * i + 1], cnt = g.h_reci[(size_t)8 * i + 3] - g.h_reci[(size_t)8 * i + 2];
+    if (r < 0 || r >= nrows || r2 >= nrows || cnt < 1 || cnt > 0x7ff) return PMH_SUCCESS;
+    for (int u = 0; u < 3 && u < cnt; u++)
+      if (g.h_reci[(size_t)8 * i + 4 + u] < 0 || g.h_reci[(size_t)8 * i + 4 + u] > 0xfffff) return PMH_SUCCESS;
+    where[r] = 2 * i, nplus += (r & 15) < FXS_S;
+    if (r2 >= 0) where[r2] = 2 * i + 1, nplus += (r2 & 15) < FXS_S;
+  }
+  for (fxs_class &C : S->C) {
+    if (!C.nc) continue;
+    fxa_class *a = C.oa;
+    if (!a || !a->narrow || C.S != FXS_S || (C.xoff & 7)) return PMH_SUCCESS;
+    std::vector<int> osize((size_t)a->norb), nfx((size_t)a->norb * 48);
+    PMH_CHK(pmh_memcpy_d2h(ctx, osize.data(), a->d_osize, sizeof(int) * osize.size()));
+    PMH_CHK(pmh_memcpy_d2h(ctx, nfx.data(), a->d_nfx, sizeof(int) * nfx.size()));
+    const size_t          nrec = (size_t)C.ngroups * a->norb * 48 * FXS_S;
+    std::vector<fxg_int4> gri(nrec, fxg_int4{0, 0, 0, 0});
+    std::vector<double>   grd(4 * nrec, 0.0);
+    double                entries = 0.0;
+    const double          live = (double)C.ngroups * C.nc * FXS_S;
+    for (int gr = 0; gr < C.ngroups; gr++)
+      for (int o = 0; o < a->norb; o++)
+        for (int t = 0; t < osize[o]; t++)
+          for (int sl = 0; sl < FXS_S; sl++) {
+            const long long row = 2 * C.xoff + (long long)gr * 2 * C.ld * FXS_S + nfx[(size_t)o * 48 + t] + sl;
+            if (row < 0 || row >= nrows || where[(size_t)row] < 0) continue;
+            const int    i = where[(size_t)row] >> 1, neg = where[(size_t)row] & 1;
+            const int   *ri = g.h_reci + (size_t)8 * i;
+            const size_t f = (((size_t)gr * a->norb + o) * 48 + t) * FXS_S + sl;
+            gri[f] = fxg_int4{(int)((unsigned)ri[4] | (unsigned)(ri[3] - ri[2]) << 20 | (unsigned)neg << 31), ri[5], ri[6], ri[2]};
+            for (int u = 0; u < 3; u++) grd[4 * f + u] = g.h_recd[(size_t)4 * i + u];
+            found++, entries += ri[3] - ri[2];
+          }
+    PMH_CHK(fxa_upload(ctx, gri, &a->d_gri));
+    PMH_CHK(fxa_upload(ctx, grd, &a->d_grd));
+    const double nwgs = (double)a->norb * C.ngroups;
+    double       tab_delta = 0.0;
+    for (int o = 0; o < a->norb; o++) tab_delta += 8.0 * (48.0 - osize[o]) * ((osize[o] + 3) & ~3) * C.ngroups;
+    a->fused_bytes = 48.0 * live - 4.0 * C.nc * C.ngroups - 8.0 * (double)C.nc * a->NC + entries * (8.0 + 9.0 * g.W) + nwgs * 8.0 * ((double)g.tab.m * g.tab.m + g.nseg) + tab_delta;
+    a->fused_flops = entries * (2.0 * g.W + 3.0) + nwgs * (2.0 * (double)g.tab.m * g.tab.m + g.nseg);
+  }
+  S->grec_ok = found == nplus;
+  return PMH_SUCCESS;
+}
+
+int fxs_gather_fused(fx_shared *S, const pmh_gather_fused_args &g)
+{
+  S->fwd_fused = 0;
+  if (S->sym != 2 || !S->fxo_ready || !S->nwg || S->stripe_size > 1 || S->ctx->size > 1 || !fxa_active(S) || !S->Bc2 || g.gather != S->Bc2->Bt) return PMH_EPI_UNSUPPORTED;
+  if ((g.W != 8 && g.W != 16) || (g.NU != 2 && g.NU != 8)) return PMH_EPI_UNSUPPORTED;
+  for (const fxs_class &C : S->C)
+    if (C.nc && !(C.oa && C.oa->narrow)) return PMH_EPI_UNSUPPORTED;
+  if (S->grec_for != g.gather || S->grec_uid != g.gather_uid) PMH_CHK(fxs_gather_records(S, g));
+  if (!S->grec_ok) return PMH_EPI_UNSUPPORTED;
+  void (*kern)(const fxg_args) = g.W == 8 ? (g.NU == 2 ? k_fxa_gather<8, 2> : k_fxa_gather<8, 8>) : (g.NU == 2 ? k_fxa_gather<16, 2> : k_fxa_gather<16, 8>);
+  {
+    static int per_cu[4] = {-1, -1, -1, -1};
+    int       &pc        = per_cu[(g.W == 16) * 2 + (g.NU == 8)];
+    if (pc < 0) PMH_HIP(hipOccupancyMaxActiveBlocksPerMultiprocessor(&pc, kern, FXN_T, 0));
+    for (const fxs_class &C : S->C)
+      if (C.oa && C.nc && (long long)(C.oa->norb + 1) * C.ngroups > (long long)pc * S->ctx->num_cus) return PMH_EPI_UNSUPPORTED;
+  }
+  hipStream_t st    = S->ctx->stream;
+  const bool  timed = S->ev_on && (size_t)(2 * S->ev_used + 2) <= S->ev.size();
+  if (timed) PMH_HIP(hipEventRecord(S->ev[2 * S->ev_used], st));
+  bool first = true;
+  for (fxs_class &C : S->C) {
+    fxa_class *a = C.oa;
+    if (!a || !C.nc) continue;
+    fxg_args A;
+    A.tab = a->d_tabN, A.osize = a->d_osize, A.recl = a->d_nxh, A.norb = a->norb, A.gri = (const int *)a->d_gri, A.grd = a->d_grd;
+    A.bcol = g.gather->d_col, A.bval = g.gather->d_val, A.ev = g.ev, A.ec = g.ec, A.ctab = g.tab, A.part = g.part, A.S = g.S, A.c_out = g.c_out;
+    A.norm_part = first ? g.norm_part : nullptr, A.Tt = g.Tt, A.y2 = g.y2, A.norm_d = g.norm_d, A.norm_h = g.norm_h, A.x = g.x, A.Xh = a->Xh;
+    const dim3 grid(a->norb + (A.norm_part ? 1 : 0), C.ngroups), block(FXN_T);
+    hipLaunchKernelGGL(kern, grid, block, 0, st, A);
+    first = false;
+  }
+  PMH_HIP(hipGetLastError());
+  S->fwd_fused = 1, S->fwd_timed = timed;
+  return PMH_SUCCESS;
+}
 
 int fxs_dense(fx_shared *S)
 {
@@ -1017,6 +1124,7 @@
     }
     PMH_HIP(hipGetLastError());
   }
+  S->fwd_fused = 0;
   return fxs_gemm(S);
 }
 long long fxs_multivector_length(fx_shared *S) { return S->nX; }
diff --git a/permon_amd/csrc/fshared_adapted.h b/permon_amd/csrc/fshared_adapted.h
--- a/permon_amd/csrc/fshared_adapted.h
+++ b/permon_amd/csrc/fshared_adapted.h
@@ -95,6 +95,198 @@
     if ((r >> sl) & 2) y[1] = sy;
   } else
     dst[rl + 2 * sl] = sx, dst[rl + 2 * sl + 2] = sy;
+}
+
+#include "emit_inline.h"
+struct fxg_args {
+  const double *tab;
+  const int    *osize;
+  const long long *recl;
+  int           norb;
+  const int    *gri;
+  const double *grd;
+  const int    *bcol;
+  const double *bval;
+  const double *ev;
+  const unsigned char *ec;
+  pmh_emit_tab  ctab;
+  const double *part, *S;
+  double       *c_out;
+  const double *norm_part, *Tt;
+  double       *y2, *norm_d, *norm_h;
+  const double *x;
+  double       *Xh;
+};
+
+template <int NU>
+static __device__ __forceinline__ void fxg_coarse_shares(const pmh_emit_tab &tab, const double *__restrict__ part, const double *__restrict__ M1, double (*ps)[64], int lane, int wave)
+{
+  static_assert(FXN_T == 192, "three waves share the 16 virtual waves");
+  const int m   = tab.m;
+  const int lr0 = lane <= m ? tab.lrow[lane] : 0, lr1 = lane < m ? tab.lrow[lane + 1] : 0;
+#pragma unroll
+  for (int i = 0; i < 6; i++) {
+    const int v = wave + 3 * i;
+    if (v >= PMH_EMIT_NW) continue;
+    double pv[4][NU], m1[4];
+#pragma unroll
+    for (int q = 0; q < 4; q++) {
+      const int  r  = v + PMH_EMIT_NW * q;
+      const bool in = r < m;
+      const int  c0 = in ? __builtin_amdgcn_readlane(lr0, r) : 0, c1 = in ? __builtin_amdgcn_readlane(lr1, r) : 0;
+#pragma unroll
+      for (int u = 0; u < NU; u++) {
+        const int c = c0 + lane + 64 * u;
+        pv[q][u]    = (c < c1) ? part[c] : 0.0;
+      }
+      m1[q] = (in && lane < m) ? M1[(size_t)r * m + lane] : 0.0;
+    }
+    double s1 = 0.0;
+#pragma unroll
+    for (int q = 0; q < 4; q++) {
+      const int r = v + PMH_EMIT_NW * q;
+      if (r >= m) break;
+      double acc = 0.0;
+#pragma unroll
+      for (int u = 0; u < NU; u++) acc += pv[q][u];
+      acc = pmh_wave_all<PMH_RED_SUM>(acc);
+      s1 += m1[q] * acc;
+    }
+    ps[v][lane] = s1;
+  }
+}
+
+template <int W> struct fxg_row {
+  int           cnt, neg, j[3], k0;
+  double        bv[3], xv[3], v0[W];
+  unsigned char c0[W];
+};
+template <int W>
+static __device__ __forceinline__ void fxg_row_load(fxg_row<W> &R, const fxg_int4 w, const dbl2 da, const dbl2 db, const fxg_args &A)
+{
+  R.cnt = (w.x >> 20) & 0x7ff, R.neg = w.x < 0, R.j[0] = w.x & 0xfffff, R.j[1] = w.y, R.j[2] = w.z, R.k0 = w.w;
+  R.bv[0] = da.x, R.bv[1] = da.y, R.bv[2] = db.x;
+#pragma unroll
+  for (int u = 0; u < 3; u++) R.xv[u] = (u < R.cnt) ? A.x[R.j[u]] : 0.0;
+#pragma unroll
+  for (int e = 0; e < W; e++) R.v0[e] = 0.0, R.c0[e] = 0;
+  if (R.cnt > 0) dc_gt_load<W>(A.ev, A.ec, R.j[0], R.v0, R.c0);
+}
+template <int W>
+static __device__ __forceinline__ double fxg_row_sum(const fxg_row<W> &R, const double *cs, const fxg_args &A)
+{
+  if (R.cnt == 0) return 0.0;
+  double sum = 0.0;
+  {
+    double q = 0.0;
+#pragma unroll
+    for (int e = 0; e < W; e++) q += R.v0[e] * cs[R.c0[e]];
+    sum += R.bv[0] * (-1.0 * q + R.xv[0]);
+  }
+#pragma unroll
+  for (int u = 1; u < 3; u++)
+    if (u < R.cnt) {
+      double        vv[W];
+      unsigned char cc[W];
+      dc_gt_load<W>(A.ev, A.ec, R.j[u], vv, cc);
+      double q = 0.0;
+#pragma unroll
+      for (int e = 0; e < W; e++) q += vv[e] * cs[cc[e]];
+      sum += R.bv[u] * (-1.0 * q + R.xv[u]);
+    }
+  for (int k = R.k0 + 3; k < R.k0 + R.cnt; k++) {
+    const int     jj = A.bcol[k];
+    double        vv[W];
+    unsigned char cc[W];
+    dc_gt_load<W>(A.ev, A.ec, jj, vv, cc);
+    double q = 0.0;
+#pragma unroll
+    for (int e = 0; e < W; e++) q += vv[e] * cs[cc[e]];
+    sum += A.bval[k] * (-1.0 * q + A.x[jj]);
+  }
+  return R.neg ? -sum : sum;
+}
+
+#ifdef FXA_TAB_NT
+#define FXA_TAB_LOAD(p) __builtin_nontemporal_load(p)
+#else
+#define FXA_TAB_LOAD(p) (*(p))
+#endif
+
+template <int W, int NU>
+__global__ __launch_bounds__(FXN_T) void k_fxa_gather(const fxg_args A)
+{
+  __shared__ dbl2   ts[48 * 24];
+  __shared__ dbl2   vs[FXN_T];
+  __shared__ double cs[64], ps[PMH_EMIT_NW][64];
+  const int t = threadIdx.x, lane = t & 63, wave = __builtin_amdgcn_readfirstlane(t >> 6), o = blockIdx.x, g = blockIdx.y, m = A.ctab.m;
+  if (o == A.norb) {
+    if (g) return;
+    fxg_coarse_shares<NU>(A.ctab, A.norm_part, A.Tt, ps, lane, wave);
+    __syncthreads();
+    if (wave == 0) {
+      double y = 0.0;
+#pragma unroll
+      for (int w = 0; w < PMH_EMIT_NW; w++) y += ps[w][lane];
+      if (lane < m) A.y2[lane] = y;
+      const double sq = pmh_wave_all<PMH_RED_SUM>(lane < m ? y * y : 0.0);
+      if (lane == 0) *A.norm_d = sq, *A.norm_h = sq;
+    }
+    return;
+  }
+  const int  a = t >> 2, sl = 2 * (t & 3), no = A.osize[o];
+  const bool live = a < no;
+  const dbl2 *__restrict__ T = (const dbl2 *)(A.tab + (long long)o * 48 * 48);
+  dbl2 tr[6];
+#pragma unroll
+  for (int u = 0; u < 6; u++) {
+    const int p = t + FXN_T * u;
+    tr[u]       = (2 * ((p >> 4) % 24) < no) ? FXA_TAB_LOAD(T + p) : dbl2{0.0, 0.0};
+  }
+  long long rl = 0;
+  fxg_int4  w0 = {0, 0, 0, 0}, w1 = {0, 0, 0, 0};
+  dbl2      d0a = {0.0, 0.0}, d0b = d0a, d1a = d0a, d1b = d0a;
+  if (live) {
+    const long long f = ((long long)g * A.norb + o) * 48 + a;
+    rl = A.recl[f];
+    const fxg_int4 *ri = (const fxg_int4 *)A.gri + f * FXS_S + sl;
+    const dbl2     *rd = (const dbl2 *)A.grd + (f * FXS_S + sl) * 2;
+    w0 = ri[0], w1 = ri[1];
+    d0a = rd[0], d0b = rd[1], d1a = rd[2], d1b = rd[3];
+  }
+  fxg_row<W> R0, R1;
+  fxg_row_load<W>(R0, w0, d0a, d0b, A);
+  fxg_row_load<W>(R1, w1, d1a, d1b, A);
+  fxg_coarse_shares<NU>(A.ctab, A.part, A.S, ps, lane, wave);
+  __syncthreads();
+  if (wave == 0) {
+    double cc = 0.0;
+#pragma unroll
+    for (int w = 0; w < PMH_EMIT_NW; w++) cc += ps[w][lane];
+    cs[lane] = cc;
+    if (o == 0 && g == 0 && lane < m) A.c_out[lane] = cc;
+  }
+#pragma unroll
+  for (int u = 0; u < 6; u++) ts[t + FXN_T * u] = tr[u];
+  __syncthreads();
+  dbl2 v = dbl2{0.0, 0.0};
+  if (live) v.x = fxg_row_sum<W>(R0, cs, A), v.y = fxg_row_sum<W>(R1, cs, A);
+  vs[t] = v;
+  __syncthreads();
+  if (!live) return;
+  const dbl2 *__restrict__ row = ts + ((a >> 4) * 24) * 16 + (a & 15);
+  dbl2 s0 = dbl2{0.0, 0.0}, s1 = s0, s2 = s0, s3 = s0;
+#pragma unroll
+  for (int k = 0; k < 12; k++)
+    if (4 * k < no) {
+      const dbl2  ta = row[16 * (2 * k)], tb = row[16 * (2 * k + 1)];
+      const dbl2 *x = vs + 4 * k * (FXS_S / 2) + (t & 3);
+      const dbl2  x0 = x[0], x1 = x[FXS_S / 2], x2 = x[2 * (FXS_S / 2)], x3 = x[3 * (FXS_S / 2)];
+      s0.x = FXS_MAD(ta.x, x0.x, s0.x), s1.x = FXS_MAD(ta.y, x1.x, s1.x), s2.x = FXS_MAD(tb.x, x2.x, s2.x), s3.x = FXS_MAD(tb.y, x3.x, s3.x);
+      s0.y = FXS_MAD(ta.x, x0.y, s0.y), s1.y = FXS_MAD(ta.y, x1.y, s1.y), s2.y = FXS_MAD(tb.x, x2.y, s2.y), s3.y = FXS_MAD(tb.y, x3.y, s3.y);
+    }
+  const double sx = (s0.x + s1.x) + (s2.x + s3.x), sy = (s0.y + s1.y) + (s2.y + s3.y);
+  A.Xh[rl + 2 * sl] = sx, A.Xh[rl + 2 * sl + 2] = sy;
 }
 
 template <bool TOYH>
diff --git a/permon_amd/csrc/fshared_types.h b/permon_amd/csrc/fshared_types.h
--- a/permon_amd/csrc/fshared_types.h
+++ b/permon_amd/csrc/fshared_types.h
@@ -10,6 +10,7 @@
 #include "reduce.h"
 
 typedef double dbl2 __attribute__((ext_vector_type(2)));
+typedef int    fxg_int4 __attribute__((ext_vector_type(4)));
 
 #define FXS_S 8
 #define FXS_PAD 128
@@ -35,6 +36,9 @@
   double    *d_tabN = nullptr, *d_tabNT = nullptr;
   int       *d_nfx = nullptr, *d_nyd = nullptr;
   long long *d_nxh = nullptr, *d_nyh = nullptr;
+  fxg_int4  *d_gri = nullptr;
+  double    *d_grd = nullptr;
+  double     fused_bytes = 0.0, fused_flops = 0.0;
   double     flops = 0.0, flops_issued = 0.0, bytes = 0.0;
   int        items_of_width[10][4] = {};
 };
@@ -115,6 +119,9 @@
   double                *Afund = nullptr, *cpart = nullptr;
   long long              afund_tot = 0, cpart_cap = 0;
   int                    fxo_ready = 0, fxo_S = 1, stripe_rank = 0, stripe_size = 0;
+  pmh_csr                grec_for = nullptr;
+  unsigned long long     grec_uid = 0;
+  int                    grec_ok = 0, fwd_fused = 0, fwd_timed = 0, last_fused = 0;
   double                 flops = 0.0, flops_issued = 0.0, flops_dense = 0.0;
 };
 
diff --git a/permon_amd/csrc/pmh_internal.h b/permon_amd/csrc/pmh_internal.h
--- a/permon_amd/csrc/pmh_internal.h
+++ b/permon_amd/csrc/pmh_internal.h
@@ -21,6 +21,7 @@
   int chain;
   int chain_applies = 0, chain_launches = 0;
   int chain_replay = 1, chain_replays = 0, chain_replays_redone = 0;
+  int chain_gather_fused = 1, chain_gather_fused_last = 0;
   int gt_fusion = 1;
   int smalxe_prefetch = 1;
   int vec_epi = 1;
@@ -164,6 +165,23 @@
   pmh_emit_out o[2];
 };
 
+struct pmh_gather_fused_args {
+  const double        *x;
+  const double        *part;
+  pmh_emit_tab         tab;
+  int                  nseg, W, NU;
+  const double        *S, *ev;
+  const unsigned char *ec;
+  double              *c_out;
+  const double        *norm_part, *Tt;
+  double              *y2, *norm_d, *norm_h;
+  pmh_csr              gather;
+  unsigned long long   gather_uid;
+  int                  nlist;
+  const int           *h_reci;
+  const double        *h_recd;
+};
+
 struct pmh_op_s {
   pmh_ctx ctx;
   int     n;
@@ -179,6 +197,7 @@
   virtual int     maxeig_start(double * ) { return PMH_EPI_UNSUPPORTED; }
   virtual int     stages(pmh_csr * , double ** , pmh_csr * , const double ** ) { return PMH_EPI_UNSUPPORTED; }
   virtual int     mid_apply() { return pmh_set_error(PMH_ERR_SUP, "this operator has no middle stage"); }
+  virtual int     gather_fused(const pmh_gather_fused_args &) { return PMH_EPI_UNSUPPORTED; }
 };
 
 struct pmh_qppf_s {
```

Result: slower. 4621 QPS iterations/s (-4.7%).
